# tpy001/VFMSeg

Hardware: AMD Instinct MI355X
Metric: train images/sec @512x512 DINOv2-L+LoRA (dg_lora_dinov2_ms_masked, 1024^2 sample = LR+HR 512^2 passes) (higher is better)
Workload: dtype bf16; 1 GPU; configs[1]: dg_lora_dinov2_ms_masked.py, synthetic 1024^2 19-class samples -> 2x512^2 passes, bs=2/GPU, full train step (fwd+bwd+allreduce+AdamW), LoRA dropout on; global_batch=2, parallelism=dp1

## Files before the change

vfmseg_amd/csrc/attention_bf16.hip:

```cpp
#include "attn_bf16_dev.h"

template <bool DQ, int NW = 4>
__global__ void __launch_bounds__(NW * 64, 2) k_attn_bf16_q(AttnP p) {
  extern __shared__ __attribute__((aligned(16))) char smem[];
  const int tid = threadIdx.x, lane = tid & 63;
  const int wave = __builtin_amdgcn_readfirstlane(tid >> 6);
  const int nq = p.nq_main + p.nq_extra, nk = p.nk_main + p.nk_extra;
  int bx, bh;
  {
    const bool light = !DQ && NW == 4 && p.nq_extra == 1 && (p.nq_main & 127) == 0 && nk <= ATTN_EXTRA_MAX;
    const int gx = gridDim.x, nbx = gx - (light ? 1 : 0), nfull = nbx * gridDim.y, lin = blockIdx.y * gx + blockIdx.x;
    if (lin >= nfull) {
      const int e = lin - nfull;
      if constexpr (!DQ) attn_extra_fwd(p, e / p.H, e % p.H, p.nq_main, smem);
      return;
    }
    xcd_map(lin, nbx, gridDim.y, p.xcd, bx, bh);
  }
  const bool cls_key = DQ && NW == 4 && p.nk_extra == 1 && p.cls_scratch != nullptr;
  const int b = bh / p.H, hh = bh % p.H;
  const int col0 = hh * 64;
  const int h = lane >> 5;
  const FragOff fo = frag_offsets(lane);
  const int q0 = bx * (NW * 32) + wave * 32;
  const int qi = q0 + (lane & 31);
  const bool qvalid = qi < nq;
  const long qrow = tok_row(b, qvalid ? qi : nq - 1, p.nq_main, p.B);
  const bf16_t* Kb = (const bf16_t*)p.k;
  const bf16_t* Vb = (const bf16_t*)p.v;
  bf16x8 qf[4], dof[4];
  load_stationary((const bf16_t*)p.q, p.ldq, qrow, col0, h, qf);
  float lse_l = 0.f, delta_l = 0.f;
  if (DQ) {
    load_stationary((const bf16_t*)p.dout, p.ld_do, qrow, col0, h, dof);
    lse_l = p.lse[((long)b * p.H + hh) * nq + (qvalid ? qi : nq - 1)] * LOG2E;
    bf16x8 of[4];
    load_stationary((const bf16_t*)p.o, p.ldo, qrow, col0, h, of);
    float dsum = 0.f;
#pragma unroll
    for (int kk = 0; kk < 4; ++kk)
#pragma unroll
      for (int e2 = 0; e2 < 8; ++e2) dsum = fmaf((float)dof[kk][e2], (float)of[kk][e2], dsum);
    delta_l = half_sum(dsum);
    if (qvalid && h == 0) p.delta[((long)b * p.H + hh) * nq + qi] = -delta_l;
    if (cls_key && p.nq_extra == 1 && bx == 0 && wave == 0) {
      const long crow = tok_row(b, p.nq_main, p.nq_main, p.B);
      bf16x8 cg[4], co[4];
      load_stationary((const bf16_t*)p.dout, p.ld_do, crow, col0, h, cg);
      load_stationary((const bf16_t*)p.o, p.ldo, crow, col0, h, co);
      float cs = 0.f;
#pragma unroll
      for (int kk = 0; kk < 4; ++kk)
#pragma unroll
        for (int e2 = 0; e2 < 8; ++e2) cs = fmaf((float)cg[kk][e2], (float)co[kk][e2], cs);
      cs = half_sum(cs);
      if (lane == 0) p.delta[((long)b * p.H + hh) * nq + p.nq_main] = -cs;
    }
  }
  float p_cls = 0.f, ds_cls = 0.f;
  const float c = p.scale * LOG2E;
  f32x16 oacc[2] = {zero16(), zero16()};
  float m = -INFINITY, l = 0.f;
  const bool r1 = NW == 4 && p.nk_extra == 1 && (!DQ || cls_key);
  const int nk_loop = r1 ? p.nk_main : nk;
  const int nt = (nk_loop + TROWS - 1) / TROWS;
  unsigned koff[8 / NW], voff[8 / NW];
  tile_offsets<NW>(p.ldk, wave, lane, koff);
  tile_offsets<NW>(p.ldv, wave, lane, voff);
  const int n_int = min(nk_loop, p.nk_main) / TROWS;
  const bool span_ok = 64l * p.ldk * 2 < (1l << 31) && 64l * p.ldv * 2 < (1l << 31);
  auto stage = [&](int buf, int t) {
    char* kt = smem + buf * 2 * TILE_BYTES;
    if (t < n_int && span_ok) {
      const long row0 = (long)b * p.nk_main + (long)t * TROWS;
      stage_tile_fast<NW>(Kb + row0 * p.ldk + col0, koff, kt, wave);
      stage_tile_fast<NW>(Vb + row0 * p.ldv + col0, voff, kt + TILE_BYTES, wave);
    } else {
      stage_tile<NW, true>(Kb, p.ldk, col0, b, t * TROWS, nk_loop, p.nk_main, p.B, kt, wave, lane);
      stage_tile<NW, true>(Vb, p.ldv, col0, b, t * TROWS, nk_loop, p.nk_main, p.B, kt + TILE_BYTES, wave, lane);
    }
  };
  stage(0, 0);
  if (r1) {
    const long crow = tok_row(b, p.nk_main, p.nk_main, p.B);
    bf16x8 kcf[4];
    load_stationary(Kb, p.ldk, crow, col0, h, kcf);
    const float s_e = dot_frag(qf, kcf);
    float oc[2][16];
    if (!DQ) {
      load_outcols(Vb, p.ldv, crow, col0, h, oc);
      m = s_e;
      l = h == 0 ? 1.f : 0.f;
#pragma unroll
      for (int j = 0; j < 2; ++j)
#pragma unroll
        for (int r = 0; r < 16; ++r) oacc[j][r] = oc[j][r];
    } else {
      bf16x8 vcf[4];
      load_stationary(Vb, p.ldv, crow, col0, h, vcf);
      const float dp_e = dot_frag(dof, vcf);
      p_cls = __builtin_amdgcn_exp2f(fmaf(s_e, c, -lse_l));
      ds_cls = p_cls * (dp_e - delta_l);
      load_outcols(Kb, p.ldk, crow, col0, h, oc);
#pragma unroll
      for (int j = 0; j < 2; ++j)
#pragma unroll
        for (int r = 0; r < 16; ++r) oacc[j][r] = ds_cls * oc[j][r];
    }
  }
#pragma unroll
  for (int kk = 0; kk < 4; ++kk) {
    asm volatile("" ::"v"(qf[kk]));
    if constexpr (DQ) asm volatile("" ::"v"(dof[kk]));
  }
  asm volatile("" ::"v"(lse_l), "v"(delta_l), "v"(m), "v"(l), "v"(p_cls), "v"(ds_cls));
#pragma unroll
  for (int j = 0; j < 2; ++j) asm volatile("" ::"v"(oacc[j]));
  constexpr int PT = 8 / NW;
  int buf = 0;
  for (int t = 0; t < nt; ++t) {
    const int nbuf = buf == 2 ? 0 : buf + 1;
    const bool il = (p.il & (DQ ? 2 : 1)) && (t + 1 < nt) && (t + 1 < n_int) && span_ok;
    if (t + 1 < nt && !il) {
      stage(nbuf, t + 1);
      if constexpr (NW == 4) asm volatile("s_waitcnt vmcnt(4)" ::: "memory");
      else asm volatile("s_waitcnt vmcnt(8)" ::: "memory");
    } else {
      asm volatile("s_waitcnt vmcnt(0)" ::: "memory");
    }
    __builtin_amdgcn_s_barrier();
    const char* kt = smem + buf * 2 * TILE_BYTES;
    const char* vt = kt + TILE_BYTES;
    f32x16 sacc[2] = {zero16(), zero16()};
    {
      bf16x8 kfr[8];
#pragma unroll
      for (int i = 0; i < 8; ++i) kfr[i] = row_frag(kt, fo, i >> 2, i & 3);
      char* nkt = smem + nbuf * 2 * TILE_BYTES;
      const long row1 = (long)b * p.nk_main + (long)(t + 1) * TROWS;
#pragma unroll
      for (int i = 0; i < 8; ++i) {
        sacc[i >> 2] = MFMA(kfr[i], qf[i & 3], sacc[i >> 2]);
        if (il) {
          if constexpr (NW == 4) {
            if (i & 1) {
              const int j = i >> 1;
              if (j < PT) stage_piece_fast<NW>(Kb + row1 * p.ldk + col0, koff[j], nkt, wave, j);
              else stage_piece_fast<NW>(Vb + row1 * p.ldv + col0, voff[j - PT], nkt + TILE_BYTES, wave, j - PT);
            }
          } else {
            if (i < PT) stage_piece_fast<NW>(Kb + row1 * p.ldk + col0, koff[i], nkt, wave, i);
            else stage_piece_fast<NW>(Vb + row1 * p.ldv + col0, voff[i - PT], nkt + TILE_BYTES, wave, i - PT);
          }
        }
      }
    }
    const bool tail = (t == nt - 1) && (nk_loop % TROWS != 0);
    if (!DQ) {
      float mx = -INFINITY;
      if (tail) {  asm volatile("" ::: "memory");
#pragma unroll
        for (int kb = 0; kb < 2; ++kb)
#pragma unroll
          for (int r = 0; r < 16; ++r)
            if (t * TROWS + kb * 32 + acc_row(r, h) >= nk_loop) sacc[kb][r] = -INFINITY;
      }
      {
        float m4[4] = {-INFINITY, -INFINITY, -INFINITY, -INFINITY};
#pragma unroll
        for (int kb = 0; kb < 2; ++kb)
#pragma unroll
          for (int r = 0; r < 16; ++r) m4[r & 3] = fmaxf(m4[r & 3], sacc[kb][r]);
        mx = fmaxf(fmaxf(m4[0], m4[1]), fmaxf(m4[2], m4[3]));
      }
      mx = half_max(mx);
      const bool need = (mx - m) * c > 8.0f;
      const float mn = need ? mx : m;
      const float alpha = need ? __builtin_amdgcn_exp2f((m - mn) * c) : 1.0f;
      const float mnc = mn * c;
      f32x2 rs2[2] = {f32x2{0.f, 0.f}, f32x2{0.f, 0.f}};
      const f32x2 c2 = f32x2{c, c}, mnc2 = f32x2{-mnc, -mnc};
#pragma unroll
      for (int kb = 0; kb < 2; ++kb)
#pragma unroll
        for (int r = 0; r < 16; r += 2) {
          const f32x2 x = __builtin_elementwise_fma(f32x2{sacc[kb][r], sacc[kb][r + 1]}, c2, mnc2);
          const f32x2 pv = f32x2{__builtin_amdgcn_exp2f(x.x), __builtin_amdgcn_exp2f(x.y)};
          sacc[kb][r] = pv.x, sacc[kb][r + 1] = pv.y;
          rs2[(r >> 1) & 1] += pv;
        }
      l = l * alpha + ((rs2[0].x + rs2[0].y) + (rs2[1].x + rs2[1].y));
      m = mn;
      if (__ballot(alpha != 1.0f) != 0ull) {
#pragma unroll
        for (int j = 0; j < 2; ++j)
#pragma unroll
          for (int r = 0; r < 16; ++r) oacc[j][r] *= alpha;
      }
    } else {
      f32x16 dpacc[2] = {zero16(), zero16()};
#pragma unroll
      for (int kb = 0; kb < 2; ++kb)
#pragma unroll
        for (int kk = 0; kk < 4; ++kk) dpacc[kb] = MFMA(row_frag(vt, fo, kb, kk), dof[kk], dpacc[kb]);
      {
        const f32x2 c2 = f32x2{c, c}, nl2 = f32x2{-lse_l, -lse_l}, nd2 = f32x2{-delta_l, -delta_l};
#pragma unroll
        for (int kb = 0; kb < 2; ++kb)
#pragma unroll
          for (int r = 0; r < 16; r += 2) {
            const f32x2 x = __builtin_elementwise_fma(f32x2{sacc[kb][r], sacc[kb][r + 1]}, c2, nl2);
            const f32x2 pv = f32x2{__builtin_amdgcn_exp2f(x.x), __builtin_amdgcn_exp2f(x.y)};
            const f32x2 ds = pv * (f32x2{dpacc[kb][r], dpacc[kb][r + 1]} + nd2);
            sacc[kb][r] = ds.x, sacc[kb][r + 1] = ds.y;
          }
      }
      if (tail) {  asm volatile("" ::: "memory");
#pragma unroll
        for (int kb = 0; kb < 2; ++kb)
#pragma unroll
          for (int r = 0; r < 16; ++r)
            if (t * TROWS + kb * 32 + acc_row(r, h) >= nk_loop) sacc[kb][r] = 0.f;
      }
    }
    const char* t2 = DQ ? kt : vt;
#pragma unroll
    for (int kb = 0; kb < 2; ++kb)
#pragma unroll
      for (int s = 0; s < 2; ++s) {
        const bf16x8 pb = acc_frag(sacc[kb], s);
#pragma unroll
        for (int j = 0; j < 2; ++j) oacc[j] = MFMA(tr_frag(t2, fo, kb, s, j), pb, oacc[j]);
      }
    buf = nbuf;
  }
  if constexpr (DQ) {
    if (cls_key) {
      __syncthreads();
      float* red = reinterpret_cast<float*>(smem) + wave * (32 * 65);
      float* scr = p.cls_scratch + ((long)b * p.H + hh) * 192;
      float wp = p_cls, wd = ds_cls;
      if (!qvalid) wp = 0.f, wd = 0.f;
      cls_partial(wd, qf, red, lane, scr + 64);
      cls_partial(wp, dof, red, lane, scr + 128);
    }
  }
  float mult;
  if (!DQ) {
    l = half_sum(l);
    mult = 1.f / l;
    if (qvalid && h == 0 && p.lse) p.lse[((long)b * p.H + hh) * nq + qi] = m * p.scale + __logf(l);
  } else {
    mult = p.scale;
  }
  if (qvalid) {
    bf16_t* out = DQ ? (bf16_t*)p.dq : (bf16_t*)p.o;
    const long ldo = DQ ? p.ld_dq : p.ldo;
#pragma unroll
    for (int j = 0; j < 2; ++j) store_block_rows(oacc[j], mult, out + qrow * ldo + col0 + 32 * j, h);
  }
}

template <int NW = 4>
__global__ void __launch_bounds__(NW * 64, 2) k_attn_bf16_dkv(AttnP p) {
  extern __shared__ __attribute__((aligned(16))) char smem[];
  constexpr int STAGE = 2 * TILE_BYTES + 1024;
  const int tid = threadIdx.x, lane = tid & 63;
  const int wave = __builtin_amdgcn_readfirstlane(tid >> 6);
  const int nq = p.nq_main + p.nq_extra, nk = p.nk_main + p.nk_extra;
  int bx, bh;
  xcd_map(blockIdx.y * gridDim.x + blockIdx.x, gridDim.x, gridDim.y, p.xcd, bx, bh);
  const bool cls_query = NW == 4 && p.nq_extra == 1 && p.cls_scratch != nullptr;
  float ds_cls = 0.f;
  const int b = bh / p.H, hh = bh % p.H;
  const int col0 = hh * 64;
  const int h = lane >> 5;
  const FragOff fo = frag_offsets(lane);
  const int k0 = bx * (NW * 32) + wave * 32;
  const int ki = k0 + (lane & 31);
  const bool kvalid = ki < nk;
  const long krow = tok_row(b, kvalid ? ki : nk - 1, p.nk_main, p.B);
  bf16x8 kf[4], vf[4];
  load_stationary((const bf16_t*)p.k, p.ldk, krow, col0, h, kf);
  load_stationary((const bf16_t*)p.v, p.ldv, krow, col0, h, vf);
  const bf16_t* Qb = (const bf16_t*)p.q;
  const bf16_t* Ob = (const bf16_t*)p.dout;
  const float* lse_g = p.lse + ((long)b * p.H + hh) * nq;
  const float* del_g = p.delta + ((long)b * p.H + hh) * nq;
  const float c = p.scale * LOG2E;
  f32x16 dk[2] = {zero16(), zero16()}, dv[2] = {zero16(), zero16()};
  const int nq_loop = cls_query ? p.nq_main : nq;
  const int nt = (nq_loop + TROWS - 1) / TROWS;
  unsigned qoff[8 / NW], ooff[8 / NW];
  tile_offsets<NW>(p.ldq, wave, lane, qoff);
  tile_offsets<NW>(p.ld_do, wave, lane, ooff);
  const int n_int = min(nq_loop, p.nq_main) / TROWS;
  const bool span_ok = 64l * p.ldq * 2 < (1l << 31) && 64l * p.ld_do * 2 < (1l << 31);
  auto stage = [&](int buf, int t) {
    char* qt = smem + buf * STAGE;
    if (t < n_int && span_ok) {
      const long row0 = (long)b * p.nq_main + (long)t * TROWS;
      stage_tile_fast<NW>(Qb + row0 * p.ldq + col0, qoff, qt, wave);
      stage_tile_fast<NW>(Ob + row0 * p.ld_do + col0, ooff, qt + TILE_BYTES, wave);
    } else {
      stage_tile<NW, true>(Qb, p.ldq, col0, b, t * TROWS, nq_loop, p.nq_main, p.B, qt, wave, lane);
      stage_tile<NW, true>(Ob, p.ld_do, col0, b, t * TROWS, nq_loop, p.nq_main, p.B, qt + TILE_BYTES, wave, lane);
    }
    int qq = t * TROWS + lane;
    if (qq > nq_loop - 1) qq = nq_loop - 1;
    const float* src = (wave & 1) ? del_g : lse_g;
    glds4_raw(src + qq, qt + 2 * TILE_BYTES + wave * 256);
  };
  stage(0, 0);
  if (cls_query) {
    const long crow = tok_row(b, p.nq_main, p.nq_main, p.B);
    bf16x8 qcf[4], gcf[4];
    load_stationary(Qb, p.ldq, crow, col0, h, qcf);
    load_stationary(Ob, p.ld_do, crow, col0, h, gcf);
    const float s_e = dot_frag(kf, qcf), dp_e = dot_frag(vf, gcf);
    const float p_e = __builtin_amdgcn_exp2f(fmaf(s_e, c, -lse_g[p.nq_main] * LOG2E));
    ds_cls = p_e * (dp_e + del_g[p.nq_main]);
    float oc[2][16];
    load_outcols(Ob, p.ld_do, crow, col0, h, oc);
#pragma unroll
    for (int j = 0; j < 2; ++j)
#pragma unroll
      for (int r = 0; r < 16; ++r) dv[j][r] = p_e * oc[j][r];
    load_outcols(Qb, p.ldq, crow, col0, h, oc);
#pragma unroll
    for (int j = 0; j < 2; ++j)
#pragma unroll
      for (int r = 0; r < 16; ++r) dk[j][r] = ds_cls * oc[j][r];
  }
#pragma unroll
  for (int kk = 0; kk < 4; ++kk) asm volatile("" ::"v"(kf[kk]), "v"(vf[kk]));
  asm volatile("" ::"v"(ds_cls));
#pragma unroll
  for (int j = 0; j < 2; ++j) asm volatile("" ::"v"(dk[j]), "v"(dv[j]));
  int buf = 0;
  for (int t = 0; t < nt; ++t) {
    const int nbuf = buf == 2 ? 0 : buf + 1;
    if (t + 1 < nt) {
      stage(nbuf, t + 1);
      if constexpr (NW == 4) asm volatile("s_waitcnt vmcnt(5)" ::: "memory");
      else asm volatile("s_waitcnt vmcnt(9)" ::: "memory");
    } else {
      asm volatile("s_waitcnt vmcnt(0)" ::: "memory");
    }
    __builtin_amdgcn_s_barrier();
    const char* qt = smem + buf * STAGE;
    const char* ot = qt + TILE_BYTES;
    const float* lse_s = reinterpret_cast<const float*>(qt + 2 * TILE_BYTES);
    const float* del_s = lse_s + 64;
    const bool tail = (t == nt - 1) && (nq_loop % TROWS != 0);
#pragma unroll
    for (int qb = 0; qb < 2; ++qb) {
      f32x16 sacc = zero16(), dpacc;
#pragma unroll
      for (int g = 0; g < 4; ++g) {
        const float4 nd = *reinterpret_cast<const float4*>(del_s + qb * 32 + 8 * g + 4 * h);
        dpacc[4 * g] = nd.x, dpacc[4 * g + 1] = nd.y, dpacc[4 * g + 2] = nd.z, dpacc[4 * g + 3] = nd.w;
      }
#pragma unroll
      for (int kk = 0; kk < 4; ++kk) {
        sacc = MFMA(row_frag(qt, fo, qb, kk), kf[kk], sacc);
        dpacc = MFMA(row_frag(ot, fo, qb, kk), vf[kk], dpacc);
      }
      f32x16 pacc;
#pragma unroll
      for (int g = 0; g < 4; ++g) {
        const float4 ls = *reinterpret_cast<const float4*>(lse_s + qb * 32 + 8 * g + 4 * h);
        const f32x2 c2 = f32x2{c, c}, nl2e = f32x2{-LOG2E, -LOG2E};
        const f32x2 lsv[2] = {f32x2{ls.x, ls.y} * nl2e, f32x2{ls.z, ls.w} * nl2e};
#pragma unroll
        for (int e = 0; e < 2; ++e) {
          const int r = 4 * g + 2 * e;
          const f32x2 x = __builtin_elementwise_fma(f32x2{sacc[r], sacc[r + 1]}, c2, lsv[e]);
          const f32x2 pv = f32x2{__builtin_amdgcn_exp2f(x.x), __builtin_amdgcn_exp2f(x.y)};
          const f32x2 ds = pv * f32x2{dpacc[r], dpacc[r + 1]};
          pacc[r] = pv.x, pacc[r + 1] = pv.y;
          sacc[r] = ds.x, sacc[r + 1] = ds.y;
        }
      }
      if (tail) {  asm volatile("" ::: "memory");
#pragma unroll
        for (int r = 0; r < 16; ++r)
          if (t * TROWS + qb * 32 + acc_row(r, h) >= nq_loop) pacc[r] = 0.f, sacc[r] = 0.f;
      }
#pragma unroll
      for (int s = 0; s < 2; ++s) {
        const bf16x8 pb = acc_frag(pacc, s), dsb = acc_frag(sacc, s);
#pragma unroll
        for (int j = 0; j < 2; ++j) {
          dv[j] = MFMA(tr_frag(ot, fo, qb, s, j), pb, dv[j]);
          dk[j] = MFMA(tr_frag(qt, fo, qb, s, j), dsb, dk[j]);
        }
      }
    }
    buf = nbuf;
  }
  if (cls_query) {
    __syncthreads();
    float* red = reinterpret_cast<float*>(smem) + wave * (32 * 65);
    float wd = ds_cls;
    if (!kvalid) wd = 0.f;
    cls_partial(wd, kf, red, lane, p.cls_scratch + ((long)b * p.H + hh) * 192);
  }
  if (kvalid) {
    bf16_t* odk = (bf16_t*)p.dk;
    bf16_t* odv = (bf16_t*)p.dv;
#pragma unroll
    for (int j = 0; j < 2; ++j) {
      store_block_rows(dk[j], p.scale, odk + krow * p.ld_dk + col0 + 32 * j, h);
      store_block_rows(dv[j], 1.0f, odv + krow * p.ld_dv + col0 + 32 * j, h);
    }
  }
}

static bool aligned_ok(const vfm_attn_desc* d, bool bwd) {
  auto ok = [](const void* ptr, long ld) { return ((uintptr_t)ptr % 16 == 0) && (ld % 8 == 0); };
  bool r = ok(d->q, d->ldq) && ok(d->k, d->ldk) && ok(d->v, d->ldv) && ok(d->o, d->ldo);
  if (bwd) r = r && ok(d->dout, d->ld_do) && ok(d->dq, d->ld_dq) && ok(d->dk, d->ld_dk) && ok(d->dv, d->ld_dv);
  return r;
}

int g_attn_short_grid = 256;
static bool short_grid(const vfm_attn_desc* d, int n) { return (long)cdiv(n, 128) * d->B * d->H < g_attn_short_grid; }

int g_attn_il = 3;
int g_attn_xcd = 1;
int g_attn_fwd64 = 0;
#ifdef VFM_EXPERIMENTAL_FWD64
bool vfm_attn_fwd64_launch(const vfm_attn_desc* d, const AttnP& p, hipStream_t s);
#else
static bool vfm_attn_fwd64_launch(const vfm_attn_desc*, const AttnP&, hipStream_t) { return false; }
#endif
int g_attn_lds_pad = 0;
int vfm_attn_bf16_fwd_impl(const vfm_attn_desc* d, hipStream_t s) {
  VFM_CHECK(aligned_ok(d, false), VFM_E_ALIGN, "vfm_attn_fwd(bf16): operands must be 16-byte aligned, ld %% 8 == 0");
  const AttnP p = to_p(d);
  const int nq = d->nq_main + d->nq_extra;
  if (g_attn_fwd64 && vfm_attn_fwd64_launch(d, p, s)) {
    VFM_LAUNCH_CHECK();
    return VFM_OK;
  }
  const size_t shm = 6 * TILE_BYTES + g_attn_lds_pad;
  static int attr_pad = -1;
  if (attr_pad != g_attn_lds_pad) {
    (void)hipFuncSetAttribute((const void*)k_attn_bf16_q<false, 4>, hipFuncAttributeMaxDynamicSharedMemorySize, (int)shm);
    attr_pad = g_attn_lds_pad;
  }
  if (short_grid(d, nq)) hipLaunchKernelGGL((k_attn_bf16_q<false, 2>), dim3(cdiv(nq, 64), d->B * d->H), dim3(128), shm, s, p);
  else hipLaunchKernelGGL((k_attn_bf16_q<false, 4>), dim3(cdiv(nq, 128), d->B * d->H), dim3(256), shm, s, p);
  VFM_LAUNCH_CHECK();
  return VFM_OK;
}

__global__ void __launch_bounds__(64) k_attn_cls_finish(AttnP p) {
  const int bh = blockIdx.x, b = bh / p.H, hh = bh % p.H, lane = threadIdx.x;
  const int nq = p.nq_main + p.nq_extra;
  const long row = tok_row(b, p.nq_main, p.nq_main, p.B);
  const int col = hh * 64 + lane;
  const float qc = bf16_to_f32(((const bf16_t*)p.q)[row * p.ldq + col]), kc = bf16_to_f32(((const bf16_t*)p.k)[row * p.ldk + col]);
  const float vc = bf16_to_f32(((const bf16_t*)p.v)[row * p.ldv + col]), gc = bf16_to_f32(((const bf16_t*)p.dout)[row * p.ld_do + col]);
  const float s = wave_sum(qc * kc) * p.scale, dp = wave_sum(gc * vc);
  const float lse = p.lse[(long)bh * nq + p.nq_main], ndelta = p.delta[(long)bh * nq + p.nq_main];
  const float pv = __expf(s - lse), ds = pv * (dp + ndelta);
  float* scr = p.cls_scratch + (long)bh * 192;
  ((bf16_t*)p.dq)[row * p.ld_dq + col] = f32_to_bf16((scr[lane] + ds * kc) * p.scale);
  ((bf16_t*)p.dk)[row * p.ld_dk + col] = f32_to_bf16((scr[64 + lane] + ds * qc) * p.scale);
  ((bf16_t*)p.dv)[row * p.ld_dv + col] = f32_to_bf16(scr[128 + lane] + pv * gc);
  scr[lane] = 0.f, scr[64 + lane] = 0.f, scr[128 + lane] = 0.f;
}

int vfm_attn_bf16_bwd_impl(const vfm_attn_desc* d, hipStream_t s) {
  VFM_CHECK(aligned_ok(d, true), VFM_E_ALIGN, "vfm_attn_bwd(bf16): operands must be 16-byte aligned, ld %% 8 == 0");
  AttnP p = to_p(d);
  const int nq = d->nq_main + d->nq_extra, nk = d->nk_main + d->nk_extra;
  const bool cls = d->nq_extra == 1 && d->nk_extra == 1 && d->nq_main == d->nk_main && (d->nq_main % 128) == 0 && !short_grid(d, nq);
  p.cls_scratch = cls ? d->delta + (long)d->B * d->H * nq : nullptr;
  if (short_grid(d, nq)) hipLaunchKernelGGL((k_attn_bf16_q<true, 2>), dim3(cdiv(nq, 64), d->B * d->H), dim3(128), 6 * TILE_BYTES, s, p);
  else hipLaunchKernelGGL((k_attn_bf16_q<true, 4>), dim3(cdiv(cls ? d->nq_main : nq, 128), d->B * d->H), dim3(256), 6 * TILE_BYTES, s, p);
  if (short_grid(d, nk)) hipLaunchKernelGGL((k_attn_bf16_dkv<2>), dim3(cdiv(nk, 64), d->B * d->H), dim3(128), 3 * (2 * TILE_BYTES + 1024), s, p);
  else hipLaunchKernelGGL((k_attn_bf16_dkv<4>), dim3(cdiv(cls ? d->nk_main : nk, 128), d->B * d->H), dim3(256), 3 * (2 * TILE_BYTES + 1024), s, p);
  if (cls) hipLaunchKernelGGL(k_attn_cls_finish, dim3(d->B * d->H), dim3(64), 0, s, p);
  VFM_LAUNCH_CHECK();
  return VFM_OK;
}
```

vfmseg_amd/csrc/attn_common.h:

```cpp
#pragma once
#include "common.h"

struct AttnP {
  const void* q; const void* k; const void* v; void* o;
  int dt; long ldq, ldk, ldv, ldo;
  int B, H;
  int nq_main, nq_extra, nk_main, nk_extra;
  float scale;
  float* lse;
  const void* dout; long ld_do;
  void* dq; void* dk; void* dv; long ld_dq, ld_dk, ld_dv;
  float* delta;
  float* cls_scratch;
  int xcd;
  int il;
};

__device__ __forceinline__ long tok_row(int b, int i, int n_main, int B) {
  return i < n_main ? (long)b * n_main + i : (long)B * n_main + b;
}


static inline AttnP to_p(const vfm_attn_desc* d) {
  AttnP p;
  p.q = d->q; p.k = d->k; p.v = d->v; p.o = d->o;
  p.dt = d->dt; p.ldq = d->ldq; p.ldk = d->ldk; p.ldv = d->ldv; p.ldo = d->ldo;
  p.B = d->B; p.H = d->H;
  p.nq_main = d->nq_main; p.nq_extra = d->nq_extra; p.nk_main = d->nk_main; p.nk_extra = d->nk_extra;
  p.scale = d->scale; p.lse = d->lse;
  p.dout = d->dout; p.ld_do = d->ld_do;
  p.dq = d->dq; p.dk = d->dk; p.dv = d->dv; p.ld_dq = d->ld_dq; p.ld_dk = d->ld_dk; p.ld_dv = d->ld_dv;
  p.delta = d->delta;
  p.cls_scratch = nullptr;
  extern int g_attn_xcd;
  p.xcd = g_attn_xcd;
  extern int g_attn_il;
  p.il = g_attn_il;
  return p;
}
```

vfmseg_amd/csrc/elementwise.hip:

```cpp
#include "common.h"

thread_local char g_vfm_err[512] = {0};

extern "C" const char* vfm_last_error(void) { return g_vfm_err; }
extern "C" int vfm_abi_version(void) { return 5; }
extern "C" int vfm_half_kind(void) { return VFM_HALF_KIND; }

template <typename TI, typename TO>
__global__ void k_cast(const TI* __restrict__ src, long ld_src, TO* __restrict__ dst, long ld_dst, long rows, long cols,
                       const float* __restrict__ colscale) {
  const long cols4 = cols >> 2;
  const long total = rows * cols4;
  for (long i = blockIdx.x * (long)blockDim.x + threadIdx.x; i < total; i += (long)gridDim.x * blockDim.x) {
    const long r = i / cols4, c = (i - r * cols4) << 2;
    float v[4];
#pragma unroll
    for (int j = 0; j < 4; ++j) v[j] = ld_f32(src + r * ld_src + c + j);
    if (colscale) {
#pragma unroll
      for (int j = 0; j < 4; ++j) v[j] *= colscale[c + j];
    }
#pragma unroll
    for (int j = 0; j < 4; ++j) st_f32(dst + r * ld_dst + c + j, v[j]);
  }
  const long tail0 = cols4 << 2;
  const long ntail = cols - tail0;
  if (ntail) {
    for (long i = blockIdx.x * (long)blockDim.x + threadIdx.x; i < rows * ntail; i += (long)gridDim.x * blockDim.x) {
      const long r = i / ntail, c = tail0 + (i - r * ntail);
      float v = ld_f32(src + r * ld_src + c);
      if (colscale) v *= colscale[c];
      st_f32(dst + r * ld_dst + c, v);
    }
  }
}

extern "C" int vfm_cast(const void* src, int src_dt, long ld_src, void* dst, int dst_dt, long ld_dst, long rows, long cols,
                        const float* colscale, void* stream) {
  VFM_CHECK(rows >= 0 && cols >= 0 && ld_src >= cols && ld_dst >= cols, VFM_E_SHAPE, "vfm_cast: bad shape");
  if (rows == 0 || cols == 0) return VFM_OK;
  hipStream_t s = (hipStream_t)stream;
  const long total = rows * ((cols + 3) / 4);
  const int grid = (int)((total + 255) / 256 > 4096 ? 4096 : (total + 255) / 256);
#define L(TI, TO) hipLaunchKernelGGL((k_cast<TI, TO>), dim3(grid), dim3(256), 0, s, (const TI*)src, ld_src, (TO*)dst, ld_dst, rows, cols, colscale)
  if (src_dt == VFM_F32 && dst_dt == VFM_F32) L(float, float);
  else if (src_dt == VFM_F32 && dst_dt == VFM_BF16) L(float, bf16_t);
  else if (src_dt == VFM_BF16 && dst_dt == VFM_F32) L(bf16_t, float);
  else if (src_dt == VFM_BF16 && dst_dt == VFM_BF16) L(bf16_t, bf16_t);
  else VFM_FAIL(VFM_E_INVAL, "vfm_cast: dtype");
#undef L
  VFM_LAUNCH_CHECK();
  return VFM_OK;
}

__global__ void k_split3(const float* __restrict__ src, long sr, long sc, bf16_t* __restrict__ dst, long ld_dst, long rows, long K, long Kp,
                         int pattern) {
  const long per_row = Kp / 4;
  const long total = rows * per_row;
  for (long i = (long)blockIdx.x * blockDim.x + threadIdx.x; i < total; i += (long)gridDim.x * blockDim.x) {
    const long r = i / per_row, c = (i % per_row) * 4;
    float v[4];
    if (sc == 1 && c + 3 < K && ((reinterpret_cast<uintptr_t>(src + r * sr + c) & 15) == 0)) {
      const float4 f = *reinterpret_cast<const float4*>(src + r * sr + c);
      v[0] = f.x, v[1] = f.y, v[2] = f.z, v[3] = f.w;
    } else {
#pragma unroll
      for (int e = 0; e < 4; ++e) v[e] = (c + e < K) ? src[r * sr + (c + e) * sc] : 0.f;
    }
    ushort4 hi, lo;
    bf16_t* ph = &hi.x;
    bf16_t* pl = &lo.x;
#pragma unroll
    for (int e = 0; e < 4; ++e) {
      ph[e] = f32_to_bf16(v[e]);
      pl[e] = f32_to_bf16(v[e] - bf16_to_f32(ph[e]));
    }
    bf16_t* d = dst + r * ld_dst + c;
    *reinterpret_cast<ushort4*>(d) = hi;
    *reinterpret_cast<ushort4*>(d + Kp) = pattern == 0 ? hi : lo;
    *reinterpret_cast<ushort4*>(d + 2 * Kp) = pattern == 0 ? lo : hi;
  }
}

extern "C" int vfm_split3(const float* src, long stride_r, long stride_c, void* dst, long ld_dst, long rows, long K, int pattern, void* stream) {
  const long Kp = (K + 63) / 64 * 64;
  VFM_CHECK(rows >= 0 && K > 0 && ld_dst >= 3 * Kp && ld_dst % 4 == 0 && ((uintptr_t)dst % 8) == 0 && (pattern == 0 || pattern == 1), VFM_E_SHAPE,
            "vfm_split3: dst must hold rows x 3 ceil64(K) bf16 (ld %% 4 == 0, 8-byte aligned)");
  if (rows == 0) return VFM_OK;
  const long total = rows * (Kp / 4);
  const int grid = (int)((total + 255) / 256 > 8192 ? 8192 : (total + 255) / 256);
  hipLaunchKernelGGL(k_split3, dim3(grid), dim3(256), 0, (hipStream_t)stream, src, stride_r, stride_c, (bf16_t*)dst, ld_dst, rows, K, Kp, pattern);
  VFM_LAUNCH_CHECK();
  return VFM_OK;
}

template <typename TI, typename TO>
__global__ void k_transpose(const TI* __restrict__ src, long ld_src, TO* __restrict__ dst, long ld_dst, long rows, long cols,
                            long pad_rows) {
  __shared__ float tile[64][65];
  const long r0 = (long)blockIdx.y * 64, c0 = (long)blockIdx.x * 64;
  const int tx = threadIdx.x & 63, ty = threadIdx.x >> 6;
  for (int i = ty; i < 64; i += 4) {
    const long r = r0 + i, c = c0 + tx;
    tile[i][tx] = (r < rows && c < cols) ? ld_f32(src + r * ld_src + c) : 0.f;
  }
  __syncthreads();
  for (int i = ty; i < 64; i += 4) {
    const long c = c0 + i, r = r0 + tx;
    if (c < cols && r < pad_rows) st_f32(dst + c * ld_dst + r, tile[tx][i]);
  }
}

extern "C" int vfm_transpose(const void* src, int src_dt, long ld_src, void* dst, int dst_dt, long ld_dst, long rows, long cols,
                             long pad_rows, void* stream) {
  VFM_CHECK(pad_rows >= rows && ld_dst >= pad_rows && ld_src >= cols, VFM_E_SHAPE, "vfm_transpose: bad shape");
  if (cols == 0 || pad_rows == 0) return VFM_OK;
  hipStream_t s = (hipStream_t)stream;
  dim3 grid(cdiv(cols, 64), cdiv(pad_rows, 64));
#define L(TI, TO) hipLaunchKernelGGL((k_transpose<TI, TO>), grid, dim3(256), 0, s, (const TI*)src, ld_src, (TO*)dst, ld_dst, rows, cols, pad_rows)
  if (src_dt == VFM_F32 && dst_dt == VFM_F32) L(float, float);
  else if (src_dt == VFM_F32 && dst_dt == VFM_BF16) L(float, bf16_t);
  else if (src_dt == VFM_BF16 && dst_dt == VFM_F32) L(bf16_t, float);
  else if (src_dt == VFM_BF16 && dst_dt == VFM_BF16) L(bf16_t, bf16_t);
  else VFM_FAIL(VFM_E_INVAL, "vfm_transpose: dtype");
#undef L
  VFM_LAUNCH_CHECK();
  return VFM_OK;
}

template <typename TI, typename TO>
__global__ void k_strided_copy(const TI* __restrict__ src, TO* __restrict__ dst, long n0, long n1, long n2, long n3, long s0,
                               long s1, long s2, long s3, long d0, long d1, long d2, long d3, int accumulate) {
  const long total = n0 * n1 * n2 * n3;
  for (long i = blockIdx.x * (long)blockDim.x + threadIdx.x; i < total; i += (long)gridDim.x * blockDim.x) {
    long t = i;
    const long i3 = t % n3; t /= n3;
    const long i2 = t % n2; t /= n2;
    const long i1 = t % n1; t /= n1;
    const float v = ld_f32(src + t * s0 + i1 * s1 + i2 * s2 + i3 * s3);
    TO* q = dst + t * d0 + i1 * d1 + i2 * d2 + i3 * d3;
    st_f32(q, accumulate ? ld_f32(q) + v : v);
  }
}

extern "C" int vfm_strided_copy(const void* src, int src_dt, void* dst, int dst_dt, long n0, long n1, long n2, long n3,
                                long s0, long s1, long s2, long s3, long d0, long d1, long d2, long d3, int accumulate,
                                void* stream) {
  const long total = n0 * n1 * n2 * n3;
  if (total == 0) return VFM_OK;
  hipStream_t s = (hipStream_t)stream;
  const int grid = (int)((total + 255) / 256 > 4096 ? 4096 : (total + 255) / 256);
#define L(TI, TO) hipLaunchKernelGGL((k_strided_copy<TI, TO>), dim3(grid), dim3(256), 0, s, (const TI*)src, (TO*)dst, n0, n1, n2, n3, s0, s1, s2, s3, d0, d1, d2, d3, accumulate)
  if (src_dt == VFM_F32 && dst_dt == VFM_F32) L(float, float);
  else if (src_dt == VFM_F32 && dst_dt == VFM_BF16) L(float, bf16_t);
  else if (src_dt == VFM_BF16 && dst_dt == VFM_F32) L(bf16_t, float);
  else if (src_dt == VFM_BF16 && dst_dt == VFM_BF16) L(bf16_t, bf16_t);
  else VFM_FAIL(VFM_E_INVAL, "vfm_strided_copy: dtype");
#undef L
  VFM_LAUNCH_CHECK();
  return VFM_OK;
}

__global__ void k_axpby(const float* __restrict__ x, float a, float* __restrict__ y, float b, long n) {
  for (long i = blockIdx.x * (long)blockDim.x + threadIdx.x; i < n; i += (long)gridDim.x * blockDim.x)
    y[i] = (b == 0.f) ? a * x[i] : a * x[i] + b * y[i];
}
extern "C" int vfm_axpby(const float* x, float a, float* y, float b, long n, void* stream) {
  if (n == 0) return VFM_OK;
  const int grid = (int)((n + 255) / 256 > 4096 ? 4096 : (n + 255) / 256);
  hipLaunchKernelGGL(k_axpby, dim3(grid), dim3(256), 0, (hipStream_t)stream, x, a, y, b, n);
  VFM_LAUNCH_CHECK();
  return VFM_OK;
}
__global__ void k_scale_dev(float* __restrict__ y, const float* __restrict__ sc, long n) {
  const float s = *sc;
  for (long i = blockIdx.x * (long)blockDim.x + threadIdx.x; i < n; i += (long)gridDim.x * blockDim.x) y[i] *= s;
}
extern "C" int vfm_scale_by_device_scalar(float* y, const float* scalar, long n, void* stream) {
  if (n == 0) return VFM_OK;
  const int grid = (int)((n + 255) / 256 > 4096 ? 4096 : (n + 255) / 256);
  hipLaunchKernelGGL(k_scale_dev, dim3(grid), dim3(256), 0, (hipStream_t)stream, y, scalar, n);
  VFM_LAUNCH_CHECK();
  return VFM_OK;
}

template <typename T>
__global__ void k_colsum1(const T* __restrict__ x, long ld, long rows, long cols, float* __restrict__ ws, int CT) {
  __shared__ float sh[256];
  const int rl = 256 / CT;
  const int tx = threadIdx.x % CT, ty = threadIdx.x / CT;
  const long c = (long)blockIdx.x * CT + tx;
  float acc = 0.f;
  if (c < cols)
    for (long r = (long)blockIdx.y * rl + ty; r < rows; r += (long)gridDim.y * rl) acc += ld_f32(x + r * ld + c);
  sh[threadIdx.x] = acc;
  __syncthreads();
  if (ty == 0 && c < cols) {
    float a = 0.f;
    for (int k = 0; k < rl; ++k) a += sh[k * CT + tx];
    ws[(long)blockIdx.y * cols + c] = a;
  }
}
__global__ void __launch_bounds__(256) k_colsum2(const float* __restrict__ ws, long cols, int parts, float* __restrict__ out, int accumulate) {
  __shared__ float sh[4][64];
  const int tx = threadIdx.x & 63, g = threadIdx.x >> 6;
  const long c = blockIdx.x * 64L + tx;
  float a = 0.f;
  if (c < cols) {
    int p = g;
    for (; p + 12 < parts; p += 16) {
      const float v0 = ws[(long)p * cols + c], v1 = ws[(long)(p + 4) * cols + c], v2 = ws[(long)(p + 8) * cols + c], v3 = ws[(long)(p + 12) * cols + c];
      a += (v0 + v1) + (v2 + v3);
    }
    for (; p < parts; p += 4) a += ws[(long)p * cols + c];
  }
  sh[g][tx] = a;
  __syncthreads();
  if (g == 0 && c < cols) {
    const float t = (sh[0][tx] + sh[1][tx]) + (sh[2][tx] + sh[3][tx]);
    out[c] = accumulate ? out[c] + t : t;
  }
}
extern "C" int vfm_colsum(const void* x, int dt, long ld, long rows, long cols, float* out, int accumulate, float* ws,
                          void* stream) {
  VFM_CHECK(ld >= cols && ws, VFM_E_SHAPE, "vfm_colsum: bad args");
  if (cols == 0) return VFM_OK;
  hipStream_t s = (hipStream_t)stream;
  int CT = 64;
  while (CT > 8 && CT / 2 >= cols) CT /= 2;
  const int rl = 256 / CT;
  long parts = (rows + rl * 8 - 1) / (rl * 8);
  if (parts > 64) parts = 64;
  if (parts < 1) parts = 1;
  dim3 grid(cdiv(cols, CT), (unsigned)parts);
  if (dt == VFM_F32) hipLaunchKernelGGL(k_colsum1<float>, grid, dim3(256), 0, s, (const float*)x, ld, rows, cols, ws, CT);
  else if (dt == VFM_BF16) hipLaunchKernelGGL(k_colsum1<bf16_t>, grid, dim3(256), 0, s, (const bf16_t*)x, ld, rows, cols, ws, CT);
  else VFM_FAIL(VFM_E_INVAL, "vfm_colsum: dtype");
  hipLaunchKernelGGL(k_colsum2, dim3(cdiv(cols, 64)), dim3(256), 0, s, ws, cols, (int)parts, out, accumulate);
  VFM_LAUNCH_CHECK();
  return VFM_OK;
}

__global__ void k_slab_reduce(const float* __restrict__ slabs, int kch, long P, long Q, long rows_used, float alpha,
                              float* __restrict__ dst, long sp, long sq, int accumulate) {
  const long total = rows_used * Q;
  for (long i = blockIdx.x * (long)blockDim.x + threadIdx.x; i < total; i += (long)gridDim.x * blockDim.x) {
    const long p = i / Q, q = i - p * Q;
    float a = 0.f;
    for (int k = 0; k < kch; ++k) a += slabs[((long)k * P + p) * Q + q];
    a *= alpha;
    float* d = dst + p * sp + q * sq;
    *d = accumulate ? *d + a : a;
  }
}
extern "C" int vfm_slab_reduce(const float* slabs, int kch, long P, long Q, long rows_used, float alpha, float* dst, long sp,
                               long sq, int accumulate, void* stream) {
  VFM_CHECK(kch >= 1 && rows_used >= 0 && rows_used <= P, VFM_E_SHAPE, "vfm_slab_reduce: bad shape");
  const long total = rows_used * Q;
  if (total == 0) return VFM_OK;
  const int grid = (int)((total + 255) / 256 > 4096 ? 4096 : (total + 255) / 256);
  hipLaunchKernelGGL(k_slab_reduce, dim3(grid), dim3(256), 0, (hipStream_t)stream, slabs, kch, P, Q, rows_used, alpha, dst, sp, sq,
                     accumulate);
  VFM_LAUNCH_CHECK();
  return VFM_OK;
}

__global__ void __launch_bounds__(256) k_strided_copy_batch(const vfm_copy_job* __restrict__ tab) {
  const vfm_copy_job t = tab[blockIdx.y];
  const unsigned n1 = (unsigned)t.n[1], n2 = (unsigned)t.n[2], n3 = (unsigned)t.n[3];
  const unsigned total = (unsigned)t.n[0] * n1 * n2 * n3;
  for (unsigned i = blockIdx.x * 256u + threadIdx.x; i < total; i += gridDim.x * 256u) {
    unsigned r = i;
    const unsigned i3 = r % n3; r /= n3;
    const unsigned i2 = r % n2; r /= n2;
    const unsigned i1 = r % n1; r /= n1;
    const float* sp = t.src + ((long)r * t.s[0] + (long)i1 * t.s[1] + (long)i2 * t.s[2] + (long)i3 * t.s[3]);
    float v = sp[0];
    for (long c = 1; c < t.nsum; ++c) v += sp[c * t.sum_stride];
    const long o = (long)r * t.d[0] + (long)i1 * t.d[1] + (long)i2 * t.d[2] + (long)i3 * t.d[3];
    if (t.accumulate) ((float*)t.dst)[o] += v;
    else st_any(t.dst, o, (int)t.dst_dt, v);
  }
}
extern "C" int vfm_strided_copy_batch(const vfm_copy_job* table_dev, int njobs, long max_elems, void* stream) {
  VFM_CHECK(table_dev && njobs >= 0, VFM_E_INVAL, "vfm_strided_copy_batch: bad args");
  if (njobs == 0 || max_elems <= 0) return VFM_OK;
  VFM_CHECK(max_elems < (1l << 31), VFM_E_SHAPE, "vfm_strided_copy_batch: jobs are limited to 2^31 elements");
  int gx = (int)((max_elems + 2047) / 2048);
  if (gx > 2048) gx = 2048;
  if (gx < 1) gx = 1;
  hipLaunchKernelGGL(k_strided_copy_batch, dim3(gx, njobs), dim3(256), 0, (hipStream_t)stream, table_dev);
  VFM_LAUNCH_CHECK();
  return VFM_OK;
}

__global__ void k_lora_pack(const vfm_lora_site* __restrict__ tab, int dt) {
  const vfm_lora_site t = tab[blockIdx.y];
  const long na = t.r * t.K, nb = t.N * t.r;
  for (long i = blockIdx.x * (long)blockDim.x + threadIdx.x; i < na + nb; i += (long)gridDim.x * blockDim.x) {
    if (i < na) {
      const long rr = i / t.K, k = i - rr * t.K;
      const float v = t.A[i];
      st_any(t.a, rr * t.ld_a + k, dt, v);
      st_any(t.at, k * t.ld_at + rr, dt, v);
    } else {
      const long j = i - na;
      const long n = j / t.r, rr = j - n * t.r;
      const float v = t.B[j];
      st_any(t.w, n * t.ld_w + t.Kw + rr, dt, v);
      if (t.wt) st_any(t.wt, (t.Kw + rr) * t.ld_wt + n, dt, v);
    }
  }
}
extern "C" int vfm_lora_pack(const vfm_lora_site* table_dev, int nsites, long max_elems, int dt, void* stream) {
  VFM_CHECK(table_dev && nsites >= 0 && (dt == VFM_F32 || dt == VFM_BF16), VFM_E_INVAL, "vfm_lora_pack: bad args");
  if (nsites == 0) return VFM_OK;
  int gx = (int)((max_elems + 255) / 256);
  if (gx > 256) gx = 256;
  if (gx < 1) gx = 1;
  hipLaunchKernelGGL(k_lora_pack, dim3(gx, nsites), dim3(256), 0, (hipStream_t)stream, table_dev, dt);
  VFM_LAUNCH_CHECK();
  return VFM_OK;
}

struct F8 { float v[8]; };
__device__ __forceinline__ F8 ld8_bf16(const bf16_t* p) {
  const uint4 u = *reinterpret_cast<const uint4*>(p);
  F8 r;
  r.v[0] = h16_lo(u.x), r.v[1] = h16_hi(u.x);
  r.v[2] = h16_lo(u.y), r.v[3] = h16_hi(u.y);
  r.v[4] = h16_lo(u.z), r.v[5] = h16_hi(u.z);
  r.v[6] = h16_lo(u.w), r.v[7] = h16_hi(u.w);
  return r;
}
__device__ __forceinline__ void st8_bf16(bf16_t* p, const F8& r) {
  uint4 u;
  u.x = (uint32_t)f32_to_bf16(r.v[0]) | ((uint32_t)f32_to_bf16(r.v[1]) << 16);
  u.y = (uint32_t)f32_to_bf16(r.v[2]) | ((uint32_t)f32_to_bf16(r.v[3]) << 16);
  u.z = (uint32_t)f32_to_bf16(r.v[4]) | ((uint32_t)f32_to_bf16(r.v[5]) << 16);
  u.w = (uint32_t)f32_to_bf16(r.v[6]) | ((uint32_t)f32_to_bf16(r.v[7]) << 16);
  *reinterpret_cast<uint4*>(p) = u;
}
__device__ __forceinline__ F8 ld8_f32(const float* p) {
  const float4 a = *reinterpret_cast<const float4*>(p), b = *reinterpret_cast<const float4*>(p + 4);
  F8 r;
  r.v[0] = a.x, r.v[1] = a.y, r.v[2] = a.z, r.v[3] = a.w, r.v[4] = b.x, r.v[5] = b.y, r.v[6] = b.z, r.v[7] = b.w;
  return r;
}
__device__ __forceinline__ void st8_f32(float* p, const F8& r) {
  *reinterpret_cast<float4*>(p) = make_float4(r.v[0], r.v[1], r.v[2], r.v[3]);
  *reinterpret_cast<float4*>(p + 4) = make_float4(r.v[4], r.v[5], r.v[6], r.v[7]);
}
static inline bool al16(const void* p) { return ((uintptr_t)p & 15) == 0; }
static inline int grid8(long total8) { return (int)((total8 + 255) / 256 > 16384 ? 16384 : (total8 + 255) / 256); }

__global__ void k_dropout_mask_bf16x8(bf16_t* __restrict__ out, long n8, float p, float keep_scale, uint64_t seed, uint64_t offset) {
  for (long i = blockIdx.x * (long)blockDim.x + threadIdx.x; i < n8; i += (long)gridDim.x * blockDim.x) {
    F8 r;
#pragma unroll
    for (int e = 0; e < 8; ++e) {
      const float u = (hash_u32(seed, offset + (uint64_t)(i * 8 + e)) >> 8) * (1.0f / 16777216.0f);
      r.v[e] = u >= p ? keep_scale : 0.f;
    }
    st8_bf16(out + i * 8, r);
  }
}
__global__ void k_mul_mask_bf16x8(const bf16_t* __restrict__ src, long ld_src, const bf16_t* __restrict__ mask, long mask_ld, long rpg,
                                  bf16_t* __restrict__ dst, long ld_dst, long rows, int cols8) {
  const long total = rows * cols8;
  for (long i = blockIdx.x * (long)blockDim.x + threadIdx.x; i < total; i += (long)gridDim.x * blockDim.x) {
    const long r = i / cols8;
    const int c = (int)(i - r * cols8) * 8;
    F8 a = ld8_bf16(src + r * ld_src + c);
    const F8 m = ld8_bf16(mask + (r / rpg) * mask_ld + c);
#pragma unroll
    for (int e = 0; e < 8; ++e) a.v[e] *= m.v[e];
    st8_bf16(dst + r * ld_dst + c, a);
  }
}
__global__ void k_act_grad_mul_bf16x8(const bf16_t* __restrict__ dy, long ld_dy, const bf16_t* __restrict__ pre, long ld_pre,
                                      bf16_t* __restrict__ out, long ld_out, long rows, int cols8, int act) {
  const long total = rows * cols8;
  for (long i = blockIdx.x * (long)blockDim.x + threadIdx.x; i < total; i += (long)gridDim.x * blockDim.x) {
    const long r = i / cols8;
    const int c = (int)(i - r * cols8) * 8;
    F8 d = ld8_bf16(dy + r * ld_dy + c);
    const F8 p = ld8_bf16(pre + r * ld_pre + c);
#pragma unroll
    for (int e = 0; e < 8; ++e) {
      const float x = p.v[e];
      const float g = act == VFM_ACT_GELU ? gelu_grad_f(x) : (act == VFM_ACT_RELU ? (x > 0.f ? 1.f : 0.f) : (act == VFM_ACT_QGELU ? qgelu_grad_f(x) : 1.f));
      d.v[e] *= g;
    }
    st8_bf16(out + r * ld_out + c, d);
  }
}
template <bool OUT_BF16>
__global__ void k_swiglu_fwd_x8(const bf16_t* __restrict__ h, long ld_h, void* __restrict__ out, long ld_out, long rows, long C, int c8) {
  const long total = rows * c8;
  for (long i = blockIdx.x * (long)blockDim.x + threadIdx.x; i < total; i += (long)gridDim.x * blockDim.x) {
    const long r = i / c8;
    const int c = (int)(i - r * c8) * 8;
    const F8 a = ld8_bf16(h + r * ld_h + c), g = ld8_bf16(h + r * ld_h + C + c);
    F8 o;
#pragma unroll
    for (int e = 0; e < 8; ++e) o.v[e] = a.v[e] / (1.f + __expf(-a.v[e])) * g.v[e];
    if constexpr (OUT_BF16) st8_bf16((bf16_t*)out + r * ld_out + c, o);
    else st8_f32((float*)out + r * ld_out + c, o);
  }
}
template <bool DO_BF16>
__global__ void k_swiglu_bwd_x8(const bf16_t* __restrict__ h, long ld_h, const void* __restrict__ dout, long ld_do, bf16_t* __restrict__ dh,
                                long ld_dh, long rows, long C, int c8) {
  const long total = rows * c8;
  for (long i = blockIdx.x * (long)blockDim.x + threadIdx.x; i < total; i += (long)gridDim.x * blockDim.x) {
    const long r = i / c8;
    const int c = (int)(i - r * c8) * 8;
    const F8 a = ld8_bf16(h + r * ld_h + c), g = ld8_bf16(h + r * ld_h + C + c);
    F8 d;
    if constexpr (DO_BF16) d = ld8_bf16((const bf16_t*)dout + r * ld_do + c);
    else d = ld8_f32((const float*)dout + r * ld_do + c);
    F8 da, dg;
#pragma unroll
    for (int e = 0; e < 8; ++e) {
      const float sg = 1.f / (1.f + __expf(-a.v[e]));
      da.v[e] = d.v[e] * g.v[e] * sg * (1.f + a.v[e] * (1.f - sg));
      dg.v[e] = d.v[e] * a.v[e] * sg;
    }
    st8_bf16(dh + r * ld_dh + c, da);
    st8_bf16(dh + r * ld_dh + C + c, dg);
  }
}

template <typename T>
__global__ void k_dropout_mask(T* __restrict__ out, long n, float p, float keep_scale, uint64_t seed, uint64_t offset) {
  for (long i = blockIdx.x * (long)blockDim.x + threadIdx.x; i < n; i += (long)gridDim.x * blockDim.x) {
    const float u = (hash_u32(seed, offset + (uint64_t)i) >> 8) * (1.0f / 16777216.0f);
    st_f32(out + i, u >= p ? keep_scale : 0.f);
  }
}
extern "C" int vfm_dropout_mask(void* out, int dt, long n, float p, uint64_t seed, uint64_t offset, void* stream) {
  VFM_CHECK(p >= 0.f && p < 1.f, VFM_E_INVAL, "vfm_dropout_mask: p");
  if (n == 0) return VFM_OK;
  const int grid = (int)((n + 255) / 256 > 4096 ? 4096 : (n + 255) / 256);
  const float ks = 1.0f / (1.0f - p);
  if (dt == VFM_F32) hipLaunchKernelGGL(k_dropout_mask<float>, dim3(grid), dim3(256), 0, (hipStream_t)stream, (float*)out, n, p, ks, seed, offset);
  else if (dt == VFM_BF16 && n % 8 == 0 && al16(out))
    hipLaunchKernelGGL(k_dropout_mask_bf16x8, dim3(grid8(n / 8)), dim3(256), 0, (hipStream_t)stream, (bf16_t*)out, n / 8, p, ks, seed, offset);
  else if (dt == VFM_BF16) hipLaunchKernelGGL(k_dropout_mask<bf16_t>, dim3(grid), dim3(256), 0, (hipStream_t)stream, (bf16_t*)out, n, p, ks, seed, offset);
  else VFM_FAIL(VFM_E_INVAL, "vfm_dropout_mask: dtype");
  VFM_LAUNCH_CHECK();
  return VFM_OK;
}

__global__ void k_mul_mask(const void* __restrict__ src, int src_dt, long ld_src, const void* __restrict__ mask, int mask_dt,
                           long mask_ld, long rpg, void* __restrict__ dst, int dst_dt, long ld_dst, long rows, long cols) {
  const long total = rows * cols;
  for (long i = blockIdx.x * (long)blockDim.x + threadIdx.x; i < total; i += (long)gridDim.x * blockDim.x) {
    const long r = i / cols, c = i - r * cols;
    const float m = ld_any(mask, (r / rpg) * mask_ld + c, mask_dt);
    st_any(dst, r * ld_dst + c, dst_dt, ld_any(src, r * ld_src + c, src_dt) * m);
  }
}
template <typename TS, typename TM, typename TD>
__global__ void k_mul_mask_x8(const TS* __restrict__ src, long ld_src, const TM* __restrict__ mask, long mask_ld, long rpg, TD* __restrict__ dst,
                              long ld_dst, long rows, int cols8) {
  const long total = rows * cols8;
  for (long i = blockIdx.x * (long)blockDim.x + threadIdx.x; i < total; i += (long)gridDim.x * blockDim.x) {
    const long r = i / cols8;
    const int c = (int)(i - r * cols8) * 8;
    F8 a, m;
    if constexpr (sizeof(TS) == 2) a = ld8_bf16(src + r * ld_src + c); else a = ld8_f32(src + r * ld_src + c);
    if constexpr (sizeof(TM) == 2) m = ld8_bf16(mask + (r / rpg) * mask_ld + c); else m = ld8_f32(mask + (r / rpg) * mask_ld + c);
#pragma unroll
    for (int e = 0; e < 8; ++e) a.v[e] *= m.v[e];
    if constexpr (sizeof(TD) == 2) st8_bf16(dst + r * ld_dst + c, a); else st8_f32(dst + r * ld_dst + c, a);
  }
}
template <typename TS, typename TM, typename TD>
static void launch_mul_mask_x8(const void* src, long ld_src, const void* mask, long mask_ld, long rpg, void* dst, long ld_dst, long rows, long cols,
                               hipStream_t s) {
  hipLaunchKernelGGL((k_mul_mask_x8<TS, TM, TD>), dim3(grid8(rows * cols / 8)), dim3(256), 0, s, (const TS*)src, ld_src, (const TM*)mask, mask_ld, rpg,
                     (TD*)dst, ld_dst, rows, (int)(cols / 8));
}
extern "C" int vfm_mul_mask(const void* src, int src_dt, long ld_src, const void* mask, int mask_dt, long mask_ld,
                            long rows_per_group, void* dst, int dst_dt, long ld_dst, long rows, long cols, void* stream) {
  VFM_CHECK(rows_per_group >= 1, VFM_E_INVAL, "vfm_mul_mask: rows_per_group");
  const long total = rows * cols;
  if (total == 0) return VFM_OK;
  auto h16 = [](int dt) { return dt == VFM_BF16; };
  auto okdt = [](int dt) { return dt == VFM_BF16 || dt == VFM_F32; };
  if (okdt(src_dt) && okdt(mask_dt) && okdt(dst_dt) && !(h16(src_dt) && h16(mask_dt) && h16(dst_dt)) && cols % 8 == 0 && ld_src % 8 == 0 &&
      mask_ld % 8 == 0 && ld_dst % 8 == 0 && al16(src) && al16(mask) && al16(dst)) {
    hipStream_t s = (hipStream_t)stream;
    const int key = (h16(src_dt) ? 4 : 0) | (h16(mask_dt) ? 2 : 0) | (h16(dst_dt) ? 1 : 0);
#define MM(TS, TM, TD) launch_mul_mask_x8<TS, TM, TD>(src, ld_src, mask, mask_ld, rows_per_group, dst, ld_dst, rows, cols, s)
    switch (key) {
      case 0: MM(float, float, float); break;
      case 1: MM(float, float, bf16_t); break;
      case 2: MM(float, bf16_t, float); break;
      case 3: MM(float, bf16_t, bf16_t); break;
      case 4: MM(bf16_t, float, float); break;
      case 5: MM(bf16_t, float, bf16_t); break;
      default: MM(bf16_t, bf16_t, float); break;
    }
#undef MM
    VFM_LAUNCH_CHECK();
    return VFM_OK;
  }
  if (src_dt == VFM_BF16 && mask_dt == VFM_BF16 && dst_dt == VFM_BF16 && cols % 8 == 0 && ld_src % 8 == 0 && mask_ld % 8 == 0 && ld_dst % 8 == 0 &&
      al16(src) && al16(mask) && al16(dst)) {
    hipLaunchKernelGGL(k_mul_mask_bf16x8, dim3(grid8(total / 8)), dim3(256), 0, (hipStream_t)stream, (const bf16_t*)src, ld_src, (const bf16_t*)mask,
                       mask_ld, rows_per_group, (bf16_t*)dst, ld_dst, rows, (int)(cols / 8));
    VFM_LAUNCH_CHECK();
    return VFM_OK;
  }
  const int grid = (int)((total + 255) / 256 > 8192 ? 8192 : (total + 255) / 256);
  hipLaunchKernelGGL(k_mul_mask, dim3(grid), dim3(256), 0, (hipStream_t)stream, src, src_dt, ld_src, mask, mask_dt, mask_ld,
                     rows_per_group, dst, dst_dt, ld_dst, rows, cols);
  VFM_LAUNCH_CHECK();
  return VFM_OK;
}

__global__ void k_geglu_fwd(const void* __restrict__ h, int h_dt, long ld_h, void* __restrict__ out, int out_dt, long ld_out,
                            long rows, long C) {
  const long total = rows * C;
  for (long i = blockIdx.x * (long)blockDim.x + threadIdx.x; i < total; i += (long)gridDim.x * blockDim.x) {
    const long r = i / C, c = i - r * C;
    const float a = ld_any(h, r * ld_h + c, h_dt), g = ld_any(h, r * ld_h + C + c, h_dt);
    st_any(out, r * ld_out + c, out_dt, a * gelu_f(g));
  }
}
__global__ void k_geglu_bwd(const void* __restrict__ h, int h_dt, long ld_h, const void* __restrict__ dout, int do_dt,
                            long ld_do, void* __restrict__ dh, int dh_dt, long ld_dh, long rows, long C) {
  const long total = rows * C;
  for (long i = blockIdx.x * (long)blockDim.x + threadIdx.x; i < total; i += (long)gridDim.x * blockDim.x) {
    const long r = i / C, c = i - r * C;
    const float a = ld_any(h, r * ld_h + c, h_dt), g = ld_any(h, r * ld_h + C + c, h_dt);
    const float d = ld_any(dout, r * ld_do + c, do_dt);
    st_any(dh, r * ld_dh + c, dh_dt, d * gelu_f(g));
    st_any(dh, r * ld_dh + C + c, dh_dt, d * a * gelu_grad_f(g));
// ... 297 lines not shown
```

vfmseg_amd/csrc/gemm_bf16.hip:

```cpp
#include "gemm_dev.h"

template <int BM, int BN, int WM_W, int WN_W, int NS>
struct Cfg {
  static constexpr int WAVES = WM_W * WN_W;
  static constexpr int THREADS = WAVES * 64;
  static constexpr int A_BYTES = BM * BK * 2, B_BYTES = BN * BK * 2;
  static constexpr int STAGE_BYTES = A_BYTES + B_BYTES;
  static constexpr int A_PIECES = BM / 8 / WAVES, B_PIECES = BN / 8 / WAVES;
  static constexpr int PIECES = A_PIECES + B_PIECES;
  static constexpr int WM = BM / WM_W, WN = BN / WN_W;
  static constexpr int MI = WM / 32, NI = WN / 32;
  static constexpr int EPI_LD = WN + 4;
  static constexpr int EPI_BYTES = WAVES * 32 * EPI_LD * 4;
  static constexpr int SMEM = (NS * STAGE_BYTES > EPI_BYTES) ? NS * STAGE_BYTES : EPI_BYTES;
  static_assert(BM % (8 * WAVES) == 0 && BN % (8 * WAVES) == 0, "tile rows must split into whole DMA pieces per wave");
  static_assert(WM % 32 == 0 && WN % 32 == 0, "wave tile must be a multiple of the 32x32 MFMA");
};

typedef short s16x4 __attribute__((ext_vector_type(4)));

__device__ __attribute__((aligned(16))) unsigned char g_zero_row[512];
template <int BM, int BN, int WM_W, int WN_W, int NS, bool VEC, bool BT, bool AT = false>
__global__ void __launch_bounds__(WM_W* WN_W * 64)
    k_gemm_bf16(const bf16_t* __restrict__ A, long lda, const bf16_t* __restrict__ B, long ldb, long M, long N, long K,
                long stride_a, long stride_b, long stride_c, int tiles_m, int tiles_n, long kb_rows, EpiParams e, SkinnyTail sk) {
  using C = Cfg<BM, BN, WM_W, WN_W, NS>;
  extern __shared__ __attribute__((aligned(16))) char smem[];
  if constexpr (!BT && C::THREADS == 512 && C::SMEM >= 65536) {
    if (sk.nblk > 0 && (int)blockIdx.x >= tiles_m * tiles_n) {
      skinny_tile(sk.A, sk.lda, B, ldb, sk.M, N, K, (long)((int)blockIdx.x - tiles_m * tiles_n) * 32, sk.e, 0, smem);
      return;
    }
  }
  const int tid = threadIdx.x, lane = tid & 63;
  const int wave = __builtin_amdgcn_readfirstlane(tid >> 6);
  const int wm = wave / WN_W, wn = wave % WN_W;

  const int ntiles = tiles_m * tiles_n;
  int bid = blockIdx.x;
  {
    const int q = ntiles >> 3, r = ntiles & 7, xcd = bid & 7, idx = bid >> 3;
    bid = (xcd < r ? xcd * (q + 1) : r * (q + 1) + (xcd - r) * q) + idx;
  }
  constexpr int GM = 8;
  const int group = bid / (GM * tiles_n);
  const int first_m = group * GM;
  const int gsz = min(tiles_m - first_m, GM);
  const int tm = first_m + (bid % (GM * tiles_n)) % gsz;
  const int tn = (bid % (GM * tiles_n)) / gsz;
  const long m0 = (long)tm * BM, n0 = (long)tn * BN;
  const long z = blockIdx.y;
  const bf16_t* Ab = A + z * stride_a;
  const bf16_t* Bb = B + z * stride_b;
  long kb_valid = K;
  if constexpr (BT) {
    if (kb_rows > 0) {
      kb_valid = kb_rows - (ldb > 0 ? z * (stride_b / ldb) : 0);
      if (kb_valid > K) kb_valid = K;
      if (kb_valid < 1) kb_valid = 1;
    } else if (kb_rows < 0) {
      kb_valid = -kb_rows;
      if (kb_valid > K) kb_valid = K;
    }
  }

  const int lr = lane >> 3, pc = lane & 7;
  const bf16_t* a_src[C::A_PIECES];
  const bf16_t* b_src[C::B_PIECES];
  int at_row[C::A_PIECES];
#pragma unroll
  for (int j = 0; j < C::A_PIECES; ++j) {
    if constexpr (!AT) {
      const int r = (wave * C::A_PIECES + j) * 8 + lr;
      long gm = m0 + r;
      if (gm > M - 1) gm = M - 1;
      a_src[j] = Ab + gm * lda + ((pc ^ ((r >> 1) & 7)) << 3);
    } else {
      static_assert(!AT || (BT && BM == 128), "transposed-A path: BM = 128 (256-byte LDS rows), together with transposed B");
      const int piece = wave * C::A_PIECES + j;
      const int r = piece * 4 + (lane >> 4);
      const int c = (lane & 15) ^ ((r & 3) << 2);
      long gm = m0 + c * 8;
      if (gm > M - 8) gm = M - 8;
      at_row[j] = r;
      a_src[j] = Ab + gm;
    }
  }
  int bt_row[C::B_PIECES];
#pragma unroll
  for (int j = 0; j < C::B_PIECES; ++j) {
    if constexpr (!BT) {
      const int r = (wave * C::B_PIECES + j) * 8 + lr;
      long gn = n0 + r;
      if (gn > N - 1) gn = N - 1;
      b_src[j] = Bb + gn * ldb + ((pc ^ ((r >> 1) & 7)) << 3);
    } else {
      static_assert(!BT || BN == 128, "transposed-B path is built for BN = 128 (256-byte LDS rows)");
      const int piece = wave * C::B_PIECES + j;
      const int r = piece * 4 + (lane >> 4);
      const int c = (lane & 15) ^ ((r & 3) << 2);
      long gn = n0 + c * 8;
      if (gn > N - 8) gn = N - 8;
      bt_row[j] = r;
      b_src[j] = Bb + gn;
    }
  }
  auto stage = [&](int slot, long k0) {
    char* sa = smem + slot * C::STAGE_BYTES;
    char* sb = sa + C::A_BYTES;
#pragma unroll
    for (int j = 0; j < C::A_PIECES; ++j) {
      if constexpr (!AT) {
        glds16(a_src[j] + k0, sa + (wave * C::A_PIECES + j) * 1024);
      } else {
        const long kr = k0 + at_row[j];
        const bf16_t* src = kr < kb_valid ? a_src[j] + kr * lda : reinterpret_cast<const bf16_t*>(g_zero_row) + (lane & 15) * 8;
        glds16(src, sa + (wave * C::A_PIECES + j) * 1024);
      }
    }
#pragma unroll
    for (int j = 0; j < C::B_PIECES; ++j) {
      if constexpr (!BT) {
        glds16(b_src[j] + k0, sb + (wave * C::B_PIECES + j) * 1024);
      } else {
        long kr = k0 + bt_row[j];
        if (kr > kb_valid - 1) kr = kb_valid - 1;
        glds16(b_src[j] + kr * ldb, sb + (wave * C::B_PIECES + j) * 1024);
      }
    }
  };

  f32x16 acc[C::MI][C::NI];
#pragma unroll
  for (int i = 0; i < C::MI; ++i)
#pragma unroll
    for (int j = 0; j < C::NI; ++j)
#pragma unroll
      for (int r = 0; r < 16; ++r) acc[i][j][r] = 0.f;

  const int fr = lane & 31, fh = lane >> 5;
  int a_off[C::MI], a_sw[C::MI], b_off[C::NI], b_sw[C::NI];
#pragma unroll
  for (int i = 0; i < C::MI; ++i) {
    const int r = wm * C::WM + i * 32 + fr;
    a_off[i] = r * 128;
    a_sw[i] = (r >> 1) & 7;
  }
#pragma unroll
  for (int j = 0; j < C::NI; ++j) {
    const int r = wn * C::WN + j * 32 + fr;
    b_off[j] = r * 128;
    b_sw[j] = (r >> 1) & 7;
  }

  const int nk = (int)(K / BK);
#pragma unroll
  for (int s = 0; s < NS - 1; ++s)
    if (s < nk) stage(s, (long)s * BK);

  for (int t = 0; t < nk; ++t) {
    const int inflight = min(NS - 2, nk - 1 - t);
    if (inflight >= NS - 2 && NS >= 2) wait_vmcnt<(NS - 2) * C::PIECES>();
    else if (NS >= 4 && inflight == NS - 3) wait_vmcnt<(NS >= 3 ? (NS - 3) : 0) * C::PIECES>();
    else if (NS >= 5 && inflight == NS - 4) wait_vmcnt<(NS >= 4 ? (NS - 4) : 0) * C::PIECES>();
    else wait_vmcnt<0>();
    __builtin_amdgcn_s_barrier();
    if (t + NS - 1 < nk) stage((t + NS - 1) % NS, (long)(t + NS - 1) * BK);
    const char* sa = smem + (t % NS) * C::STAGE_BYTES;
    const char* sb = sa + C::A_BYTES;
    auto read_b = [&](int s2, int j) -> bf16x8 {
      if constexpr (!BT) {
        return *reinterpret_cast<const bf16x8*>(sb + b_off[j] + (((2 * s2 + fh) ^ b_sw[j]) << 4));
      } else {
        const int g = lane >> 4, i2 = lane & 15, q = i2 >> 2, p = i2 & 3, h2 = g >> 1;
        const int chunk = (wn * C::WN + j * 32) / 8 + 2 * (g & 1) + (p >> 1);
        const int r0 = 16 * s2 + 8 * h2 + q, r1 = r0 + 4;
        const s16x4 lo = __builtin_amdgcn_ds_read_tr16_b64_v4i16(
            (__attribute__((address_space(3))) s16x4*)(sb + r0 * 256 + ((chunk ^ ((r0 & 3) << 2)) << 4) + ((p & 1) << 3)));
        const s16x4 hi = __builtin_amdgcn_ds_read_tr16_b64_v4i16(
            (__attribute__((address_space(3))) s16x4*)(sb + r1 * 256 + ((chunk ^ ((r1 & 3) << 2)) << 4) + ((p & 1) << 3)));
        union { struct { s16x4 a, b; } st; bf16x8 v; } u;
        u.st.a = lo;
        u.st.b = hi;
        return u.v;
      }
    };
    auto read_a = [&](int s2, int i) -> bf16x8 {
      if constexpr (!AT) {
        return *reinterpret_cast<const bf16x8*>(sa + a_off[i] + (((2 * s2 + fh) ^ a_sw[i]) << 4));
      } else {
        const int g = lane >> 4, i2 = lane & 15, q = i2 >> 2, p = i2 & 3, h2 = g >> 1;
        const int chunk = (wm * C::WM + i * 32) / 8 + 2 * (g & 1) + (p >> 1);
        const int r0 = 16 * s2 + 8 * h2 + q, r1 = r0 + 4;
        const s16x4 lo = __builtin_amdgcn_ds_read_tr16_b64_v4i16(
            (__attribute__((address_space(3))) s16x4*)(sa + r0 * 256 + ((chunk ^ ((r0 & 3) << 2)) << 4) + ((p & 1) << 3)));
        const s16x4 hi = __builtin_amdgcn_ds_read_tr16_b64_v4i16(
            (__attribute__((address_space(3))) s16x4*)(sa + r1 * 256 + ((chunk ^ ((r1 & 3) << 2)) << 4) + ((p & 1) << 3)));
        union { struct { s16x4 a, b; } st; bf16x8 v; } u;
        u.st.a = lo;
        u.st.b = hi;
        return u.v;
      }
    };
    bf16x8 af[2][C::MI], bfr[2][C::NI];
#pragma unroll
    for (int i = 0; i < C::MI; ++i) af[0][i] = read_a(0, i);
#pragma unroll
    for (int j = 0; j < C::NI; ++j) bfr[0][j] = read_b(0, j);
#pragma unroll
    for (int s = 0; s < BK / 16; ++s) {
      const int cur = s & 1, nxt = cur ^ 1;
      if (s + 1 < BK / 16) {
#pragma unroll
        for (int i = 0; i < C::MI; ++i)
          af[nxt][i] = read_a(s + 1, i);
#pragma unroll
        for (int j = 0; j < C::NI; ++j) bfr[nxt][j] = read_b(s + 1, j);
      }
#pragma unroll
      for (int i = 0; i < C::MI; ++i)
#pragma unroll
        for (int j = 0; j < C::NI; ++j)
          acc[i][j] = VFM_MFMA16(af[cur][i], bfr[cur][j], acc[i][j]);
    }
  }

  const long zoff = z * stride_c;
  __syncthreads();
  float* img = reinterpret_cast<float*>(smem) + wave * 32 * C::EPI_LD;
  if constexpr (VEC) epi_wave_tile<C::MI, C::NI, 1>(e, zoff, acc, img, lane, m0 + wm * C::WM, n0 + wn * C::WN, M, N);
  else epi_scalar<C::MI, C::NI, 1>(e, zoff, acc, img, lane, m0 + wm * C::WM, n0 + wn * C::WN, M, N);
}

template <int BM, int BN, int WM_W, int WN_W, int NS, bool VEC, bool BT, bool AT = false>
static bool launch_one(const vfm_gemm_desc* d, hipStream_t s, const vfm_gemm_desc* tail = nullptr) {
  using C = Cfg<BM, BN, WM_W, WN_W, NS>;
  const int tiles_m = cdiv(d->M, BM), tiles_n = cdiv(d->N, BN);
  const long batch = d->batch > 0 ? d->batch : 1;
  static bool attr = false;
  if (!attr) {
    (void)hipFuncSetAttribute((const void*)k_gemm_bf16<BM, BN, WM_W, WN_W, NS, VEC, BT, AT>, hipFuncAttributeMaxDynamicSharedMemorySize, C::SMEM);
    attr = true;
  }
  SkinnyTail sk;
  sk.nblk = 0;
  const bool fold = tail && !BT && C::THREADS == 512 && C::SMEM >= 65536 && batch == 1;
  if (fold) {
    sk.A = (const bf16_t*)tail->A, sk.lda = tail->sa_m, sk.M = tail->M, sk.nblk = cdiv(tail->N, 32), sk.e = make_epi(tail);
  }
  dim3 grid(tiles_m * tiles_n + sk.nblk, (unsigned)batch), blk(C::THREADS);
  const long ldb = BT ? d->sb_k : d->sb_n;
  const long kb_rows = d->kb_rows;
  hipLaunchKernelGGL((k_gemm_bf16<BM, BN, WM_W, WN_W, NS, VEC, BT, AT>), grid, blk, C::SMEM, s, (const bf16_t*)d->A, AT ? d->sa_k : d->sa_m,
                     (const bf16_t*)d->B, ldb, d->M, d->N, d->K, d->stride_a, d->stride_b, d->stride_c, tiles_m, tiles_n, kb_rows,
                     make_epi(d), sk);
  return fold || !tail;
}

template <int BM, int BN, int WM_W, int WN_W, int NS>
static bool launch_cfg(const vfm_gemm_desc* d, hipStream_t s, bool vec, const vfm_gemm_desc* tail = nullptr) {
  if (vec) return launch_one<BM, BN, WM_W, WN_W, NS, true, false>(d, s, tail);
  return launch_one<BM, BN, WM_W, WN_W, NS, false, false>(d, s, tail);
}

template <int BM, int WM_W, int WN_W, int NS = 2>
static void launch_bt(const vfm_gemm_desc* d, hipStream_t s, bool vec) {
  if (vec) launch_one<BM, 128, WM_W, WN_W, NS, true, true>(d, s);
  else launch_one<BM, 128, WM_W, WN_W, NS, false, true>(d, s);
}

__global__ void __launch_bounds__(512) k_gemm_bf16_skinny(const bf16_t* __restrict__ A, long lda, const bf16_t* __restrict__ B, long ldb,
                                                          long M, long N, long K, long stride_a, long stride_b, long stride_c,
                                                          EpiParams e) {
  __shared__ __attribute__((aligned(16))) char stg[65536];
  const long z = blockIdx.y;
  skinny_tile(A + z * stride_a, lda, B + z * stride_b, ldb, M, N, K, (long)blockIdx.x * 32, e, z * stride_c, stg);
}

static void launch_skinny(const vfm_gemm_desc* d, hipStream_t s) {
  const long batch = d->batch > 0 ? d->batch : 1;
  hipLaunchKernelGGL(k_gemm_bf16_skinny, dim3(cdiv(d->N, 32), (unsigned)batch), dim3(512), 0, s, (const bf16_t*)d->A, d->sa_m,
                     (const bf16_t*)d->B, d->sb_n, d->M, d->N, d->K, d->stride_a, d->stride_b, d->stride_c, make_epi(d));
}

static int g_force_cfg = -1;
static int g_split_tail = 3;
static int g_batch_tiles = 1;
static int g_bt64 = 1;
static int g_fold_tail = 1;
static int g_use_pp = 184;
long g_nt_bytes = 0;
static int g_use_ps = 0;
static int g_use_192 = 3;
static int g_w44_k = 1024;
static int g_deep_sep_k = 0;
static int g_deep_tail_k = 0;
extern "C" int vfm_tune(const char* key, int value) {
  if (key && strcmp(key, "gemm_cfg") == 0) {
    g_force_cfg = value;
    return VFM_OK;
  }
  if (key && strcmp(key, "pp_dbg") == 0) {
    extern int g_pp_dbg;
    g_pp_dbg = value;
    return VFM_OK;
  }
  if (key && strcmp(key, "attn_short_grid") == 0) {
    extern int g_attn_short_grid;
    g_attn_short_grid = value;
    return VFM_OK;
  }
  if (key && strcmp(key, "attn_il") == 0) {
    if (value < 0 || value > 3) VFM_FAIL(VFM_E_INVAL, "vfm_tune(attn_il): 0 .. 3");
    extern int g_attn_il;
    g_attn_il = value;
    return VFM_OK;
  }
  if (key && strcmp(key, "attn_xcd") == 0) {
    extern int g_attn_xcd;
    g_attn_xcd = value;
    return VFM_OK;
  }
  if (key && strcmp(key, "attn_fwd64") == 0) {
    extern int g_attn_fwd64;
    g_attn_fwd64 = value;
    return VFM_OK;
  }
  if (key && strcmp(key, "attn_lds_pad") == 0) {
    extern int g_attn_lds_pad;
    g_attn_lds_pad = value;
    return VFM_OK;
  }
  if (key && strcmp(key, "gemm_w44_k") == 0) {
    if (value < 0) VFM_FAIL(VFM_E_INVAL, "vfm_tune(gemm_w44_k): negative value");
    g_w44_k = value;
    return VFM_OK;
  }
  if (key && strcmp(key, "gemm_deep_sep_k") == 0) {
    if (value < 0) return VFM_E_INVAL;
    g_deep_sep_k = value;
    return VFM_OK;
  }
  if (key && strcmp(key, "gemm_deep_tail_k") == 0) {
    g_deep_tail_k = value;
    return VFM_OK;
  }
  if (key && strcmp(key, "gemm_nt_mb") == 0) {
    g_nt_bytes = (long)value << 20;
    return VFM_OK;
  }
  if (key && strcmp(key, "ps_burst") == 0) {
#ifdef VFM_EXPERIMENTAL_GEMM
    extern int g_ps_burst;
    g_ps_burst = value;
#endif
    return VFM_OK;
  }
  if (key && strcmp(key, "gemm_use_ps") == 0) {
    g_use_ps = value;
    return VFM_OK;
  }
  if (key && strcmp(key, "gemm_use_pp") == 0) {
    g_use_pp = value;
    return VFM_OK;
  }
  if (key && strcmp(key, "gemm_use_192") == 0) {
    g_use_192 = value;
    return VFM_OK;
  }
  if (key && strcmp(key, "gemm_batch_tiles") == 0) {
    g_batch_tiles = value;
    return VFM_OK;
  }
  if (key && strcmp(key, "gemm_bt64") == 0) {
    g_bt64 = value;
    return VFM_OK;
  }
  if (key && strcmp(key, "gemm_fold_tail") == 0) {
    g_fold_tail = value;
    return VFM_OK;
  }
  if (key && strcmp(key, "gemm_split_tail") == 0) {
    g_split_tail = value;
    return VFM_OK;
  }
  VFM_FAIL(VFM_E_INVAL, "vfm_tune: unknown key");
}

static bool vec_ok(const vfm_gemm_desc* d) {
  auto a16 = [](const void* p) { return ((uintptr_t)p % 16) == 0; };
  const long bm = d->bias_mod > 0 ? d->bias_mod : d->N;
  bool ok = (d->N % 4 == 0) && (d->ldc % 4 == 0) && a16(d->C) && (d->stride_c % 4 == 0);
  if (d->bias) ok = ok && a16(d->bias) && (bm % 4 == 0);
  if (d->colscale) ok = ok && a16(d->colscale);
  if (d->residual) ok = ok && a16(d->residual) && (d->ldr % 4 == 0);
  if (d->aux) ok = ok && a16(d->aux) && (d->ld_aux % 4 == 0);
  if (d->C2) ok = ok && a16(d->C2) && (d->ldc2 % 4 == 0);
  return ok;
}

static int gemm_main(const vfm_gemm_desc* d, hipStream_t s, const vfm_gemm_desc* tail = nullptr, bool* folded = nullptr);
bool vfm_gemm_launch_pp256(const vfm_gemm_desc* d, hipStream_t s, bool vec, const vfm_gemm_desc* tail);
bool vfm_gemm_launch_pp128(const vfm_gemm_desc* d, hipStream_t s, bool vec, const vfm_gemm_desc* tail);
bool vfm_gemm_launch_w4(const vfm_gemm_desc* d, hipStream_t s, bool vec, const vfm_gemm_desc* tail, int waves);
bool vfm_gemm_splitk_ok(const vfm_gemm_desc* d, bool vec);
bool vfm_gemm_launch_w4_splitk(const vfm_gemm_desc* d, hipStream_t s, const vfm_gemm_desc* tail);
#ifdef VFM_EXPERIMENTAL_GEMM
bool vfm_gemm_launch_v5(const vfm_gemm_desc* d, hipStream_t s, bool vec, const vfm_gemm_desc* tail, int form);
bool vfm_gemm_ps_ok(const vfm_gemm_desc* d, int per);
bool vfm_gemm_launch_ps(const vfm_gemm_desc* d, hipStream_t s, const vfm_gemm_desc* tail, int per);
#else
static bool vfm_gemm_launch_v5(const vfm_gemm_desc*, hipStream_t, bool, const vfm_gemm_desc*, int) { return false; }
static bool vfm_gemm_ps_ok(const vfm_gemm_desc*, int) { return false; }
static bool vfm_gemm_launch_ps(const vfm_gemm_desc*, hipStream_t, const vfm_gemm_desc*, int) { return false; }
#endif

int vfm_gemm_bf16_impl(const vfm_gemm_desc* d0, hipStream_t s) {
  const long tail = d0->M % 128;
  const bool bt = (d0->sb_n == 1 && d0->sb_k != 1);
  if (bt) return gemm_main(d0, s);
  const long t128m = (long)((d0->M - tail) / 128) * cdiv(d0->N, 128);
  const bool pp_coarse = !(g_use_pp & 64) && tail > 0 && t128m >= 96 && t128m <= 160 && d0->N >= 512 && d0->K >= 1024 && d0->batch <= 1;
  const bool rows64 = !pp_coarse && d0->N > 32 && d0->K >= 512 && (long)cdiv(d0->M, 128) * cdiv(d0->N, 128) <= 160 &&
                      (long)cdiv(d0->M, 64) * cdiv(d0->N, 64) <= 544;
  if (g_split_tail && !(rows64 && (g_split_tail & 2)) && d0->M > 512 && tail > 0 && tail <= 32 && (d0->batch <= 1)) {
    vfm_gemm_desc dm = *d0, dt = *d0;
    const long mm = d0->M - tail;
    dm.M = mm;
    dt.M = tail;
    auto adv = [&](const void* p, int dt_, long ld) -> const void* {
      return p ? (const void*)((const char*)p + mm * ld * (dt_ == VFM_BF16 || dt_ == VFM_SPLIT3 ? 2 : 4)) : nullptr;
    };
    dt.A = adv(d0->A, VFM_BF16, d0->sa_m);
    dt.C = (void*)adv(d0->C, d0->c_dt, d0->ldc);
    dt.residual = adv(d0->residual, d0->r_dt, d0->ldr);
    dt.aux = adv(d0->aux, d0->aux_dt, d0->ld_aux);
    dt.C2 = (void*)adv(d0->C2, d0->c2_dt, d0->ldc2);
    bool folded = false;
    int rc = gemm_main(&dm, s, g_fold_tail ? &dt : nullptr, &folded);
    if (rc) return rc;
    if (!folded) launch_skinny(&dt, s);
    return VFM_OK;
  }
  if (d0->M <= 32 && d0->N >= 32) {
    launch_skinny(d0, s);
    return VFM_OK;
  }
  return gemm_main(d0, s);
}

static int gemm_main(const vfm_gemm_desc* d, hipStream_t s, const vfm_gemm_desc* tail, bool* folded) {
  const bool vec = vec_ok(d);
  bool fd = false;
  if (d->sb_n == 1 && d->sb_k != 1) {
    if (d->sa_m == 1 && d->sa_k != 1) {
      if (vec) launch_one<128, 128, 2, 4, 2, true, true, true>(d, s);
      else launch_one<128, 128, 2, 4, 2, false, true, true>(d, s);
      return VFM_OK;
    }
    const bool few = (long)cdiv(d->M, 128) * cdiv(d->N, 128) * (d->batch > 0 ? d->batch : 1) < 128;
    if (d->M <= 64 || (g_bt64 && few)) launch_bt<64, 1, 4>(d, s, vec);
    else launch_bt<128, 2, 4>(d, s, vec);
    return VFM_OK;
  }
  int cfg = g_force_cfg;
  if (cfg < 0) {
    const long nbatch = d->batch > 0 ? d->batch : 1;
    const long t128 = (long)cdiv(d->M, 128) * cdiv(d->N, 128) * (g_batch_tiles ? nbatch : 1);
    const long t256 = (long)cdiv(d->M, 256) * cdiv(d->N, 256);
    const bool span31 = (d->M + 128) * d->sa_m < (1l << 31) && (d->N + 128) * d->sb_n < (1l << 31);
    const bool span33 = (d->M + 256) * d->sa_m < (1l << 31) && (d->N + 256) * d->sb_n < (1l << 31);
    const long t192 = (long)cdiv(d->M, 192) * cdiv(d->N, 256);
    const double eff192 = (double)t192 / (256.0 * cdiv(t192, 256)), eff256 = (double)t256 / (256.0 * cdiv(t256, 256));
    const bool big_m = d->M >= 8192 && d->N >= 1024 && d->K >= 1024 && nbatch == 1 && span33 && !(g_use_pp & 64);
    if (d->N <= 32) cfg = 10;
    else if ((g_use_192 & 1) && big_m && eff192 >= eff256 + 0.08)
      cfg = 40;
    else if ((g_use_192 & 2) && big_m && d->N >= 2048 && t256 > 256 && eff256 >= 0.8 && eff256 < 0.9)
      cfg = 33;
    else if ((g_use_ps & 1) && d->N >= 2048 && t256 >= 224 && t256 % 256 == 0 && d->K >= 1024 && vfm_gemm_ps_ok(d, 2))
      cfg = 37;
    else if (!(g_use_pp & 64) && tail && t128 >= 96 && t128 <= 160 && d->N >= 512 && d->K >= 1024 && span31 && nbatch == 1)
      cfg = 31;
    else if (!(g_use_pp & 64) && d->N >= 1024 && d->N < 2048 && t256 >= 128 && t256 <= 200 && span33 && nbatch == 1 &&
             (d->K >= 2048 || (t256 >= 170 && d->K >= 1024)))
      cfg = 33;
    else if (!(g_use_pp & 64) && d->N >= 4096 && t256 >= 700 && t256 < 768 && d->K >= 1024 && span33 && nbatch == 1)
      cfg = 33;
    else if (!(g_use_pp & 64) && d->N >= 2048 && t256 >= 224 && t256 <= 256 && d->K >= 1024 && span33 && nbatch == 1 && !tail)
      cfg = 33;
    else if (t128 <= 160 && d->K >= 512 && (long)cdiv(d->M, 64) * cdiv(d->N, 64) <= 544)
      cfg = 10;
    else if (t128 <= 160) cfg = 18;
    else if ((g_use_pp & 2) && t128 > 160 && t128 <= 272 && d->K >= 256 && (d->M + 128) * d->sa_m < (1l << 31) && (d->N + 128) * d->sb_n < (1l << 31))
      cfg = 31;
    else if ((g_use_pp & 128) && d->N >= 2048 && t256 >= 176 && t256 < 256 && d->K >= 512 && span33 && nbatch == 1)
      cfg = 33;
    else if ((g_use_pp & 16) && d->N >= 2048 && (t256 % 256 == 0 || t256 >= 768) && d->K >= 128 && (d->M + 256) * d->sa_m < (1l << 31) &&
             (d->N + 256) * d->sb_n < (1l << 31))
      cfg = 33;
    else if (d->N >= 2048 && (t256 % 256 == 0 || t256 >= 768) && !(g_use_pp & 8))
      cfg = ((g_use_pp & 1) && d->K >= 128 && (d->M + 256) * d->sa_m < (1l << 31) && (d->N + 256) * d->sb_n < (1l << 31)) ? 30 : 16;
    else cfg = 17;
    if (cfg == 17 && (g_use_pp & 32) && d->K >= 128 && (d->M + 128) * d->sa_m < (1l << 31) && (d->N + 128) * d->sb_n < (1l << 31))
      cfg = 34;
    if (cfg == 34 && g_w44_k > 0 && d->K >= g_w44_k) cfg = 52;
    if (cfg == 34 && !tail && t128 <= 256 && d->K >= 256 && d->M % 128 == 0) cfg = 35;
    if (cfg == 34 && tail && t128 <= 256 && d->M % 128 == 0 && d->K >= g_deep_tail_k && g_deep_tail_k > 0) cfg = 35;
    if (cfg == 34 && tail && t128 <= 256 && d->M % 128 == 0 && d->K >= 256 && g_deep_sep_k > 0 && d->K >= g_deep_sep_k) {
      if (folded) *folded = false;
      vfm_gemm_launch_w4(d, s, vec, nullptr, 3);
      return VFM_OK;
    }
  }
  switch (cfg) {
    case 0: fd = launch_cfg<128, 128, 2, 2, 2>(d, s, vec, tail); break;
    case 1: fd = launch_cfg<128, 128, 2, 2, 3>(d, s, vec, tail); break;
    case 2: fd = launch_cfg<128, 128, 2, 2, 4>(d, s, vec, tail); break;
    case 3: fd = launch_cfg<128, 64, 2, 2, 3>(d, s, vec, tail); break;
    case 4: fd = launch_cfg<128, 64, 2, 2, 4>(d, s, vec, tail); break;
    case 5: fd = launch_cfg<256, 128, 2, 2, 2>(d, s, vec, tail); break;
    case 6: fd = launch_cfg<256, 128, 2, 2, 3>(d, s, vec, tail); break;
    case 7: fd = launch_cfg<256, 128, 4, 2, 3>(d, s, vec, tail); break;
    case 8: fd = launch_cfg<256, 256, 2, 4, 2>(d, s, vec, tail); break;
    case 9: fd = launch_cfg<128, 256, 2, 2, 3>(d, s, vec, tail); break;
    case 10: fd = launch_cfg<64, 64, 2, 2, 4>(d, s, vec, tail); break;
    case 11: fd = launch_cfg<256, 64, 4, 2, 3>(d, s, vec, tail); break;
    case 12: fd = launch_cfg<128, 128, 4, 2, 2>(d, s, vec, tail); break;
    case 13: fd = launch_cfg<128, 128, 4, 2, 3>(d, s, vec, tail); break;
    case 14: fd = launch_cfg<256, 128, 4, 2, 2>(d, s, vec, tail); break;
    case 15: fd = launch_cfg<256, 256, 4, 2, 2>(d, s, vec, tail); break;
    case 16: fd = launch_cfg<256, 256, 4, 4, 2>(d, s, vec, tail); break;
    case 17: fd = launch_cfg<128, 128, 2, 4, 2>(d, s, vec, tail); break;
    case 18: fd = launch_cfg<64, 128, 2, 2, 2>(d, s, vec, tail); break;
    case 19: fd = launch_cfg<128, 64, 2, 2, 2>(d, s, vec, tail); break;
    case 20: fd = launch_cfg<256, 128, 4, 4, 3>(d, s, vec, tail); break;
    case 21: fd = launch_cfg<128, 256, 4, 4, 3>(d, s, vec, tail); break;
    case 22: fd = launch_cfg<256, 128, 4, 4, 2>(d, s, vec, tail); break;
    case 23: fd = launch_cfg<128, 128, 4, 4, 3>(d, s, vec, tail); break;
    case 24: fd = launch_cfg<128, 128, 4, 4, 2>(d, s, vec, tail); break;
    case 25: fd = launch_cfg<64, 128, 2, 2, 4>(d, s, vec, tail); break;
    case 26: fd = launch_cfg<32, 64, 1, 2, 4>(d, s, vec, tail); break;
    case 27: fd = launch_cfg<32, 128, 1, 4, 4>(d, s, vec, tail); break;
    case 28: fd = launch_cfg<64, 64, 2, 2, 6>(d, s, vec, tail); break;
    case 29: fd = launch_cfg<32, 64, 1, 2, 8>(d, s, vec, tail); break;
    case 31:
      VFM_CHECK(d->K >= 256, VFM_E_UNSUPPORTED, "vfm_gemm(bf16): the 128x128 ping-pong kernel needs K >= 256");
      fd = vfm_gemm_launch_pp128(d, s, vec, tail);
      break;
    case 32:
    case 33:
    case 34:
    case 35:
    case 36:
      VFM_CHECK(d->K >= 128 && d->K % 64 == 0 && (d->M + 256) * d->sa_m < (1l << 31) && (d->N + 256) * d->sb_n < (1l << 31), VFM_E_UNSUPPORTED,
                "vfm_gemm(bf16): the 4-wave 256x256 kernel needs K >= 128 and operands spanning < 4 GiB");
      VFM_CHECK(cfg < 35 || d->K >= 256, VFM_E_UNSUPPORTED, "vfm_gemm(bf16): the deep-ring 128x128 kernels need K >= 256");
      fd = vfm_gemm_launch_w4(d, s, vec, tail, cfg == 32 ? 4 : (cfg == 33 ? 8 : (cfg == 34 ? 2 : (cfg == 35 ? 3 : 5))));
      break;
    case 51:
      VFM_CHECK(d->K % 64 == 0 && (d->M + 256) * d->sa_m < (1l << 31) && (d->N + 256) * d->sb_n < (1l << 31) && vfm_gemm_splitk_ok(d, vec), VFM_E_UNSUPPORTED,
                "vfm_gemm(bf16): the split-K ring kernel needs K %% 128 == 0, K >= 512, one batch, <= 512 tiles of 128 x 128, a 16-byte aligned epilogue");
      fd = vfm_gemm_launch_w4_splitk(d, s, tail);
      break;
    case 52:
      VFM_CHECK(d->K >= 128 && d->K % 64 == 0 && (d->M + 256) * d->sa_m < (1l << 31) && (d->N + 256) * d->sb_n < (1l << 31), VFM_E_UNSUPPORTED,
                "vfm_gemm(bf16): the 4-wave 128x128 kernel needs K >= 128 and operands spanning < 4 GiB");
      fd = vfm_gemm_launch_w4(d, s, vec, tail, 9);
      break;
    case 39:
    case 40:
      VFM_CHECK(d->K >= 128 && d->K % 64 == 0 && (d->M + 256) * d->sa_m < (1l << 31) && (d->N + 256) * d->sb_n < (1l << 31), VFM_E_UNSUPPORTED,
                "vfm_gemm(bf16): the 192x256 kernel needs K >= 128 and operands spanning < 4 GiB");
      fd = vfm_gemm_launch_w4(d, s, vec, tail, cfg == 39 ? 6 : 7);
      break;
    case 50:
#ifndef VFM_EXPERIMENTAL_GEMM
      VFM_FAIL(VFM_E_UNSUPPORTED, "vfm_gemm(bf16): config 50 (gemm_v5.hip) is an experiment: build with VFMSEG_EXPERIMENTAL=1");
#endif
      VFM_CHECK(d->K >= 128 && d->K % 64 == 0 && (d->M + 256) * d->sa_m < (1l << 31) && (d->N + 256) * d->sb_n < (1l << 31), VFM_E_UNSUPPORTED,
                "vfm_gemm(bf16): the 16x16x32 256x256 kernel needs K >= 128 and operands spanning < 4 GiB");
      fd = vfm_gemm_launch_v5(d, s, vec, tail, 0);
      break;
    case 37:
    case 38:
      VFM_CHECK(vfm_gemm_ps_ok(d, cfg == 37 ? 2 : 1), VFM_E_UNSUPPORTED,
                "vfm_gemm(bf16): the persistent kernel needs M %% 256 == 0, N %% %d == 0, K %% 64 == 0, K >= 576 and a bf16 bias / GELU / multiply epilogue",
                cfg == 37 ? 256 : 128);
      fd = vfm_gemm_launch_ps(d, s, tail, cfg == 37 ? 2 : 1);
      break;
    case 30:
      VFM_CHECK(d->K >= 128, VFM_E_UNSUPPORTED, "vfm_gemm(bf16): the ping-pong kernel needs K >= 128");
      fd = vfm_gemm_launch_pp256(d, s, vec, tail);
      break;
    default: VFM_FAIL(VFM_E_INVAL, "vfm_gemm(bf16): unknown config %d", cfg);
  }
  if (folded) *folded = fd && tail;
  return VFM_OK;
}
```

vfmseg_amd/csrc/norm.hip:

```cpp
#include "common.h"

__device__ __forceinline__ float act_f(float v, int act) {
  return act == VFM_ACT_GELU ? gelu_f(v) : (act == VFM_ACT_RELU ? fmaxf(v, 0.f) : v);
}
__device__ __forceinline__ float act_grad_f(float v, int act) {
  return act == VFM_ACT_GELU ? gelu_grad_f(v) : (act == VFM_ACT_RELU ? (v > 0.f ? 1.f : 0.f) : 1.f);
}

template <typename TO, int MAXPL>
__global__ void k_ln_fwd(const float* __restrict__ x, long ld_x, const float* __restrict__ w, const float* __restrict__ b,
                         float eps, TO* __restrict__ y, long ld_y, float* __restrict__ stats, long rows, int C) {
  const int lane = threadIdx.x & 63;
  const long row = (long)blockIdx.x * (blockDim.x >> 6) + (threadIdx.x >> 6);
  if (row >= rows) return;
  const float* xr = x + row * ld_x;
  float v[MAXPL];
  float s = 0.f;
#pragma unroll
  for (int i = 0; i < MAXPL; ++i) {
    const int c = i * 64 + lane;
    v[i] = c < C ? xr[c] : 0.f;
    s += v[i];
  }
  const float mean = wave_sum(s) / C;
  float q = 0.f;
#pragma unroll
  for (int i = 0; i < MAXPL; ++i) {
    const int c = i * 64 + lane;
    const float d = c < C ? v[i] - mean : 0.f;
    q += d * d;
  }
  const float rstd = rsqrtf(wave_sum(q) / C + eps);
  if (stats && lane == 0) {
    stats[row * 2] = mean;
    stats[row * 2 + 1] = rstd;
  }
#pragma unroll
  for (int i = 0; i < MAXPL; ++i) {
    const int c = i * 64 + lane;
    if (c < C) st_f32(y + row * ld_y + c, (v[i] - mean) * rstd * w[c] + b[c]);
  }
}


struct LnDrop {
  void* yd; long ld_yd; void* mask; long ld_mask; float p, keep_scale; uint64_t seed, offset;
};
struct Split3Out {
  bf16_t* y3; long ld3; long plane;
};
__device__ __forceinline__ void store_split4(const Split3Out& so, long row, int c0, float4 o) {
  const bf16_t h0 = f32_to_bf16(o.x), h1 = f32_to_bf16(o.y), h2 = f32_to_bf16(o.z), h3 = f32_to_bf16(o.w);
  const ushort4 hi = {h0, h1, h2, h3};
  const ushort4 lo = {f32_to_bf16(o.x - bf16_to_f32(h0)), f32_to_bf16(o.y - bf16_to_f32(h1)), f32_to_bf16(o.z - bf16_to_f32(h2)),
                      f32_to_bf16(o.w - bf16_to_f32(h3))};
  bf16_t* p = so.y3 + row * so.ld3 + c0;
  *reinterpret_cast<ushort4*>(p) = hi;
  *reinterpret_cast<ushort4*>(p + so.plane) = hi;
  *reinterpret_cast<ushort4*>(p + 2 * so.plane) = lo;
}
template <typename TO, int NV, bool DROP = false, bool SPLIT = false>
__global__ void k_ln_fwd_v4(const float* __restrict__ x, long ld_x, const float* __restrict__ w, const float* __restrict__ b,
                            float eps, TO* __restrict__ y, long ld_y, float* __restrict__ stats, long rows, int C, LnDrop dr = LnDrop(),
                            Split3Out so = Split3Out()) {
  const int lane = threadIdx.x & 63;
  const long row = (long)blockIdx.x * (blockDim.x >> 6) + (threadIdx.x >> 6);
  if (row >= rows) return;
  const float* xr = x + row * ld_x;
  float4 v[NV];
  float s = 0.f;
#pragma unroll
  for (int i = 0; i < NV; ++i) {
    v[i] = *reinterpret_cast<const float4*>(xr + (i * 64 + lane) * 4);
    s += (v[i].x + v[i].y) + (v[i].z + v[i].w);
  }
  const float mean = wave_sum(s) / C;
  float q = 0.f;
#pragma unroll
  for (int i = 0; i < NV; ++i) {
    const float a = v[i].x - mean, bb = v[i].y - mean, c = v[i].z - mean, d = v[i].w - mean;
    q += (a * a + bb * bb) + (c * c + d * d);
  }
  const float rstd = rsqrtf(wave_sum(q) / C + eps);
  if (stats && lane == 0) {
    stats[row * 2] = mean;
    stats[row * 2 + 1] = rstd;
  }
#pragma unroll
  for (int i = 0; i < NV; ++i) {
    const int c0 = (i * 64 + lane) * 4;
    const float4 ww = *reinterpret_cast<const float4*>(w + c0);
    const float4 bv = *reinterpret_cast<const float4*>(b + c0);
    float4 o;
    o.x = (v[i].x - mean) * rstd * ww.x + bv.x;
    o.y = (v[i].y - mean) * rstd * ww.y + bv.y;
    o.z = (v[i].z - mean) * rstd * ww.z + bv.z;
    o.w = (v[i].w - mean) * rstd * ww.w + bv.w;
    if constexpr (sizeof(TO) == 2) {
      ushort4 p = {f32_to_bf16(o.x), f32_to_bf16(o.y), f32_to_bf16(o.z), f32_to_bf16(o.w)};
      *reinterpret_cast<ushort4*>(y + row * ld_y + c0) = p;
      if constexpr (DROP) {
        const uint64_t e0 = dr.offset + (uint64_t)row * C + c0;
        const bf16_t ks = f32_to_bf16(dr.keep_scale);
        const float ksf = bf16_to_f32(ks);
        ushort4 mk, yd;
        const bool k0 = (hash_u32(dr.seed, e0) >> 8) * (1.0f / 16777216.0f) >= dr.p;
        const bool k1 = (hash_u32(dr.seed, e0 + 1) >> 8) * (1.0f / 16777216.0f) >= dr.p;
        const bool k2 = (hash_u32(dr.seed, e0 + 2) >> 8) * (1.0f / 16777216.0f) >= dr.p;
        const bool k3 = (hash_u32(dr.seed, e0 + 3) >> 8) * (1.0f / 16777216.0f) >= dr.p;
        mk.x = k0 ? ks : 0, mk.y = k1 ? ks : 0, mk.z = k2 ? ks : 0, mk.w = k3 ? ks : 0;
        yd.x = k0 ? f32_to_bf16(bf16_to_f32(p.x) * ksf) : f32_to_bf16(bf16_to_f32(p.x) * 0.f);
        yd.y = k1 ? f32_to_bf16(bf16_to_f32(p.y) * ksf) : f32_to_bf16(bf16_to_f32(p.y) * 0.f);
        yd.z = k2 ? f32_to_bf16(bf16_to_f32(p.z) * ksf) : f32_to_bf16(bf16_to_f32(p.z) * 0.f);
        yd.w = k3 ? f32_to_bf16(bf16_to_f32(p.w) * ksf) : f32_to_bf16(bf16_to_f32(p.w) * 0.f);
        *reinterpret_cast<ushort4*>((bf16_t*)dr.mask + row * dr.ld_mask + c0) = mk;
        *reinterpret_cast<ushort4*>((bf16_t*)dr.yd + row * dr.ld_yd + c0) = yd;
      }
    } else {
      if (!SPLIT || y != nullptr) *reinterpret_cast<float4*>(y + row * ld_y + c0) = o;
      if constexpr (SPLIT) store_split4(so, row, c0, o);
    }
  }
}

template <typename TD, int NV>
__global__ void k_ln_bwd_v4(const TD* __restrict__ dy, long ld_dy, const float* __restrict__ x, long ld_x,
                            const float* __restrict__ w, const float* __restrict__ stats, float* __restrict__ dx, long ld_dx,
                            int accumulate_dx, long rows, int C, bf16_t* __restrict__ t_out = nullptr, long ld_t = 0,
                            const float* __restrict__ t_scale = nullptr) {
  const int lane = threadIdx.x & 63;
  const long row = (long)blockIdx.x * (blockDim.x >> 6) + (threadIdx.x >> 6);
  if (row >= rows) return;
  const float mean = stats[row * 2], rstd = stats[row * 2 + 1];
  float4 g[NV], xh[NV];
  float s1 = 0.f, s2 = 0.f;
#pragma unroll
  for (int i = 0; i < NV; ++i) {
    const int c0 = (i * 64 + lane) * 4;
    float4 d;
    if constexpr (sizeof(TD) == 2) {
      const ushort4 p = *reinterpret_cast<const ushort4*>(dy + row * ld_dy + c0);
      d = make_float4(bf16_to_f32(p.x), bf16_to_f32(p.y), bf16_to_f32(p.z), bf16_to_f32(p.w));
    } else {
      d = *reinterpret_cast<const float4*>(dy + row * ld_dy + c0);
    }
    const float4 xv = *reinterpret_cast<const float4*>(x + row * ld_x + c0);
    const float4 ww = *reinterpret_cast<const float4*>(w + c0);
    xh[i] = make_float4((xv.x - mean) * rstd, (xv.y - mean) * rstd, (xv.z - mean) * rstd, (xv.w - mean) * rstd);
    g[i] = make_float4(d.x * ww.x, d.y * ww.y, d.z * ww.z, d.w * ww.w);
    s1 += (g[i].x + g[i].y) + (g[i].z + g[i].w);
    s2 += (g[i].x * xh[i].x + g[i].y * xh[i].y) + (g[i].z * xh[i].z + g[i].w * xh[i].w);
  }
  s1 = wave_sum(s1) / C;
  s2 = wave_sum(s2) / C;
#pragma unroll
  for (int i = 0; i < NV; ++i) {
    const int c0 = (i * 64 + lane) * 4;
    float4 o = make_float4(rstd * (g[i].x - s1 - xh[i].x * s2), rstd * (g[i].y - s1 - xh[i].y * s2),
                           rstd * (g[i].z - s1 - xh[i].z * s2), rstd * (g[i].w - s1 - xh[i].w * s2));
    float4* p = reinterpret_cast<float4*>(dx + row * ld_dx + c0);
    if (accumulate_dx) {
      const float4 old = *p;
      o.x += old.x, o.y += old.y, o.z += old.z, o.w += old.w;
    }
    *p = o;
    if (t_out) {
      const float4 ts = *reinterpret_cast<const float4*>(t_scale + c0);
      const ushort4 tv = {f32_to_bf16(o.x * ts.x), f32_to_bf16(o.y * ts.y), f32_to_bf16(o.z * ts.z), f32_to_bf16(o.w * ts.w)};
      *reinterpret_cast<ushort4*>(t_out + row * ld_t + c0) = tv;
    }
  }
}

template <typename TO, int MAXP2>
__global__ void k_ln_fwd_v2(const float* __restrict__ x, long ld_x, const float* __restrict__ w, const float* __restrict__ b, float eps,
                            TO* __restrict__ y, long ld_y, float* __restrict__ stats, long rows, int C) {
  const int lane = threadIdx.x & 63;
  const long row = (long)blockIdx.x * (blockDim.x >> 6) + (threadIdx.x >> 6);
  if (row >= rows) return;
  const float* xr = x + row * ld_x;
  float2 v[MAXP2];
  float s = 0.f;
#pragma unroll
  for (int i = 0; i < MAXP2; ++i) {
    const int c = (i * 64 + lane) * 2;
    v[i] = c < C ? *reinterpret_cast<const float2*>(xr + c) : make_float2(0.f, 0.f);
    s += v[i].x + v[i].y;
  }
  const float mean = wave_sum(s) / C;
  float q = 0.f;
#pragma unroll
  for (int i = 0; i < MAXP2; ++i) {
    const int c = (i * 64 + lane) * 2;
    if (c < C) {
      const float a = v[i].x - mean, bb = v[i].y - mean;
      q += a * a + bb * bb;
    }
  }
  const float rstd = rsqrtf(wave_sum(q) / C + eps);
  if (stats && lane == 0) {
    stats[row * 2] = mean;
    stats[row * 2 + 1] = rstd;
  }
#pragma unroll
  for (int i = 0; i < MAXP2; ++i) {
    const int c = (i * 64 + lane) * 2;
    if (c < C) {
      const float2 ww = *reinterpret_cast<const float2*>(w + c), bv = *reinterpret_cast<const float2*>(b + c);
      const float o0 = (v[i].x - mean) * rstd * ww.x + bv.x, o1 = (v[i].y - mean) * rstd * ww.y + bv.y;
      if constexpr (sizeof(TO) == 2) {
        const ushort2 pk = {f32_to_bf16(o0), f32_to_bf16(o1)};
        *reinterpret_cast<ushort2*>(y + row * ld_y + c) = pk;
      } else {
        *reinterpret_cast<float2*>(y + row * ld_y + c) = make_float2(o0, o1);
      }
    }
  }
}

template <typename TO, int MAXP4>
__global__ void k_ln_fwd_v4t(const float* __restrict__ x, long ld_x, const float* __restrict__ w, const float* __restrict__ b, float eps,
                             TO* __restrict__ y, long ld_y, float* __restrict__ stats, long rows, int C) {
  const int lane = threadIdx.x & 63;
  const long row = (long)blockIdx.x * (blockDim.x >> 6) + (threadIdx.x >> 6);
  if (row >= rows) return;
  const float* xr = x + row * ld_x;
  float v[MAXP4][4];
  float s = 0.f;
#pragma unroll
  for (int i = 0; i < MAXP4; ++i) {
    const int c = (i * 64 + lane) * 4;
    const float4 t = c < C ? *reinterpret_cast<const float4*>(xr + c) : make_float4(0.f, 0.f, 0.f, 0.f);
    v[i][0] = t.x, v[i][1] = t.y, v[i][2] = t.z, v[i][3] = t.w;
#pragma unroll
    for (int e = 0; e < 4; ++e)
      if (c + e < C) s += v[i][e];
  }
  const float mean = wave_sum(s) / C;
  float q = 0.f;
#pragma unroll
  for (int i = 0; i < MAXP4; ++i) {
    const int c = (i * 64 + lane) * 4;
#pragma unroll
    for (int e = 0; e < 4; ++e)
      if (c + e < C) q += (v[i][e] - mean) * (v[i][e] - mean);
  }
  const float rstd = rsqrtf(wave_sum(q) / C + eps);
  if (stats && lane == 0) {
    stats[row * 2] = mean;
    stats[row * 2 + 1] = rstd;
  }
#pragma unroll
  for (int i = 0; i < MAXP4; ++i) {
    const int c = (i * 64 + lane) * 4;
    if (c < C) {
      if (c + 4 <= C) {
        const float4 ww = *reinterpret_cast<const float4*>(w + c), bv = *reinterpret_cast<const float4*>(b + c);
        const float o0 = (v[i][0] - mean) * rstd * ww.x + bv.x, o1 = (v[i][1] - mean) * rstd * ww.y + bv.y;
        const float o2 = (v[i][2] - mean) * rstd * ww.z + bv.z, o3 = (v[i][3] - mean) * rstd * ww.w + bv.w;
        if constexpr (sizeof(TO) == 2) {
          const ushort4 pk = {f32_to_bf16(o0), f32_to_bf16(o1), f32_to_bf16(o2), f32_to_bf16(o3)};
          *reinterpret_cast<ushort4*>(y + row * ld_y + c) = pk;
        } else {
          *reinterpret_cast<float4*>(y + row * ld_y + c) = make_float4(o0, o1, o2, o3);
        }
      } else {
#pragma unroll
        for (int e = 0; e < 4; ++e)
          if (c + e < C) {
            const float o = (v[i][e] - mean) * rstd * w[c + e] + b[c + e];
            if constexpr (sizeof(TO) == 2) y[row * ld_y + c + e] = f32_to_bf16(o);
            else y[row * ld_y + c + e] = o;
          }
      }
    }
  }
}

extern "C" int vfm_layernorm_fwd_split3(const float* x, long ld_x, const float* w, const float* b, float eps, float* y, long ld_y, void* y3,
                                        long ld3, long plane, float* stats, long rows, long C, void* stream) {
  const int nv = (int)(C / 256);
  VFM_CHECK(C > 0 && C % 256 == 0 && (nv == 1 || nv == 2 || nv == 4 || nv == 5 || nv == 8) && ld_x >= C && ld_x % 4 == 0 && (uintptr_t)x % 16 == 0 &&
                (uintptr_t)w % 16 == 0 && (uintptr_t)b % 16 == 0,
            VFM_E_SHAPE, "vfm_layernorm_fwd_split3: C=%ld must be 256, 512, 1024, 1280 or 2048 with 16-byte aligned rows", C);
  VFM_CHECK(y3 && (uintptr_t)y3 % 8 == 0 && plane >= C && plane % 4 == 0 && ld3 >= 3 * plane && ld3 % 4 == 0 && (!y || (ld_y >= C && ld_y % 4 == 0 && (uintptr_t)y % 16 == 0)),
            VFM_E_ALIGN, "vfm_layernorm_fwd_split3: y3 [rows, >= 3 plane] bf16 with plane >= C, 8-byte aligned; y (optional fp32 copy) 16-byte aligned");
  if (rows == 0) return VFM_OK;
  hipStream_t s = (hipStream_t)stream;
  dim3 grid(cdiv(rows, 4)), blk(256);
  Split3Out so;
  so.y3 = (bf16_t*)y3, so.ld3 = ld3, so.plane = plane;
#define LVS(NV) hipLaunchKernelGGL((k_ln_fwd_v4<float, NV, false, true>), grid, blk, 0, s, x, ld_x, w, b, eps, y, ld_y, stats, rows, (int)C, LnDrop(), so)
  if (nv == 1) LVS(1); else if (nv == 2) LVS(2); else if (nv == 4) LVS(4); else if (nv == 5) LVS(5); else LVS(8);
#undef LVS
  VFM_LAUNCH_CHECK();
  return VFM_OK;
}

extern "C" int vfm_layernorm_fwd(const float* x, long ld_x, const float* w, const float* b, float eps, void* y, int y_dt,
                                 long ld_y, float* stats, long rows, long C, void* stream) {
  VFM_CHECK(C > 0 && C <= 3072 && ld_x >= C && ld_y >= C, VFM_E_SHAPE, "vfm_layernorm_fwd: C=%ld unsupported", C);
  if (rows == 0) return VFM_OK;
  hipStream_t s = (hipStream_t)stream;
  dim3 grid(cdiv(rows, 4)), blk(256);
  const int nvq = (int)(C / 256);
  const bool v4 = (C % 256 == 0) && (nvq == 1 || nvq == 2 || nvq == 4 || nvq == 5 || nvq == 8) && (ld_x % 4 == 0) && (ld_y % 4 == 0) && ((uintptr_t)x % 16 == 0) &&
                  ((uintptr_t)y % 8 == 0) && ((uintptr_t)w % 16 == 0) && ((uintptr_t)b % 16 == 0);
  if (v4) {
#define LV(TO, NV) hipLaunchKernelGGL((k_ln_fwd_v4<TO, NV>), grid, blk, 0, s, x, ld_x, w, b, eps, (TO*)y, ld_y, stats, rows, (int)C)
    const int nv = (int)(C / 256);
    if (y_dt == VFM_BF16) { if (nv == 1) LV(bf16_t, 1); else if (nv == 4) LV(bf16_t, 4); else if (nv == 5) LV(bf16_t, 5); else if (nv == 2) LV(bf16_t, 2); else LV(bf16_t, 8); }
    else if (y_dt == VFM_F32) { if (nv == 1) LV(float, 1); else if (nv == 4) LV(float, 4); else if (nv == 5) LV(float, 5); else if (nv == 2) LV(float, 2); else LV(float, 8); }
    else VFM_FAIL(VFM_E_INVAL, "vfm_layernorm_fwd: dtype");
#undef LV
    if (!(nv == 1 || nv == 2 || nv == 4 || nv == 5 || nv == 8)) VFM_FAIL(VFM_E_SHAPE, "vfm_layernorm_fwd: C=%ld", C);
    VFM_LAUNCH_CHECK();
    return VFM_OK;
  }
  if (C > 1024 && C <= 2816 && ld_x % 4 == 0 && ld_y % 4 == 0 && ld_x >= (C + 3) / 4 * 4 && ld_y >= (C + 3) / 4 * 4 && (uintptr_t)x % 16 == 0 &&
      (uintptr_t)y % 16 == 0 && (uintptr_t)w % 16 == 0 && (uintptr_t)b % 16 == 0) {
    if (y_dt == VFM_BF16) hipLaunchKernelGGL((k_ln_fwd_v4t<bf16_t, 11>), grid, blk, 0, s, x, ld_x, w, b, eps, (bf16_t*)y, ld_y, stats, rows, (int)C);
    else if (y_dt == VFM_F32) hipLaunchKernelGGL((k_ln_fwd_v4t<float, 11>), grid, blk, 0, s, x, ld_x, w, b, eps, (float*)y, ld_y, stats, rows, (int)C);
    else VFM_FAIL(VFM_E_INVAL, "vfm_layernorm_fwd: dtype");
    VFM_LAUNCH_CHECK();
    return VFM_OK;
  }
  if (C > 1024 && C % 2 == 0 && ld_x % 2 == 0 && ld_y % 2 == 0 && (uintptr_t)x % 8 == 0 && (uintptr_t)y % 8 == 0 && (uintptr_t)w % 8 == 0 &&
      (uintptr_t)b % 8 == 0) {
    if (y_dt == VFM_BF16) hipLaunchKernelGGL((k_ln_fwd_v2<bf16_t, 24>), grid, blk, 0, s, x, ld_x, w, b, eps, (bf16_t*)y, ld_y, stats, rows, (int)C);
    else if (y_dt == VFM_F32) hipLaunchKernelGGL((k_ln_fwd_v2<float, 24>), grid, blk, 0, s, x, ld_x, w, b, eps, (float*)y, ld_y, stats, rows, (int)C);
    else VFM_FAIL(VFM_E_INVAL, "vfm_layernorm_fwd: dtype");
    VFM_LAUNCH_CHECK();
    return VFM_OK;
  }
#define L(TO, PL) hipLaunchKernelGGL((k_ln_fwd<TO, PL>), grid, blk, 0, s, x, ld_x, w, b, eps, (TO*)y, ld_y, stats, rows, (int)C)
  const int pl = (int)((C + 63) / 64);
  if (y_dt == VFM_BF16) { if (pl <= 4) L(bf16_t, 4); else if (pl <= 16) L(bf16_t, 16); else if (pl <= 32) L(bf16_t, 32); else L(bf16_t, 48); }
  else if (y_dt == VFM_F32) { if (pl <= 4) L(float, 4); else if (pl <= 16) L(float, 16); else if (pl <= 32) L(float, 32); else L(float, 48); }
  else VFM_FAIL(VFM_E_INVAL, "vfm_layernorm_fwd: dtype");
#undef L
  VFM_LAUNCH_CHECK();
  return VFM_OK;
}

extern "C" int vfm_layernorm_dropout_fwd(const float* x, long ld_x, const float* w, const float* b, float eps, void* y, long ld_y,
                                         float* stats, void* y_drop, long ld_yd, void* mask, long ld_mask, float p, uint64_t seed,
                                         uint64_t offset, long rows, long C, void* stream) {
  VFM_CHECK(p >= 0.f && p < 1.f, VFM_E_INVAL, "vfm_layernorm_dropout_fwd: p");
  const long nv = C / 256;
  VFM_CHECK(C % 256 == 0 && (nv == 1 || nv == 2 || nv == 4 || nv == 5 || nv == 8), VFM_E_SHAPE, "vfm_layernorm_dropout_fwd: C=%ld", C);
  VFM_CHECK(ld_x % 4 == 0 && ld_y % 4 == 0 && ld_yd % 4 == 0 && ld_mask % 4 == 0 && (uintptr_t)x % 16 == 0 && (uintptr_t)y % 8 == 0 &&
                (uintptr_t)y_drop % 8 == 0 && (uintptr_t)mask % 8 == 0 && (uintptr_t)w % 16 == 0 && (uintptr_t)b % 16 == 0,
            VFM_E_ALIGN, "vfm_layernorm_dropout_fwd: alignment");
  if (rows == 0) return VFM_OK;
  hipStream_t s = (hipStream_t)stream;
  dim3 blk(256), grid(cdiv(rows, 4));
  LnDrop dr{y_drop, ld_yd, mask, ld_mask, p, 1.0f / (1.0f - p), seed, offset};
#define LVD(NV) hipLaunchKernelGGL((k_ln_fwd_v4<bf16_t, NV, true>), grid, blk, 0, s, x, ld_x, w, b, eps, (bf16_t*)y, ld_y, stats, rows, (int)C, dr)
  if (nv == 1) LVD(1); else if (nv == 2) LVD(2); else if (nv == 4) LVD(4); else if (nv == 5) LVD(5); else LVD(8);
#undef LVD
  VFM_LAUNCH_CHECK();
  return VFM_OK;
}

template <typename TD, int MAXPL, bool NEED_W>
__global__ void k_ln_bwd(const TD* __restrict__ dy, long ld_dy, const float* __restrict__ x, long ld_x,
                         const float* __restrict__ w, const float* __restrict__ stats, float* __restrict__ dx, long ld_dx,
                         int accumulate_dx, float* __restrict__ ws, long rows, int C) {
  const int lane = threadIdx.x & 63, wv = threadIdx.x >> 6, nw = blockDim.x >> 6;
  float pdw[NEED_W ? MAXPL : 1], pdb[NEED_W ? MAXPL : 1];
#pragma unroll
  for (int i = 0; i < (NEED_W ? MAXPL : 1); ++i) pdw[i] = pdb[i] = 0.f;
  for (long row = (long)blockIdx.x * nw + wv; row < rows; row += (long)gridDim.x * nw) {
    const float mean = stats[row * 2], rstd = stats[row * 2 + 1];
    float g[MAXPL], xh[MAXPL];
    float s1 = 0.f, s2 = 0.f;
#pragma unroll
    for (int i = 0; i < MAXPL; ++i) {
      const int c = i * 64 + lane;
      if (c < C) {
        const float d = ld_f32(dy + row * ld_dy + c);
        xh[i] = (x[row * ld_x + c] - mean) * rstd;
        g[i] = d * w[c];
        s1 += g[i];
        s2 += g[i] * xh[i];
        if constexpr (NEED_W) {
          pdw[i] += d * xh[i];
          pdb[i] += d;
        }
      } else {
        g[i] = xh[i] = 0.f;
      }
    }
    s1 = wave_sum(s1) / C;
    s2 = wave_sum(s2) / C;
#pragma unroll
    for (int i = 0; i < MAXPL; ++i) {
      const int c = i * 64 + lane;
      if (c < C) {
        const float v = rstd * (g[i] - s1 - xh[i] * s2);
        float* p = dx + row * ld_dx + c;
        *p = accumulate_dx ? *p + v : v;
      }
    }
  }
  if constexpr (NEED_W) {
    extern __shared__ float sh[];
#pragma unroll
    for (int i = 0; i < MAXPL; ++i) {
      const int c = i * 64 + lane;
      if (c < C) {
        sh[(wv * 2 + 0) * C + c] = pdw[i];
        sh[(wv * 2 + 1) * C + c] = pdb[i];
      }
    }
    __syncthreads();
    for (int c = threadIdx.x; c < 2 * C; c += blockDim.x) {
      const int which = c / C, cc = c - which * C;
      float a = 0.f;
      for (int k = 0; k < nw; ++k) a += sh[(k * 2 + which) * C + cc];
      ws[((long)blockIdx.x * 2 + which) * C + cc] = a;
    }
  }
}
__global__ void k_ln_bwd_fin(const float* __restrict__ ws, int parts, int C, float* __restrict__ dw, float* __restrict__ db) {
  __shared__ float sh[2][4][64];
  const int tx = threadIdx.x & 63, ty = threadIdx.x >> 6;
  const int c = blockIdx.x * 64 + tx;
  float a = 0.f, b = 0.f;
  if (c < C) {
#pragma unroll 8
    for (int p = ty; p < parts; p += 4) {
      a += ws[((long)p * 2 + 0) * C + c];
      b += ws[((long)p * 2 + 1) * C + c];
    }
  }
  sh[0][ty][tx] = a, sh[1][ty][tx] = b;
  __syncthreads();
  if (ty == 0 && c < C) {
    if (dw) dw[c] += (sh[0][0][tx] + sh[0][1][tx]) + (sh[0][2][tx] + sh[0][3][tx]);
    if (db) db[c] += (sh[1][0][tx] + sh[1][1][tx]) + (sh[1][2][tx] + sh[1][3][tx]);
  }
}

template <typename TD, int MAXP4>
__global__ void k_ln_bwd_v4t(const TD* __restrict__ dy, long ld_dy, const float* __restrict__ x, long ld_x, const float* __restrict__ w,
                             const float* __restrict__ stats, float* __restrict__ dx, long ld_dx, int accumulate_dx, long rows, int C) {
  const int lane = threadIdx.x & 63;
  const long row = (long)blockIdx.x * (blockDim.x >> 6) + (threadIdx.x >> 6);
  if (row >= rows) return;
  const float mean = stats[row * 2], rstd = stats[row * 2 + 1];
  float g[MAXP4][4], xh[MAXP4][4];
  float s1 = 0.f, s2 = 0.f;
#pragma unroll
  for (int i = 0; i < MAXP4; ++i) {
    const int c = (i * 64 + lane) * 4;
#pragma unroll
    for (int e = 0; e < 4; ++e) g[i][e] = xh[i][e] = 0.f;
    if (c < C) {
      float d[4];
      if constexpr (sizeof(TD) == 2) {
        const ushort4 pp = *reinterpret_cast<const ushort4*>(dy + row * ld_dy + c);
        d[0] = bf16_to_f32(pp.x), d[1] = bf16_to_f32(pp.y), d[2] = bf16_to_f32(pp.z), d[3] = bf16_to_f32(pp.w);
      } else {
        const float4 t = *reinterpret_cast<const float4*>(dy + row * ld_dy + c);
        d[0] = t.x, d[1] = t.y, d[2] = t.z, d[3] = t.w;
      }
      const float4 xv4 = *reinterpret_cast<const float4*>(x + row * ld_x + c);
      const float xv[4] = {xv4.x, xv4.y, xv4.z, xv4.w};
      float wv[4] = {0.f, 0.f, 0.f, 0.f};
      if (c + 4 <= C) {
        const float4 ww = *reinterpret_cast<const float4*>(w + c);
        wv[0] = ww.x, wv[1] = ww.y, wv[2] = ww.z, wv[3] = ww.w;
      } else {
#pragma unroll
        for (int e = 0; e < 4; ++e)
          if (c + e < C) wv[e] = w[c + e];
      }
#pragma unroll
      for (int e = 0; e < 4; ++e)
        if (c + e < C) {
          xh[i][e] = (xv[e] - mean) * rstd;
          g[i][e] = d[e] * wv[e];
          s1 += g[i][e];
          s2 += g[i][e] * xh[i][e];
        }
    }
  }
  s1 = wave_sum(s1) / C;
  s2 = wave_sum(s2) / C;
#pragma unroll
  for (int i = 0; i < MAXP4; ++i) {
    const int c = (i * 64 + lane) * 4;
    if (c < C) {
      float o[4];
#pragma unroll
      for (int e = 0; e < 4; ++e) o[e] = rstd * (g[i][e] - s1 - xh[i][e] * s2);
      if (c + 4 <= C) {
        float4* pp = reinterpret_cast<float4*>(dx + row * ld_dx + c);
        if (accumulate_dx) {
          const float4 old = *pp;
          o[0] += old.x, o[1] += old.y, o[2] += old.z, o[3] += old.w;
        }
        *pp = make_float4(o[0], o[1], o[2], o[3]);
      } else {
#pragma unroll
        for (int e = 0; e < 4; ++e)
          if (c + e < C) dx[row * ld_dx + c + e] = accumulate_dx ? dx[row * ld_dx + c + e] + o[e] : o[e];
      }
    }
  }
}

static int ln_bwd_impl(const void* dy, int dy_dt, long ld_dy, const float* x, long ld_x, const float* w, const float* stats,
                       float* dx, long ld_dx, int accumulate_dx, float* dw, float* db, float* ws, long rows, long C, void* t_out,
                       long ld_t, const float* t_scale, void* stream);
extern "C" int vfm_layernorm_bwd(const void* dy, int dy_dt, long ld_dy, const float* x, long ld_x, const float* w,
                                 const float* stats, float* dx, long ld_dx, int accumulate_dx, float* dw, float* db,
                                 float* ws, long rows, long C, void* stream) {
  return ln_bwd_impl(dy, dy_dt, ld_dy, x, ld_x, w, stats, dx, ld_dx, accumulate_dx, dw, db, ws, rows, C, nullptr, 0, nullptr, stream);
}
extern "C" int vfm_layernorm_bwd_scaled(const void* dy, int dy_dt, long ld_dy, const float* x, long ld_x, const float* w,
                                        const float* stats, float* dx, long ld_dx, int accumulate_dx, void* t_out, long ld_t,
                                        const float* t_scale, long rows, long C, void* stream) {
  VFM_CHECK(t_out && t_scale && ld_t % 4 == 0 && (uintptr_t)t_out % 8 == 0 && (uintptr_t)t_scale % 16 == 0, VFM_E_INVAL,
            "vfm_layernorm_bwd_scaled: t_out / t_scale");
  return ln_bwd_impl(dy, dy_dt, ld_dy, x, ld_x, w, stats, dx, ld_dx, accumulate_dx, nullptr, nullptr, nullptr, rows, C, t_out, ld_t,
                     t_scale, stream);
}
template <typename TD, int MAXP2>
__global__ void k_ln_bwd_v2(const TD* __restrict__ dy, long ld_dy, const float* __restrict__ x, long ld_x, const float* __restrict__ w,
                            const float* __restrict__ stats, float* __restrict__ dx, long ld_dx, int accumulate_dx, long rows, int C) {
  const int lane = threadIdx.x & 63;
  const long row = (long)blockIdx.x * (blockDim.x >> 6) + (threadIdx.x >> 6);
  if (row >= rows) return;
  const float mean = stats[row * 2], rstd = stats[row * 2 + 1];
  float2 g[MAXP2], xh[MAXP2];
  float s1 = 0.f, s2 = 0.f;
#pragma unroll
  for (int i = 0; i < MAXP2; ++i) {
    const int c = (i * 64 + lane) * 2;
    g[i] = xh[i] = make_float2(0.f, 0.f);
    if (c < C) {
      float2 d;
      if constexpr (sizeof(TD) == 2) {
        const ushort2 pp = *reinterpret_cast<const ushort2*>(dy + row * ld_dy + c);
        d = make_float2(bf16_to_f32(pp.x), bf16_to_f32(pp.y));
      } else {
        d = *reinterpret_cast<const float2*>(dy + row * ld_dy + c);
      }
      const float2 xv = *reinterpret_cast<const float2*>(x + row * ld_x + c);
      const float2 ww = *reinterpret_cast<const float2*>(w + c);
      xh[i] = make_float2((xv.x - mean) * rstd, (xv.y - mean) * rstd);
      g[i] = make_float2(d.x * ww.x, d.y * ww.y);
      s1 += g[i].x + g[i].y;
      s2 += g[i].x * xh[i].x + g[i].y * xh[i].y;
    }
  }
  s1 = wave_sum(s1) / C;
  s2 = wave_sum(s2) / C;
#pragma unroll
  for (int i = 0; i < MAXP2; ++i) {
    const int c = (i * 64 + lane) * 2;
    if (c < C) {
      float2 o = make_float2(rstd * (g[i].x - s1 - xh[i].x * s2), rstd * (g[i].y - s1 - xh[i].y * s2));
      float2* pp = reinterpret_cast<float2*>(dx + row * ld_dx + c);
      if (accumulate_dx) {
        const float2 old = *pp;
        o.x += old.x, o.y += old.y;
      }
      *pp = o;
    }
  }
}

static int ln_bwd_impl(const void* dy, int dy_dt, long ld_dy, const float* x, long ld_x, const float* w, const float* stats,
                       float* dx, long ld_dx, int accumulate_dx, float* dw, float* db, float* ws, long rows, long C, void* t_out,
                       long ld_t, const float* t_scale, void* stream) {
  VFM_CHECK(C > 0 && (C <= 1024 || (C <= 3072 && !(dw || db))), VFM_E_SHAPE, "vfm_layernorm_bwd: C=%ld unsupported", C);
  VFM_CHECK(!(dw || db) || ws, VFM_E_INVAL, "vfm_layernorm_bwd: ws required for dw/db");
  if (rows == 0) return VFM_OK;
  hipStream_t s = (hipStream_t)stream;
  const bool need_w = (dw || db);
  const int nv = (int)(C / 256);
  const bool v4 = !need_w && (C % 256 == 0) && (nv == 1 || nv == 2 || nv == 4 || nv == 5) && (ld_x % 4 == 0) && (ld_dx % 4 == 0) &&
                  (ld_dy % 4 == 0) && ((uintptr_t)x % 16 == 0) && ((uintptr_t)dx % 16 == 0) && ((uintptr_t)dy % 8 == 0) &&
                  ((uintptr_t)w % 16 == 0);
  if (v4) {
    dim3 grid(cdiv(rows, 4)), blk(256);
#define LV(TD, NV) hipLaunchKernelGGL((k_ln_bwd_v4<TD, NV>), grid, blk, 0, s, (const TD*)dy, ld_dy, x, ld_x, w, stats, dx, ld_dx, accumulate_dx, rows, (int)C, (bf16_t*)t_out, ld_t, t_scale)
    if (dy_dt == VFM_BF16) { if (nv == 1) LV(bf16_t, 1); else if (nv == 2) LV(bf16_t, 2); else if (nv == 4) LV(bf16_t, 4); else LV(bf16_t, 5); }
    else if (dy_dt == VFM_F32) { if (nv == 1) LV(float, 1); else if (nv == 2) LV(float, 2); else if (nv == 4) LV(float, 4); else LV(float, 5); }
    else VFM_FAIL(VFM_E_INVAL, "vfm_layernorm_bwd: dtype");
#undef LV
    VFM_LAUNCH_CHECK();
    return VFM_OK;
  }
  VFM_CHECK(!t_out, VFM_E_UNSUPPORTED, "vfm_layernorm_bwd_scaled: needs the vectorised path (C %% 256 == 0, aligned operands, no dw/db)");
  {
    const long cp = (C + 3) / 4 * 4;
    if (!need_w && C > 1024 && C <= 2816 && ld_x % 4 == 0 && ld_dx % 4 == 0 && ld_dy % 4 == 0 && ld_x >= cp && ld_dx >= cp && ld_dy >= cp &&
        (uintptr_t)x % 16 == 0 && (uintptr_t)dx % 16 == 0 && (uintptr_t)dy % 16 == 0 && (uintptr_t)w % 16 == 0) {
      dim3 grid(cdiv(rows, 4)), blk(256);
      if (dy_dt == VFM_BF16)
        hipLaunchKernelGGL((k_ln_bwd_v4t<bf16_t, 11>), grid, blk, 0, s, (const bf16_t*)dy, ld_dy, x, ld_x, w, stats, dx, ld_dx, accumulate_dx, rows, (int)C);
      else if (dy_dt == VFM_F32)
        hipLaunchKernelGGL((k_ln_bwd_v4t<float, 11>), grid, blk, 0, s, (const float*)dy, ld_dy, x, ld_x, w, stats, dx, ld_dx, accumulate_dx, rows, (int)C);
      else VFM_FAIL(VFM_E_INVAL, "vfm_layernorm_bwd: dtype");
      VFM_LAUNCH_CHECK();
      return VFM_OK;
    }
  }
  if (!need_w && C > 1024 && C % 2 == 0 && ld_x % 2 == 0 && ld_dx % 2 == 0 && ld_dy % 2 == 0 && (uintptr_t)x % 8 == 0 &&
      (uintptr_t)dx % 8 == 0 && (uintptr_t)dy % 8 == 0 && (uintptr_t)w % 8 == 0) {
    dim3 grid(cdiv(rows, 4)), blk(256);
    if (dy_dt == VFM_BF16)
      hipLaunchKernelGGL((k_ln_bwd_v2<bf16_t, 24>), grid, blk, 0, s, (const bf16_t*)dy, ld_dy, x, ld_x, w, stats, dx, ld_dx, accumulate_dx, rows, (int)C);
    else if (dy_dt == VFM_F32)
      hipLaunchKernelGGL((k_ln_bwd_v2<float, 24>), grid, blk, 0, s, (const float*)dy, ld_dy, x, ld_x, w, stats, dx, ld_dx, accumulate_dx, rows, (int)C);
    else VFM_FAIL(VFM_E_INVAL, "vfm_layernorm_bwd: dtype");
    VFM_LAUNCH_CHECK();
    return VFM_OK;
  }
  const int parts = need_w ? 128 : cdiv(rows, 4);
  const size_t shm = need_w ? (size_t)4 * 2 * C * sizeof(float) : 0;
  float* wsp = need_w ? ws : nullptr;
#define L(TD, PL, NW) hipLaunchKernelGGL((k_ln_bwd<TD, PL, NW>), dim3(parts), dim3(256), shm, s, (const TD*)dy, ld_dy, x, ld_x, w, stats, dx, ld_dx, accumulate_dx, wsp, rows, (int)C)
  const int pl = (int)((C + 63) / 64);
  if (need_w) {
    if (dy_dt == VFM_BF16) { if (pl <= 4) L(bf16_t, 4, true); else L(bf16_t, 16, true); }
    else if (dy_dt == VFM_F32) { if (pl <= 4) L(float, 4, true); else L(float, 16, true); }
    else VFM_FAIL(VFM_E_INVAL, "vfm_layernorm_bwd: dtype");
  } else {
    if (dy_dt == VFM_BF16) { if (pl <= 4) L(bf16_t, 4, false); else if (pl <= 16) L(bf16_t, 16, false); else L(bf16_t, 48, false); }
    else if (dy_dt == VFM_F32) { if (pl <= 4) L(float, 4, false); else if (pl <= 16) L(float, 16, false); else L(float, 48, false); }
    else VFM_FAIL(VFM_E_INVAL, "vfm_layernorm_bwd: dtype");
  }
#undef L
  if (need_w) hipLaunchKernelGGL(k_ln_bwd_fin, dim3(cdiv(C, 64)), dim3(256), 0, s, ws, parts, (int)C, dw, db);
  VFM_LAUNCH_CHECK();
  return VFM_OK;
}

template <int MODE, typename TD>
__global__ void k_chan_moments(const float* __restrict__ x, const TD* __restrict__ dy, const float* __restrict__ w,
                               const float* __restrict__ bb, const float* __restrict__ stats, int G, float eps, int act,
                               float* __restrict__ ws, long P, int C, int rows_per_chunk) {
  __shared__ float sh[2][4][64];
  const int tx = threadIdx.x & 63, ty = threadIdx.x >> 6;
  const int c = blockIdx.x * 64 + tx;
  const long b = blockIdx.z;
  const long r0 = (long)blockIdx.y * rows_per_chunk;
  long r1 = r0 + rows_per_chunk;
  if (r1 > P) r1 = P;
  float a1 = 0.f, a2 = 0.f;
  if (c < C) {
    float mean = 0.f, rstd = 1.f, wc = 1.f, bc = 0.f;
    if (MODE == 1) {
      if (G > 0) {
        const int g = c / (C / G);
        mean = stats[(b * G + g) * 2];
        rstd = stats[(b * G + g) * 2 + 1];
      } else {
        mean = stats[c];
        rstd = rsqrtf(stats[C + c] + eps);
      }
      wc = w[c];
      bc = bb[c];
    }
    const float* xp = x + (b * P) * C + c;
    for (long r = r0 + ty; r < r1; r += 4) {
      const float xv = xp[r * C];
      if (MODE == 0) {
        a1 += xv;
        a2 += xv * xv;
      } else {
        const float xh = (xv - mean) * rstd;
        float d = ld_f32(dy + (b * P + r) * C + c);
        if (act != VFM_ACT_NONE) d *= act_grad_f(xh * wc + bc, act);
        a1 += d;
        a2 += d * xh;
      }
    }
  }
  sh[0][ty][tx] = a1;
  sh[1][ty][tx] = a2;
  __syncthreads();
  if (ty == 0 && c < C) {
    const long slot = b * gridDim.y + blockIdx.y;
    ws[(slot * 2 + 0) * C + c] = sh[0][0][tx] + sh[0][1][tx] + sh[0][2][tx] + sh[0][3][tx];
    ws[(slot * 2 + 1) * C + c] = sh[1][0][tx] + sh[1][1][tx] + sh[1][2][tx] + sh[1][3][tx];
  }
}

static inline int pick_chunks(long P) {
  int n = (int)((P + 63) / 64);
  if (n > 64) n = 64;
  if (n < 1) n = 1;
  return n;
}

__device__ __forceinline__ double wave_sum_f64(double v) {
#pragma unroll
  for (int o = 32; o > 0; o >>= 1) v += __shfl_xor(v, o, 64);
  return v;
}
__global__ void k_gn_fin_fwd(const float* __restrict__ ws, int nchunk, int C, int G, long P, float eps,
                             float* __restrict__ stats, int BG) {
  const int i = blockIdx.x * (blockDim.x >> 6) + (threadIdx.x >> 6), lane = threadIdx.x & 63;
  if (i >= BG) return;
  const int b = i / G, g = i - b * G, cg = C / G;
  double s = 0.0, q = 0.0;
  for (int e = lane; e < nchunk * cg; e += 64) {
    const int k = e / cg, j = e - k * cg;
    const long slot = (long)b * nchunk + k;
    s += ws[(slot * 2 + 0) * C + g * cg + j];
    q += ws[(slot * 2 + 1) * C + g * cg + j];
  }
  s = wave_sum_f64(s), q = wave_sum_f64(q);
  if (lane) return;
  const double n = (double)P * cg;
  const double mean = s / n;
  double var = q / n - mean * mean;
  if (var < 0) var = 0;
  stats[i * 2] = (float)mean;
  stats[i * 2 + 1] = (float)(1.0 / sqrt(var + (double)eps));
}
template <typename TO>
__global__ void k_gn_apply(const float* __restrict__ x, const float* __restrict__ w, const float* __restrict__ b,
                           const float* __restrict__ stats, int G, int act, TO* __restrict__ y, long B, long P, int C) {
  const long total = B * P * C;
  const int cg = C / G;
  for (long i = blockIdx.x * (long)blockDim.x + threadIdx.x; i < total; i += (long)gridDim.x * blockDim.x) {
    const int c = (int)(i % C);
    const long bi = i / ((long)P * C);
    const int g = c / cg;
    const float mean = stats[(bi * G + g) * 2], rstd = stats[(bi * G + g) * 2 + 1];
    st_f32(y + i, act_f((x[i] - mean) * rstd * w[c] + b[c], act));
  }
}
extern "C" int vfm_groupnorm_fwd(const float* x, const float* w, const float* b, float eps, int G, int act, void* y, int y_dt,
                                 float* stats, float* ws_in, long B, long P, long C, void* stream) {
  VFM_CHECK(G > 0 && C % G == 0 && ws_in, VFM_E_SHAPE, "vfm_groupnorm_fwd: C %% G / ws");
  if (B * P * C == 0) return VFM_OK;
  hipStream_t s = (hipStream_t)stream;
  const int nchunk = pick_chunks(P);
  const int rpc = (int)((P + nchunk - 1) / nchunk);
  float* ws = ws_in + B * G * 2;
  hipLaunchKernelGGL((k_chan_moments<0, float>), dim3(cdiv(C, 64), nchunk, (unsigned)B), dim3(256), 0, s, x, (const float*)nullptr,
                     (const float*)nullptr, (const float*)nullptr, (const float*)nullptr, 0, 0.f, 0, ws, P, (int)C, rpc);
  hipLaunchKernelGGL(k_gn_fin_fwd, dim3(cdiv(B * G, 4)), dim3(256), 0, s, ws, nchunk, (int)C, G, P, eps, stats, (int)(B * G));
  const long total = B * P * C;
  const int grid = (int)((total + 255) / 256 > 8192 ? 8192 : (total + 255) / 256);
  if (y_dt == VFM_BF16) hipLaunchKernelGGL(k_gn_apply<bf16_t>, dim3(grid), dim3(256), 0, s, x, w, b, stats, G, act, (bf16_t*)y, B, P, (int)C);
  else if (y_dt == VFM_F32) hipLaunchKernelGGL(k_gn_apply<float>, dim3(grid), dim3(256), 0, s, x, w, b, stats, G, act, (float*)y, B, P, (int)C);
  else VFM_FAIL(VFM_E_INVAL, "vfm_groupnorm_fwd: dtype");
  VFM_LAUNCH_CHECK();
  return VFM_OK;
}

__global__ void k_gn_fin_bwd(const float* __restrict__ ws, int nchunk, int C, int G, const float* __restrict__ w,
                             float* __restrict__ gs, int BG) {
  const int i = blockIdx.x * (blockDim.x >> 6) + (threadIdx.x >> 6), lane = threadIdx.x & 63;
  if (i >= BG) return;
  const int b = i / G, g = i - b * G, cg = C / G;
  double s1 = 0.0, s2 = 0.0;
  for (int e = lane; e < nchunk * cg; e += 64) {
    const int k = e / cg, j = e - k * cg;
    const long slot = (long)b * nchunk + k;
    const int c = g * cg + j;
    s1 += (double)w[c] * ws[(slot * 2 + 0) * C + c];
    s2 += (double)w[c] * ws[(slot * 2 + 1) * C + c];
  }
  s1 = wave_sum_f64(s1), s2 = wave_sum_f64(s2);
  if (lane) return;
  gs[i * 2] = (float)s1;
  gs[i * 2 + 1] = (float)s2;
}
__global__ void k_chan_fin_wb(const float* __restrict__ ws, int slots, int C, float* __restrict__ dw, float* __restrict__ db) {
  __shared__ float sh[2][4][64];
  const int tx = threadIdx.x & 63, ty = threadIdx.x >> 6;
  const int c = blockIdx.x * 64 + tx;
  float a = 0.f, b = 0.f;
  if (c < C) {
#pragma unroll 8
    for (int k = ty; k < slots; k += 4) {
      b += ws[((long)k * 2 + 0) * C + c];
      a += ws[((long)k * 2 + 1) * C + c];
    }
  }
  sh[0][ty][tx] = a, sh[1][ty][tx] = b;
  __syncthreads();
  if (ty == 0 && c < C) {
    if (dw) dw[c] += (sh[0][0][tx] + sh[0][1][tx]) + (sh[0][2][tx] + sh[0][3][tx]);
    if (db) db[c] += (sh[1][0][tx] + sh[1][1][tx]) + (sh[1][2][tx] + sh[1][3][tx]);
  }
}
template <typename TD>
__global__ void k_gn_bwd_apply(const TD* __restrict__ dy, const float* __restrict__ x, const float* __restrict__ w,
                               const float* __restrict__ b, const float* __restrict__ stats, const float* __restrict__ gs,
                               int G, int act, float* __restrict__ dx, long B, long P, int C) {
  const long total = B * P * C;
  const int cg = C / G;
  const float inv_n = 1.0f / ((float)P * cg);
  for (long i = blockIdx.x * (long)blockDim.x + threadIdx.x; i < total; i += (long)gridDim.x * blockDim.x) {
    const int c = (int)(i % C);
    const long bi = i / ((long)P * C);
    const int g = c / cg;
    const float mean = stats[(bi * G + g) * 2], rstd = stats[(bi * G + g) * 2 + 1];
    const float xh = (x[i] - mean) * rstd;
    float d = ld_f32(dy + i);
    if (act != VFM_ACT_NONE) d *= act_grad_f(xh * w[c] + b[c], act);
    dx[i] = rstd * (d * w[c] - (gs[(bi * G + g) * 2] + xh * gs[(bi * G + g) * 2 + 1]) * inv_n);
  }
}
extern "C" int vfm_groupnorm_bwd(const void* dy, int dy_dt, const float* x, const float* w, const float* b,
                                 const float* stats, int G, int act, float* dx, float* dw, float* db, float* ws, long B,
                                 long P, long C, void* stream) {
  VFM_CHECK(G > 0 && C % G == 0 && ws, VFM_E_SHAPE, "vfm_groupnorm_bwd: args");
  if (B * P * C == 0) return VFM_OK;
  hipStream_t s = (hipStream_t)stream;
  const int nchunk = pick_chunks(P);
  const int rpc = (int)((P + nchunk - 1) / nchunk);
  float* gs = ws;
  float* part = ws + B * G * 2;
  dim3 grid(cdiv(C, 64), nchunk, (unsigned)B);
  if (dy_dt == VFM_BF16)
    hipLaunchKernelGGL((k_chan_moments<1, bf16_t>), grid, dim3(256), 0, s, x, (const bf16_t*)dy, w, b, stats, G, 0.f, act, part, P, (int)C, rpc);
  else if (dy_dt == VFM_F32)
    hipLaunchKernelGGL((k_chan_moments<1, float>), grid, dim3(256), 0, s, x, (const float*)dy, w, b, stats, G, 0.f, act, part, P, (int)C, rpc);
  else VFM_FAIL(VFM_E_INVAL, "vfm_groupnorm_bwd: dtype");
  hipLaunchKernelGGL(k_gn_fin_bwd, dim3(cdiv(B * G, 4)), dim3(256), 0, s, part, nchunk, (int)C, G, w, gs, (int)(B * G));
  if (dw || db) hipLaunchKernelGGL(k_chan_fin_wb, dim3(cdiv(C, 64)), dim3(256), 0, s, part, (int)(B * nchunk), (int)C, dw, db);
  const long total = B * P * C;
  const int g2 = (int)((total + 255) / 256 > 8192 ? 8192 : (total + 255) / 256);
  if (dy_dt == VFM_BF16) hipLaunchKernelGGL(k_gn_bwd_apply<bf16_t>, dim3(g2), dim3(256), 0, s, (const bf16_t*)dy, x, w, b, stats, gs, G, act, dx, B, P, (int)C);
  else hipLaunchKernelGGL(k_gn_bwd_apply<float>, dim3(g2), dim3(256), 0, s, (const float*)dy, x, w, b, stats, gs, G, act, dx, B, P, (int)C);
  VFM_LAUNCH_CHECK();
  return VFM_OK;
}

#define GNT_THREADS 512
#define GNT_SLAB 32
#define GNT_ROWS 64
#define GNT_STEPS 16
static inline bool gn_tile_covers(long P, long C, int G) {
  if (G <= 0 || C <= 0 || P <= 0 || C % G) return false;
  const long cg = C / G;
  return (cg == 4 || cg == 8 || cg == 16 || cg == 32) && C % GNT_SLAB == 0 && P <= (long)GNT_ROWS * GNT_STEPS;
}
extern "C" int vfm_groupnorm_tile_ok(long P, long C, int G) { return gn_tile_covers(P, C, G) ? 1 : 0; }

__device__ __forceinline__ float gnt_group_sum(float v, int qpg, float (*sh)[8]) {
  v += __shfl_xor(v, 8, 64);
  v += __shfl_xor(v, 16, 64);
  v += __shfl_xor(v, 32, 64);
  for (int o = 1; o < qpg; o <<= 1) v += __shfl_xor(v, o, 64);
  const int lane = threadIdx.x & 63;
  if (lane < 8) sh[threadIdx.x >> 6][lane] = v;
  __syncthreads();
  float r = 0.f;
#pragma unroll
  for (int k = 0; k < GNT_THREADS / 64; ++k) r += sh[k][lane & 7];
  return r;
}
__device__ __forceinline__ void gnt_store4(float* p, float a, float b, float c, float d) { *reinterpret_cast<float4*>(p) = make_float4(a, b, c, d); }
__device__ __forceinline__ void gnt_store4(bf16_t* p, float a, float b, float c, float d) {
  uint2 o;
  o.x = (uint32_t)f32_to_bf16(a) | ((uint32_t)f32_to_bf16(b) << 16);
  o.y = (uint32_t)f32_to_bf16(c) | ((uint32_t)f32_to_bf16(d) << 16);
  *reinterpret_cast<uint2*>(p) = o;
}
__device__ __forceinline__ float4 gnt_load4(const float* p) { return *reinterpret_cast<const float4*>(p); }
__device__ __forceinline__ float4 gnt_load4(const bf16_t* p) {
  const uint2 o = *reinterpret_cast<const uint2*>(p);
  return make_float4(h16_lo(o.x), h16_hi(o.x), h16_lo(o.y), h16_hi(o.y));
}

template <typename TO>
__global__ void __launch_bounds__(GNT_THREADS) k_gn_tile_fwd(const float* __restrict__ x, const float* __restrict__ w, const float* __restrict__ b,
                                                             float eps, int G, int act, TO* __restrict__ y, float* __restrict__ stats, int P, int C) {
  __shared__ float sh[2][GNT_THREADS / 64][8];
  const int lane = threadIdx.x & 63, q = lane & 7, row0 = (threadIdx.x >> 6) * 8 + (lane >> 3);
  const int c0 = blockIdx.x * GNT_SLAB + q * 4, cg = C / G, qpg = cg >> 2;
  const long base = (long)blockIdx.y * P * C + c0;
  float4 v[GNT_STEPS];
#pragma unroll
  for (int k = 0; k < GNT_STEPS; ++k) {
    const int r = k * GNT_ROWS + row0;
    v[k] = r < P ? gnt_load4(x + base + (long)r * C) : make_float4(0.f, 0.f, 0.f, 0.f);
  }
  float s = 0.f;
#pragma unroll
  for (int k = 0; k < GNT_STEPS; ++k) s += (v[k].x + v[k].y) + (v[k].z + v[k].w);
  const float inv_n = 1.0f / ((float)P * (float)cg);
  const float mean = gnt_group_sum(s, qpg, sh[0]) * inv_n;
  float d = 0.f;
#pragma unroll
  for (int k = 0; k < GNT_STEPS; ++k) {
    if (k * GNT_ROWS + row0 < P) {
      const float a0 = v[k].x - mean, a1 = v[k].y - mean, a2 = v[k].z - mean, a3 = v[k].w - mean;
      d += (a0 * a0 + a1 * a1) + (a2 * a2 + a3 * a3);
    }
  }
  const float rstd = 1.0f / sqrtf(gnt_group_sum(d, qpg, sh[1]) * inv_n + eps);
  if (threadIdx.x < 8 && q % qpg == 0) {
    const long i = (long)blockIdx.y * G + c0 / cg;
    stats[i * 2] = mean;
    stats[i * 2 + 1] = rstd;
  }
  const float4 wv = gnt_load4(w + c0), bv = gnt_load4(b + c0);
#pragma unroll
  for (int k = 0; k < GNT_STEPS; ++k) {
    const int r = k * GNT_ROWS + row0;
    if (r < P)
      gnt_store4(y + base + (long)r * C, act_f((v[k].x - mean) * rstd * wv.x + bv.x, act), act_f((v[k].y - mean) * rstd * wv.y + bv.y, act),
                 act_f((v[k].z - mean) * rstd * wv.z + bv.z, act), act_f((v[k].w - mean) * rstd * wv.w + bv.w, act));
  }
}
extern "C" int vfm_groupnorm_tile_fwd(const float* x, const float* w, const float* b, float eps, int G, int act, void* y, int y_dt,
                                      float* stats, long B, long P, long C, void* stream) {
  VFM_CHECK(gn_tile_covers(P, C, G) && B > 0 && B <= 65535, VFM_E_SHAPE, "vfm_groupnorm_tile_fwd: (P %ld, C %ld, G %d) is outside the tile kernel's coverage", P, C, G);
  VFM_CHECK(act == VFM_ACT_NONE || act == VFM_ACT_RELU, VFM_E_UNSUPPORTED, "vfm_groupnorm_tile_fwd: activation");
  hipStream_t s = (hipStream_t)stream;
  const dim3 grid((unsigned)(C / GNT_SLAB), (unsigned)B);
  if (y_dt == VFM_BF16) hipLaunchKernelGGL(k_gn_tile_fwd<bf16_t>, grid, dim3(GNT_THREADS), 0, s, x, w, b, eps, G, act, (bf16_t*)y, stats, (int)P, (int)C);
  else if (y_dt == VFM_F32) hipLaunchKernelGGL(k_gn_tile_fwd<float>, grid, dim3(GNT_THREADS), 0, s, x, w, b, eps, G, act, (float*)y, stats, (int)P, (int)C);
  else VFM_FAIL(VFM_E_INVAL, "vfm_groupnorm_tile_fwd: dtype");
  VFM_LAUNCH_CHECK();
  return VFM_OK;
}

template <typename TD>
__global__ void __launch_bounds__(GNT_THREADS) k_gn_tile_bwd(const TD* __restrict__ dy, const float* __restrict__ x, const float* __restrict__ w,
                                                             const float* __restrict__ b, const float* __restrict__ stats, int G, int act,
                                                             float* __restrict__ dx, float* __restrict__ part, int P, int C) {
  __shared__ float sh[2][GNT_THREADS / 64][8];
  __shared__ float shc[GNT_THREADS / 64][2][GNT_SLAB];
  const int lane = threadIdx.x & 63, q = lane & 7, wave = threadIdx.x >> 6, row0 = wave * 8 + (lane >> 3);
  const int c0 = blockIdx.x * GNT_SLAB + q * 4, cg = C / G, qpg = cg >> 2;
  const long base = (long)blockIdx.y * P * C + c0;
  float4 v[GNT_STEPS], d[GNT_STEPS];
#pragma unroll
  for (int k = 0; k < GNT_STEPS; ++k) {
    const int r = k * GNT_ROWS + row0;
    v[k] = r < P ? gnt_load4(x + base + (long)r * C) : make_float4(0.f, 0.f, 0.f, 0.f);
    d[k] = r < P ? gnt_load4(dy + base + (long)r * C) : make_float4(0.f, 0.f, 0.f, 0.f);
  }
  const long gi = (long)blockIdx.y * G + c0 / cg;
  const float mean = stats[gi * 2], rstd = stats[gi * 2 + 1];
  const float4 wv = gnt_load4(w + c0), bv = gnt_load4(b + c0);
  float4 a1 = make_float4(0.f, 0.f, 0.f, 0.f), a2 = a1;
#pragma unroll
  for (int k = 0; k < GNT_STEPS; ++k) {
    if (k * GNT_ROWS + row0 < P) {
#define GNT_ELEM(m)                                                   \
  {                                                                   \
    const float xh = (v[k].m - mean) * rstd;                          \
    float dz = d[k].m;                                                \
    if (act != VFM_ACT_NONE) dz *= act_grad_f(xh * wv.m + bv.m, act); \
    v[k].m = xh, d[k].m = dz;                                         \
    a1.m += dz, a2.m += dz * xh;                                      \
  }
      GNT_ELEM(x) GNT_ELEM(y) GNT_ELEM(z) GNT_ELEM(w)
#undef GNT_ELEM
    }
  }
  const float s1 = gnt_group_sum((wv.x * a1.x + wv.y * a1.y) + (wv.z * a1.z + wv.w * a1.w), qpg, sh[0]);
  const float s2 = gnt_group_sum((wv.x * a2.x + wv.y * a2.y) + (wv.z * a2.z + wv.w * a2.w), qpg, sh[1]);
#pragma unroll
  for (int o = 8; o < 64; o <<= 1) {
    a1.x += __shfl_xor(a1.x, o, 64), a1.y += __shfl_xor(a1.y, o, 64), a1.z += __shfl_xor(a1.z, o, 64), a1.w += __shfl_xor(a1.w, o, 64);
    a2.x += __shfl_xor(a2.x, o, 64), a2.y += __shfl_xor(a2.y, o, 64), a2.z += __shfl_xor(a2.z, o, 64), a2.w += __shfl_xor(a2.w, o, 64);
  }
  if (lane < 8) {
    *reinterpret_cast<float4*>(&shc[wave][0][q * 4]) = a1;
    *reinterpret_cast<float4*>(&shc[wave][1][q * 4]) = a2;
  }
  __syncthreads();
  if (threadIdx.x < 2 * GNT_SLAB) {
    const int kind = threadIdx.x >> 5, c = threadIdx.x & 31;
    float r = 0.f;
#pragma unroll
    for (int k = 0; k < GNT_THREADS / 64; ++k) r += shc[k][kind][c];
    part[((long)blockIdx.y * 2 + kind) * C + blockIdx.x * GNT_SLAB + c] = r;
  }
  const float inv_n = 1.0f / ((float)P * (float)cg);
#pragma unroll
  for (int k = 0; k < GNT_STEPS; ++k) {
    const int r = k * GNT_ROWS + row0;
    if (r < P)
      gnt_store4(dx + base + (long)r * C, rstd * (d[k].x * wv.x - (s1 + v[k].x * s2) * inv_n), rstd * (d[k].y * wv.y - (s1 + v[k].y * s2) * inv_n),
                 rstd * (d[k].z * wv.z - (s1 + v[k].z * s2) * inv_n), rstd * (d[k].w * wv.w - (s1 + v[k].w * s2) * inv_n));
  }
}
extern "C" int vfm_groupnorm_tile_bwd(const void* dy, int dy_dt, const float* x, const float* w, const float* b, const float* stats,
                                      int G, int act, float* dx, float* dw, float* db, float* ws, long B, long P, long C, void* stream) {
  VFM_CHECK(gn_tile_covers(P, C, G) && B > 0 && B <= 65535, VFM_E_SHAPE, "vfm_groupnorm_tile_bwd: (P %ld, C %ld, G %d) is outside the tile kernel's coverage", P, C, G);
  VFM_CHECK(act == VFM_ACT_NONE || act == VFM_ACT_RELU, VFM_E_UNSUPPORTED, "vfm_groupnorm_tile_bwd: activation");
  VFM_CHECK(ws, VFM_E_INVAL, "vfm_groupnorm_tile_bwd: ws");
  hipStream_t s = (hipStream_t)stream;
  const dim3 grid((unsigned)(C / GNT_SLAB), (unsigned)B);
  if (dy_dt == VFM_BF16) hipLaunchKernelGGL(k_gn_tile_bwd<bf16_t>, grid, dim3(GNT_THREADS), 0, s, (const bf16_t*)dy, x, w, b, stats, G, act, dx, ws, (int)P, (int)C);
  else if (dy_dt == VFM_F32) hipLaunchKernelGGL(k_gn_tile_bwd<float>, grid, dim3(GNT_THREADS), 0, s, (const float*)dy, x, w, b, stats, G, act, dx, ws, (int)P, (int)C);
  else VFM_FAIL(VFM_E_INVAL, "vfm_groupnorm_tile_bwd: dtype");
  if (dw || db) hipLaunchKernelGGL(k_chan_fin_wb, dim3(cdiv(C, 64)), dim3(256), 0, s, ws, (int)B, (int)C, dw, db);
  VFM_LAUNCH_CHECK();
  return VFM_OK;
}

__global__ void __launch_bounds__(256) k_bn_fin_sums(const float* __restrict__ ws, int slots, int C, float* __restrict__ sums) {
  __shared__ double sh[2][4][64];
  const int tx = threadIdx.x & 63, ty = threadIdx.x >> 6;
  const int c = blockIdx.x * 64 + tx;
  double a = 0.0, b = 0.0;
  if (c < C) {
#pragma unroll 8
    for (int k = ty; k < slots; k += 4) {
      a += ws[((long)k * 2 + 0) * C + c];
      b += ws[((long)k * 2 + 1) * C + c];
    }
  }
  sh[0][ty][tx] = a, sh[1][ty][tx] = b;
  __syncthreads();
  if (ty == 0 && c < C) {
    sums[c] = (float)((sh[0][0][tx] + sh[0][1][tx]) + (sh[0][2][tx] + sh[0][3][tx]));
    sums[C + c] = (float)((sh[1][0][tx] + sh[1][1][tx]) + (sh[1][2][tx] + sh[1][3][tx]));
  }
}
extern "C" int vfm_bn_moments(const float* x, long rows, long C, float* sums, float* ws, void* stream) {
  VFM_CHECK(ws && sums, VFM_E_INVAL, "vfm_bn_moments: args");
  hipStream_t s = (hipStream_t)stream;
  const int nchunk = pick_chunks(rows);
  const int rpc = (int)((rows + nchunk - 1) / nchunk);
  hipLaunchKernelGGL((k_chan_moments<0, float>), dim3(cdiv(C, 64), nchunk, 1), dim3(256), 0, s, x, (const float*)nullptr,
                     (const float*)nullptr, (const float*)nullptr, (const float*)nullptr, 0, 0.f, 0, ws, rows, (int)C, rpc);
  hipLaunchKernelGGL(k_bn_fin_sums, dim3(cdiv(C, 64)), dim3(256), 0, s, ws, nchunk, (int)C, sums);
  VFM_LAUNCH_CHECK();
  return VFM_OK;
}
__global__ void k_bn_finalize(const float* __restrict__ sums, float count, float* __restrict__ mean_var,
                              float* __restrict__ rmean, float* __restrict__ rvar, float momentum, int C) {
  const int c = blockIdx.x * blockDim.x + threadIdx.x;
  if (c >= C) return;
  const double mean = (double)sums[c] / count;
  double var = (double)sums[C + c] / count - mean * mean;
  if (var < 0) var = 0;
  mean_var[c] = (float)mean;
  mean_var[C + c] = (float)var;
  if (rmean) rmean[c] = (1.f - momentum) * rmean[c] + momentum * (float)mean;
  if (rvar) rvar[c] = (1.f - momentum) * rvar[c] + momentum * (float)(var * (count / fmaxf(count - 1.f, 1.f)));
}
extern "C" int vfm_bn_finalize(const float* sums, float count, float* mean_var, float* running_mean, float* running_var,
                               float momentum, long C, void* stream) {
  hipLaunchKernelGGL(k_bn_finalize, dim3(cdiv(C, 256)), dim3(256), 0, (hipStream_t)stream, sums, count, mean_var, running_mean,
                     running_var, momentum, (int)C);
  VFM_LAUNCH_CHECK();
  return VFM_OK;
}
template <typename TO>
__global__ void k_bn_apply(const float* __restrict__ x, const float* __restrict__ mv, const float* __restrict__ w,
                           const float* __restrict__ b, float eps, int act, TO* __restrict__ y, long rows, int C) {
  const long total = rows * C;
  for (long i = blockIdx.x * (long)blockDim.x + threadIdx.x; i < total; i += (long)gridDim.x * blockDim.x) {
    const int c = (int)(i % C);
    st_f32(y + i, act_f((x[i] - mv[c]) * rsqrtf(mv[C + c] + eps) * w[c] + b[c], act));
  }
}
extern "C" int vfm_bn_apply(const float* x, const float* mean_var, const float* w, const float* b, float eps, int act, void* y,
                            int y_dt, long rows, long C, void* stream) {
  const long total = rows * C;
  if (total == 0) return VFM_OK;
  const int grid = (int)((total + 255) / 256 > 8192 ? 8192 : (total + 255) / 256);
  hipStream_t s = (hipStream_t)stream;
  if (y_dt == VFM_BF16) hipLaunchKernelGGL(k_bn_apply<bf16_t>, dim3(grid), dim3(256), 0, s, x, mean_var, w, b, eps, act, (bf16_t*)y, rows, (int)C);
  else if (y_dt == VFM_F32) hipLaunchKernelGGL(k_bn_apply<float>, dim3(grid), dim3(256), 0, s, x, mean_var, w, b, eps, act, (float*)y, rows, (int)C);
  else VFM_FAIL(VFM_E_INVAL, "vfm_bn_apply: dtype");
  VFM_LAUNCH_CHECK();
  return VFM_OK;
}
extern "C" int vfm_bn_bwd_reduce(const void* dy, int dy_dt, const float* x, const float* mean_var, const float* w,
                                 const float* b, float eps, int act, float* sums_dy, float* ws, long rows, long C,
                                 void* stream) {
  VFM_CHECK(ws && sums_dy, VFM_E_INVAL, "vfm_bn_bwd_reduce: args");
  hipStream_t s = (hipStream_t)stream;
  const int nchunk = pick_chunks(rows);
  const int rpc = (int)((rows + nchunk - 1) / nchunk);
  dim3 grid(cdiv(C, 64), nchunk, 1);
  if (dy_dt == VFM_BF16)
    hipLaunchKernelGGL((k_chan_moments<1, bf16_t>), grid, dim3(256), 0, s, x, (const bf16_t*)dy, w, b, mean_var, 0, eps, act, ws, rows, (int)C, rpc);
  else if (dy_dt == VFM_F32)
    hipLaunchKernelGGL((k_chan_moments<1, float>), grid, dim3(256), 0, s, x, (const float*)dy, w, b, mean_var, 0, eps, act, ws, rows, (int)C, rpc);
  else VFM_FAIL(VFM_E_INVAL, "vfm_bn_bwd_reduce: dtype");
  hipLaunchKernelGGL(k_bn_fin_sums, dim3(cdiv(C, 64)), dim3(256), 0, s, ws, nchunk, (int)C, sums_dy);
  VFM_LAUNCH_CHECK();
  return VFM_OK;
}
template <typename TD>
__global__ void k_bn_bwd_apply(const TD* __restrict__ dy, const float* __restrict__ x, const float* __restrict__ mv,
                               const float* __restrict__ w, const float* __restrict__ b, float eps, int act,
                               const float* __restrict__ sums, float inv_n, float* __restrict__ dx, long rows, int C) {
  const long total = rows * C;
  for (long i = blockIdx.x * (long)blockDim.x + threadIdx.x; i < total; i += (long)gridDim.x * blockDim.x) {
    const int c = (int)(i % C);
    const float rstd = rsqrtf(mv[C + c] + eps);
    const float xh = (x[i] - mv[c]) * rstd;
    float d = ld_f32(dy + i);
    if (act != VFM_ACT_NONE) d *= act_grad_f(xh * w[c] + b[c], act);
    dx[i] = rstd * w[c] * (d - (sums[c] + xh * sums[C + c]) * inv_n);
  }
}
extern "C" int vfm_bn_bwd_apply(const void* dy, int dy_dt, const float* x, const float* mean_var, const float* w,
                                const float* b, float eps, int act, const float* sums_dy, float total_rows, float* dx,
                                long rows, long C, void* stream) {
  const long total = rows * C;
  if (total == 0) return VFM_OK;
  const int grid = (int)((total + 255) / 256 > 8192 ? 8192 : (total + 255) / 256);
  hipStream_t s = (hipStream_t)stream;
  const float inv_n = 1.0f / total_rows;
  if (dy_dt == VFM_BF16) hipLaunchKernelGGL(k_bn_bwd_apply<bf16_t>, dim3(grid), dim3(256), 0, s, (const bf16_t*)dy, x, mean_var, w, b, eps, act, sums_dy, inv_n, dx, rows, (int)C);
  else if (dy_dt == VFM_F32) hipLaunchKernelGGL(k_bn_bwd_apply<float>, dim3(grid), dim3(256), 0, s, (const float*)dy, x, mean_var, w, b, eps, act, sums_dy, inv_n, dx, rows, (int)C);
  else VFM_FAIL(VFM_E_INVAL, "vfm_bn_bwd_apply: dtype");
  VFM_LAUNCH_CHECK();
  return VFM_OK;
}
```

Before: 128.9 images/s.

## Fold reduction finisher kernels into producer via last-block atomic ticket

Adds a last-block-done pattern: producer blocks write partials with coherent stores, take an atomic ticket on a per-stream counter, and the final block runs the finishing reduction in place of a separate finish kernel. It is applied to the attention CLS finish in the dK/dV backward and, behind flags, to colsum, layernorm backward and channel-moment reductions. The aim is to remove small follow-up kernel launches and their serialization gaps. The cost is extra atomics, a vmcnt wait and barrier in every block, and tail work done by one block. Only the attention CLS fold is enabled by default.

```diff
diff --git a/vfmseg_amd/csrc/attention_bf16.hip b/vfmseg_amd/csrc/attention_bf16.hip
--- a/vfmseg_amd/csrc/attention_bf16.hip
+++ b/vfmseg_amd/csrc/attention_bf16.hip
@@ -1,4 +1,5 @@
 #include "attn_bf16_dev.h"
+#include "fold_fin.h"
 
 template <bool DQ, int NW = 4>
 __global__ void __launch_bounds__(NW * 64, 2) k_attn_bf16_q(AttnP p) {
@@ -259,6 +260,36 @@
 #pragma unroll
     for (int j = 0; j < 2; ++j) store_block_rows(oacc[j], mult, out + qrow * ldo + col0 + 32 * j, h);
   }
+}
+
+struct ClsFin { float kc, qc, gc, pv, ds, sk, sv; };
+__device__ __forceinline__ ClsFin attn_cls_finish_load(const AttnP& p, int bh, int lane) {
+  const int b = bh / p.H, hh = bh % p.H;
+  const int nq = p.nq_main + p.nq_extra;
+  const long row = tok_row(b, p.nq_main, p.nq_main, p.B);
+  const int col = hh * 64 + lane;
+  const float qc = bf16_to_f32(((const bf16_t*)p.q)[row * p.ldq + col]), kc = bf16_to_f32(((const bf16_t*)p.k)[row * p.ldk + col]);
+  const float vc = bf16_to_f32(((const bf16_t*)p.v)[row * p.ldv + col]), gc = bf16_to_f32(((const bf16_t*)p.dout)[row * p.ld_do + col]);
+  const float s = wave_sum(qc * kc) * p.scale, dp = wave_sum(gc * vc);
+  const float lse = p.lse[(long)bh * nq + p.nq_main], ndelta = p.delta[(long)bh * nq + p.nq_main];
+  const float pv = __expf(s - lse), ds = pv * (dp + ndelta);
+  const float* scr = p.cls_scratch + (long)bh * 192;
+  return ClsFin{kc, qc, gc, pv, ds, scr[64 + lane], scr[128 + lane]};
+}
+template <bool COH>
+__device__ __forceinline__ void attn_cls_finish_store(const AttnP& p, int bh, int lane, const ClsFin& f) {
+  const int b = bh / p.H, hh = bh % p.H;
+  const long row = tok_row(b, p.nq_main, p.nq_main, p.B);
+  const int col = hh * 64 + lane;
+  float* scr = p.cls_scratch + (long)bh * 192;
+  ((bf16_t*)p.dq)[row * p.ld_dq + col] = f32_to_bf16((fin_ld<COH>(scr + lane) + f.ds * f.kc) * p.scale);
+  ((bf16_t*)p.dk)[row * p.ld_dk + col] = f32_to_bf16((f.sk + f.ds * f.qc) * p.scale);
+  ((bf16_t*)p.dv)[row * p.ld_dv + col] = f32_to_bf16(f.sv + f.pv * f.gc);
+  scr[lane] = 0.f, scr[64 + lane] = 0.f, scr[128 + lane] = 0.f;
+}
+__global__ void __launch_bounds__(64) k_attn_cls_finish(AttnP p) {
+  const ClsFin f = attn_cls_finish_load(p, blockIdx.x, threadIdx.x);
+  attn_cls_finish_store<false>(p, blockIdx.x, threadIdx.x, f);
 }
 
 template <int NW = 4>
@@ -406,6 +437,15 @@
     if (!kvalid) wd = 0.f;
     cls_partial(wd, kf, red, lane, p.cls_scratch + ((long)b * p.H + hh) * 192);
   }
+  const bool fold = cls_query && p.cls_cnt != nullptr;
+  unsigned ticket = 0;
+  ClsFin cf = {};
+  if (fold) {
+    asm volatile("s_waitcnt vmcnt(0)" ::: "memory");
+    __syncthreads();
+    if (tid == 0) ticket = __hip_atomic_fetch_add(p.cls_cnt + bh, 1u, __ATOMIC_RELAXED, __HIP_MEMORY_SCOPE_AGENT);
+    if (wave == 0) cf = attn_cls_finish_load(p, bh, lane);
+  }
   if (kvalid) {
     bf16_t* odk = (bf16_t*)p.dk;
     bf16_t* odv = (bf16_t*)p.dv;
@@ -413,6 +453,15 @@
     for (int j = 0; j < 2; ++j) {
       store_block_rows(dk[j], p.scale, odk + krow * p.ld_dk + col0 + 32 * j, h);
       store_block_rows(dv[j], 1.0f, odv + krow * p.ld_dv + col0 + 32 * j, h);
+    }
+  }
+  if (fold) {
+    unsigned* slot = reinterpret_cast<unsigned*>(smem);
+    if (tid == 0) *slot = ticket;
+    __syncthreads();
+    if (*reinterpret_cast<volatile unsigned*>(slot) == gridDim.x - 1 && wave == 0) {
+      attn_cls_finish_store<true>(p, bh, lane, cf);
+      if (lane == 0) __hip_atomic_store(p.cls_cnt + bh, 0u, __ATOMIC_RELAXED, __HIP_MEMORY_SCOPE_AGENT);
     }
   }
 }
@@ -456,34 +505,18 @@
   return VFM_OK;
 }
 
-__global__ void __launch_bounds__(64) k_attn_cls_finish(AttnP p) {
-  const int bh = blockIdx.x, b = bh / p.H, hh = bh % p.H, lane = threadIdx.x;
-  const int nq = p.nq_main + p.nq_extra;
-  const long row = tok_row(b, p.nq_main, p.nq_main, p.B);
-  const int col = hh * 64 + lane;
-  const float qc = bf16_to_f32(((const bf16_t*)p.q)[row * p.ldq + col]), kc = bf16_to_f32(((const bf16_t*)p.k)[row * p.ldk + col]);
-  const float vc = bf16_to_f32(((const bf16_t*)p.v)[row * p.ldv + col]), gc = bf16_to_f32(((const bf16_t*)p.dout)[row * p.ld_do + col]);
-  const float s = wave_sum(qc * kc) * p.scale, dp = wave_sum(gc * vc);
-  const float lse = p.lse[(long)bh * nq + p.nq_main], ndelta = p.delta[(long)bh * nq + p.nq_main];
-  const float pv = __expf(s - lse), ds = pv * (dp + ndelta);
-  float* scr = p.cls_scratch + (long)bh * 192;
-  ((bf16_t*)p.dq)[row * p.ld_dq + col] = f32_to_bf16((scr[lane] + ds * kc) * p.scale);
-  ((bf16_t*)p.dk)[row * p.ld_dk + col] = f32_to_bf16((scr[64 + lane] + ds * qc) * p.scale);
-  ((bf16_t*)p.dv)[row * p.ld_dv + col] = f32_to_bf16(scr[128 + lane] + pv * gc);
-  scr[lane] = 0.f, scr[64 + lane] = 0.f, scr[128 + lane] = 0.f;
-}
-
 int vfm_attn_bf16_bwd_impl(const vfm_attn_desc* d, hipStream_t s) {
   VFM_CHECK(aligned_ok(d, true), VFM_E_ALIGN, "vfm_attn_bwd(bf16): operands must be 16-byte aligned, ld %% 8 == 0");
   AttnP p = to_p(d);
   const int nq = d->nq_main + d->nq_extra, nk = d->nk_main + d->nk_extra;
   const bool cls = d->nq_extra == 1 && d->nk_extra == 1 && d->nq_main == d->nk_main && (d->nq_main % 128) == 0 && !short_grid(d, nq);
   p.cls_scratch = cls ? d->delta + (long)d->B * d->H * nq : nullptr;
+  if (cls && (g_fold_fin & FOLD_ATTN_CLS) && d->B * d->H <= FOLD_WORDS) p.cls_cnt = fold_counters(s);
   if (short_grid(d, nq)) hipLaunchKernelGGL((k_attn_bf16_q<true, 2>), dim3(cdiv(nq, 64), d->B * d->H), dim3(128), 6 * TILE_BYTES, s, p);
   else hipLaunchKernelGGL((k_attn_bf16_q<true, 4>), dim3(cdiv(cls ? d->nq_main : nq, 128), d->B * d->H), dim3(256), 6 * TILE_BYTES, s, p);
   if (short_grid(d, nk)) hipLaunchKernelGGL((k_attn_bf16_dkv<2>), dim3(cdiv(nk, 64), d->B * d->H), dim3(128), 3 * (2 * TILE_BYTES + 1024), s, p);
   else hipLaunchKernelGGL((k_attn_bf16_dkv<4>), dim3(cdiv(cls ? d->nk_main : nk, 128), d->B * d->H), dim3(256), 3 * (2 * TILE_BYTES + 1024), s, p);
-  if (cls) hipLaunchKernelGGL(k_attn_cls_finish, dim3(d->B * d->H), dim3(64), 0, s, p);
+  if (cls && !p.cls_cnt) hipLaunchKernelGGL(k_attn_cls_finish, dim3(d->B * d->H), dim3(64), 0, s, p);
   VFM_LAUNCH_CHECK();
   return VFM_OK;
 }
diff --git a/vfmseg_amd/csrc/attn_common.h b/vfmseg_amd/csrc/attn_common.h
--- a/vfmseg_amd/csrc/attn_common.h
+++ b/vfmseg_amd/csrc/attn_common.h
@@ -12,6 +12,7 @@
   void* dq; void* dk; void* dv; long ld_dq, ld_dk, ld_dv;
   float* delta;
   float* cls_scratch;
+  unsigned* cls_cnt;
   int xcd;
   int il;
 };
@@ -32,6 +33,7 @@
   p.dq = d->dq; p.dk = d->dk; p.dv = d->dv; p.ld_dq = d->ld_dq; p.ld_dk = d->ld_dk; p.ld_dv = d->ld_dv;
   p.delta = d->delta;
   p.cls_scratch = nullptr;
+  p.cls_cnt = nullptr;
   extern int g_attn_xcd;
   p.xcd = g_attn_xcd;
   extern int g_attn_il;
diff --git a/vfmseg_amd/csrc/elementwise.hip b/vfmseg_amd/csrc/elementwise.hip
--- a/vfmseg_amd/csrc/elementwise.hip
+++ b/vfmseg_amd/csrc/elementwise.hip
@@ -1,6 +1,23 @@
 #include "common.h"
+#include "fold_fin.h"
 
 thread_local char g_vfm_err[512] = {0};
+
+extern const int g_fold_fin_default = FOLD_ATTN_CLS;
+int g_fold_fin = g_fold_fin_default;
+unsigned* fold_counters(hipStream_t s) {
+  struct Ent { hipStream_t s; unsigned* w; };
+  static thread_local Ent tab[8];
+  static thread_local int n = 0;
+  for (int i = 0; i < n; ++i)
+    if (tab[i].s == s) return tab[i].w;
+  if (n == 8) return nullptr;
+  void* p = nullptr;
+  if (hipMalloc(&p, FOLD_WORDS * sizeof(unsigned)) != hipSuccess) return nullptr;
+  (void)hipMemsetAsync(p, 0, FOLD_WORDS * sizeof(unsigned), s);
+  tab[n].s = s, tab[n].w = (unsigned*)p, ++n;
+  return (unsigned*)p;
+}
 
 extern "C" const char* vfm_last_error(void) { return g_vfm_err; }
 extern "C" int vfm_abi_version(void) { return 5; }
@@ -184,9 +201,33 @@
   return VFM_OK;
 }
 
+template <bool COH>
+__device__ __forceinline__ void colsum2_dev(const float* __restrict__ ws, long cols, int parts, float* __restrict__ out, int accumulate, int vb,
+                                            float (*sh)[64]) {
+  const int tx = threadIdx.x & 63, g = threadIdx.x >> 6;
+  const long c = vb * 64L + tx;
+  float a = 0.f;
+  if (c < cols) {
+    int p = g;
+    for (; p + 12 < parts; p += 16) {
+      const float v0 = fin_ld<COH>(ws + (long)p * cols + c), v1 = fin_ld<COH>(ws + (long)(p + 4) * cols + c),
+                  v2 = fin_ld<COH>(ws + (long)(p + 8) * cols + c), v3 = fin_ld<COH>(ws + (long)(p + 12) * cols + c);
+      a += (v0 + v1) + (v2 + v3);
+    }
+    for (; p < parts; p += 4) a += fin_ld<COH>(ws + (long)p * cols + c);
+  }
+  sh[g][tx] = a;
+  __syncthreads();
+  if (g == 0 && c < cols) {
+    const float t = (sh[0][tx] + sh[1][tx]) + (sh[2][tx] + sh[3][tx]);
+    out[c] = accumulate ? out[c] + t : t;
+  }
+}
 template <typename T>
-__global__ void k_colsum1(const T* __restrict__ x, long ld, long rows, long cols, float* __restrict__ ws, int CT) {
+__global__ void k_colsum1(const T* __restrict__ x, long ld, long rows, long cols, float* __restrict__ ws, int CT, unsigned* __restrict__ cnt,
+                          float* __restrict__ out, int accumulate) {
   __shared__ float sh[256];
+  __shared__ unsigned slot;
   const int rl = 256 / CT;
   const int tx = threadIdx.x % CT, ty = threadIdx.x / CT;
   const long c = (long)blockIdx.x * CT + tx;
@@ -198,28 +239,17 @@
   if (ty == 0 && c < cols) {
     float a = 0.f;
     for (int k = 0; k < rl; ++k) a += sh[k * CT + tx];
-    ws[(long)blockIdx.y * cols + c] = a;
+    fin_st(ws + (long)blockIdx.y * cols + c, a, cnt != nullptr);
+  }
+  if (cnt) {
+    if (!fin_last_block(cnt + blockIdx.x, gridDim.y, &slot)) return;
+    colsum2_dev<true>(ws, cols, (int)gridDim.y, out, accumulate, blockIdx.x, reinterpret_cast<float(*)[64]>(sh));
+    fin_reset(cnt + blockIdx.x);
   }
 }
 __global__ void __launch_bounds__(256) k_colsum2(const float* __restrict__ ws, long cols, int parts, float* __restrict__ out, int accumulate) {
   __shared__ float sh[4][64];
-  const int tx = threadIdx.x & 63, g = threadIdx.x >> 6;
-  const long c = blockIdx.x * 64L + tx;
-  float a = 0.f;
-  if (c < cols) {
-    int p = g;
-    for (; p + 12 < parts; p += 16) {
-      const float v0 = ws[(long)p * cols + c], v1 = ws[(long)(p + 4) * cols + c], v2 = ws[(long)(p + 8) * cols + c], v3 = ws[(long)(p + 12) * cols + c];
-      a += (v0 + v1) + (v2 + v3);
-    }
-    for (; p < parts; p += 4) a += ws[(long)p * cols + c];
-  }
-  sh[g][tx] = a;
-  __syncthreads();
-  if (g == 0 && c < cols) {
-    const float t = (sh[0][tx] + sh[1][tx]) + (sh[2][tx] + sh[3][tx]);
-    out[c] = accumulate ? out[c] + t : t;
-  }
+  colsum2_dev<false>(ws, cols, parts, out, accumulate, blockIdx.x, sh);
 }
 extern "C" int vfm_colsum(const void* x, int dt, long ld, long rows, long cols, float* out, int accumulate, float* ws,
                           void* stream) {
@@ -233,10 +263,11 @@
   if (parts > 64) parts = 64;
   if (parts < 1) parts = 1;
   dim3 grid(cdiv(cols, CT), (unsigned)parts);
-  if (dt == VFM_F32) hipLaunchKernelGGL(k_colsum1<float>, grid, dim3(256), 0, s, (const float*)x, ld, rows, cols, ws, CT);
-  else if (dt == VFM_BF16) hipLaunchKernelGGL(k_colsum1<bf16_t>, grid, dim3(256), 0, s, (const bf16_t*)x, ld, rows, cols, ws, CT);
+  unsigned* cnt = (g_fold_fin & FOLD_COLSUM) && grid.x <= (unsigned)FOLD_WORDS && grid.x == (unsigned)cdiv(cols, 64) ? fold_counters(s) : nullptr;
+  if (dt == VFM_F32) hipLaunchKernelGGL(k_colsum1<float>, grid, dim3(256), 0, s, (const float*)x, ld, rows, cols, ws, CT, cnt, out, accumulate);
+  else if (dt == VFM_BF16) hipLaunchKernelGGL(k_colsum1<bf16_t>, grid, dim3(256), 0, s, (const bf16_t*)x, ld, rows, cols, ws, CT, cnt, out, accumulate);
   else VFM_FAIL(VFM_E_INVAL, "vfm_colsum: dtype");
-  hipLaunchKernelGGL(k_colsum2, dim3(cdiv(cols, 64)), dim3(256), 0, s, ws, cols, (int)parts, out, accumulate);
+  if (!cnt) hipLaunchKernelGGL(k_colsum2, dim3(cdiv(cols, 64)), dim3(256), 0, s, ws, cols, (int)parts, out, accumulate);
   VFM_LAUNCH_CHECK();
   return VFM_OK;
 }
diff --git a/vfmseg_amd/csrc/fold_fin.h b/vfmseg_amd/csrc/fold_fin.h
--- /dev/null
+++ b/vfmseg_amd/csrc/fold_fin.h
@@ -0,0 +1,28 @@
+#pragma once
+#include "common.h"
+
+enum { FOLD_ATTN_CLS = 1, FOLD_CHAN = 2, FOLD_COLSUM = 4, FOLD_LN_BWD = 8, FOLD_ALL = 15 };
+extern int g_fold_fin;
+extern const int g_fold_fin_default;
+constexpr int FOLD_WORDS = 4096;
+unsigned* fold_counters(hipStream_t s);
+
+template <bool COH>
+__device__ __forceinline__ float fin_ld(const float* p) {
+  if constexpr (COH) return __hip_atomic_load(p, __ATOMIC_RELAXED, __HIP_MEMORY_SCOPE_AGENT);
+  else return *p;
+}
+__device__ __forceinline__ void fin_st(float* p, float v, bool coh) {
+  if (coh) __hip_atomic_store(p, v, __ATOMIC_RELAXED, __HIP_MEMORY_SCOPE_AGENT);
+  else *p = v;
+}
+__device__ __forceinline__ bool fin_last_block(unsigned* cnt, unsigned nblocks, unsigned* slot) {
+  asm volatile("s_waitcnt vmcnt(0)" ::: "memory");
+  __syncthreads();
+  if (threadIdx.x == 0) *slot = __hip_atomic_fetch_add(cnt, 1u, __ATOMIC_RELAXED, __HIP_MEMORY_SCOPE_AGENT);
+  __syncthreads();
+  return *reinterpret_cast<volatile unsigned*>(slot) == nblocks - 1;
+}
+__device__ __forceinline__ void fin_reset(unsigned* cnt) {
+  if (threadIdx.x == 0) __hip_atomic_store(cnt, 0u, __ATOMIC_RELAXED, __HIP_MEMORY_SCOPE_AGENT);
+}
diff --git a/vfmseg_amd/csrc/gemm_bf16.hip b/vfmseg_amd/csrc/gemm_bf16.hip
--- a/vfmseg_amd/csrc/gemm_bf16.hip
+++ b/vfmseg_amd/csrc/gemm_bf16.hip
@@ -1,4 +1,5 @@
 #include "gemm_dev.h"
+#include "fold_fin.h"
 
 template <int BM, int BN, int WM_W, int WN_W, int NS>
 struct Cfg {
@@ -329,6 +330,10 @@
   if (key && strcmp(key, "attn_lds_pad") == 0) {
     extern int g_attn_lds_pad;
     g_attn_lds_pad = value;
+    return VFM_OK;
+  }
+  if (key && strcmp(key, "fold_fin") == 0) {
+    g_fold_fin = value < 0 ? g_fold_fin_default : value;
     return VFM_OK;
   }
   if (key && strcmp(key, "gemm_w44_k") == 0) {
diff --git a/vfmseg_amd/csrc/norm.hip b/vfmseg_amd/csrc/norm.hip
--- a/vfmseg_amd/csrc/norm.hip
+++ b/vfmseg_amd/csrc/norm.hip
@@ -1,4 +1,5 @@
 #include "common.h"
+#include "fold_fin.h"
 
 __device__ __forceinline__ float act_f(float v, int act) {
   return act == VFM_ACT_GELU ? gelu_f(v) : (act == VFM_ACT_RELU ? fmaxf(v, 0.f) : v);
@@ -363,10 +364,31 @@
   return VFM_OK;
 }
 
+template <bool COH>
+__device__ __forceinline__ void ln_bwd_fin_dev(const float* __restrict__ ws, int parts, int C, float* __restrict__ dw, float* __restrict__ db, int vb,
+                                               float (*sh)[4][64]) {
+  const int tx = threadIdx.x & 63, ty = threadIdx.x >> 6;
+  const int c = vb * 64 + tx;
+  float a = 0.f, b = 0.f;
+  if (c < C) {
+#pragma unroll 8
+    for (int p = ty; p < parts; p += 4) {
+      a += fin_ld<COH>(ws + ((long)p * 2 + 0) * C + c);
+      b += fin_ld<COH>(ws + ((long)p * 2 + 1) * C + c);
+    }
+  }
+  sh[0][ty][tx] = a, sh[1][ty][tx] = b;
+  __syncthreads();
+  if (ty == 0 && c < C) {
+    if (dw) dw[c] += (sh[0][0][tx] + sh[0][1][tx]) + (sh[0][2][tx] + sh[0][3][tx]);
+    if (db) db[c] += (sh[1][0][tx] + sh[1][1][tx]) + (sh[1][2][tx] + sh[1][3][tx]);
+  }
+}
 template <typename TD, int MAXPL, bool NEED_W>
 __global__ void k_ln_bwd(const TD* __restrict__ dy, long ld_dy, const float* __restrict__ x, long ld_x,
                          const float* __restrict__ w, const float* __restrict__ stats, float* __restrict__ dx, long ld_dx,
-                         int accumulate_dx, float* __restrict__ ws, long rows, int C) {
+                         int accumulate_dx, float* __restrict__ ws, long rows, int C, unsigned* __restrict__ cnt = nullptr,
+                         float* __restrict__ dw = nullptr, float* __restrict__ db = nullptr) {
   const int lane = threadIdx.x & 63, wv = threadIdx.x >> 6, nw = blockDim.x >> 6;
   float pdw[NEED_W ? MAXPL : 1], pdb[NEED_W ? MAXPL : 1];
 #pragma unroll
@@ -419,28 +441,23 @@
       const int which = c / C, cc = c - which * C;
       float a = 0.f;
       for (int k = 0; k < nw; ++k) a += sh[(k * 2 + which) * C + cc];
-      ws[((long)blockIdx.x * 2 + which) * C + cc] = a;
+      fin_st(ws + ((long)blockIdx.x * 2 + which) * C + cc, a, cnt != nullptr);
+    }
+    if (cnt) {
+      __shared__ float fsh[2][4][64];
+      __shared__ unsigned slot;
+      if (!fin_last_block(cnt, gridDim.x, &slot)) return;
+      for (int vb = 0; vb * 64 < C; ++vb) {
+        ln_bwd_fin_dev<true>(ws, (int)gridDim.x, C, dw, db, vb, fsh);
+        __syncthreads();
+      }
+      fin_reset(cnt);
     }
   }
 }
 __global__ void k_ln_bwd_fin(const float* __restrict__ ws, int parts, int C, float* __restrict__ dw, float* __restrict__ db) {
   __shared__ float sh[2][4][64];
-  const int tx = threadIdx.x & 63, ty = threadIdx.x >> 6;
-  const int c = blockIdx.x * 64 + tx;
-  float a = 0.f, b = 0.f;
-  if (c < C) {
-#pragma unroll 8
-    for (int p = ty; p < parts; p += 4) {
-      a += ws[((long)p * 2 + 0) * C + c];
-      b += ws[((long)p * 2 + 1) * C + c];
-    }
-  }
-  sh[0][ty][tx] = a, sh[1][ty][tx] = b;
-  __syncthreads();
-  if (ty == 0 && c < C) {
-    if (dw) dw[c] += (sh[0][0][tx] + sh[0][1][tx]) + (sh[0][2][tx] + sh[0][3][tx]);
-    if (db) db[c] += (sh[1][0][tx] + sh[1][1][tx]) + (sh[1][2][tx] + sh[1][3][tx]);
-  }
+  ln_bwd_fin_dev<false>(ws, parts, C, dw, db, blockIdx.x, sh);
 }
 
 template <typename TD, int MAXP4>
@@ -625,7 +642,8 @@
   const int parts = need_w ? 128 : cdiv(rows, 4);
   const size_t shm = need_w ? (size_t)4 * 2 * C * sizeof(float) : 0;
   float* wsp = need_w ? ws : nullptr;
-#define L(TD, PL, NW) hipLaunchKernelGGL((k_ln_bwd<TD, PL, NW>), dim3(parts), dim3(256), shm, s, (const TD*)dy, ld_dy, x, ld_x, w, stats, dx, ld_dx, accumulate_dx, wsp, rows, (int)C)
+  unsigned* cnt = need_w && (g_fold_fin & FOLD_LN_BWD) ? fold_counters(s) : nullptr;
+#define L(TD, PL, NW) hipLaunchKernelGGL((k_ln_bwd<TD, PL, NW>), dim3(parts), dim3(256), shm, s, (const TD*)dy, ld_dy, x, ld_x, w, stats, dx, ld_dx, accumulate_dx, wsp, rows, (int)C, cnt, dw, db)
   const int pl = (int)((C + 63) / 64);
   if (need_w) {
     if (dy_dt == VFM_BF16) { if (pl <= 4) L(bf16_t, 4, true); else L(bf16_t, 16, true); }
@@ -637,15 +655,130 @@
     else VFM_FAIL(VFM_E_INVAL, "vfm_layernorm_bwd: dtype");
   }
 #undef L
-  if (need_w) hipLaunchKernelGGL(k_ln_bwd_fin, dim3(cdiv(C, 64)), dim3(256), 0, s, ws, parts, (int)C, dw, db);
+  if (need_w && !cnt) hipLaunchKernelGGL(k_ln_bwd_fin, dim3(cdiv(C, 64)), dim3(256), 0, s, ws, parts, (int)C, dw, db);
   VFM_LAUNCH_CHECK();
   return VFM_OK;
+}
+
+__device__ __forceinline__ double wave_sum_f64(double v) {
+#pragma unroll
+  for (int o = 32; o > 0; o >>= 1) v += __shfl_xor(v, o, 64);
+  return v;
+}
+template <bool COH>
+__device__ __forceinline__ void gn_fin_fwd_dev(const float* __restrict__ ws, int nchunk, int C, int G, long P, float eps,
+                                               float* __restrict__ stats, int BG, int vb) {
+  const int i = vb * 4 + (threadIdx.x >> 6), lane = threadIdx.x & 63;
+  if (i >= BG) return;
+  const int b = i / G, g = i - b * G, cg = C / G;
+  double s = 0.0, q = 0.0;
+  for (int e = lane; e < nchunk * cg; e += 64) {
+    const int k = e / cg, j = e - k * cg;
+    const long slot = (long)b * nchunk + k;
+    s += fin_ld<COH>(ws + (slot * 2 + 0) * C + g * cg + j);
+    q += fin_ld<COH>(ws + (slot * 2 + 1) * C + g * cg + j);
+  }
+  s = wave_sum_f64(s), q = wave_sum_f64(q);
+  if (lane) return;
+  const double n = (double)P * cg;
+  const double mean = s / n;
+  double var = q / n - mean * mean;
+  if (var < 0) var = 0;
+  stats[i * 2] = (float)mean;
+  stats[i * 2 + 1] = (float)(1.0 / sqrt(var + (double)eps));
+}
+template <bool COH>
+__device__ __forceinline__ void gn_fin_bwd_dev(const float* __restrict__ ws, int nchunk, int C, int G, const float* __restrict__ w,
+                                               float* __restrict__ gs, int BG, int vb) {
+  const int i = vb * 4 + (threadIdx.x >> 6), lane = threadIdx.x & 63;
+  if (i >= BG) return;
+  const int b = i / G, g = i - b * G, cg = C / G;
+  double s1 = 0.0, s2 = 0.0;
+  for (int e = lane; e < nchunk * cg; e += 64) {
+    const int k = e / cg, j = e - k * cg;
+    const long slot = (long)b * nchunk + k;
+    const int c = g * cg + j;
+    s1 += (double)w[c] * fin_ld<COH>(ws + (slot * 2 + 0) * C + c);
+    s2 += (double)w[c] * fin_ld<COH>(ws + (slot * 2 + 1) * C + c);
+  }
+  s1 = wave_sum_f64(s1), s2 = wave_sum_f64(s2);
+  if (lane) return;
+  gs[i * 2] = (float)s1;
+  gs[i * 2 + 1] = (float)s2;
+}
+template <bool COH>
+__device__ __forceinline__ void chan_fin_wb_dev(const float* __restrict__ ws, int slots, int C, float* __restrict__ dw, float* __restrict__ db, int vb,
+                                                float (*sh)[4][64]) {
+  const int tx = threadIdx.x & 63, ty = threadIdx.x >> 6;
+  const int c = vb * 64 + tx;
+  float a = 0.f, b = 0.f;
+  if (c < C) {
+#pragma unroll 8
+    for (int k = ty; k < slots; k += 4) {
+      b += fin_ld<COH>(ws + ((long)k * 2 + 0) * C + c);
+      a += fin_ld<COH>(ws + ((long)k * 2 + 1) * C + c);
+    }
+  }
+  sh[0][ty][tx] = a, sh[1][ty][tx] = b;
+  __syncthreads();
+  if (ty == 0 && c < C) {
+    if (dw) dw[c] += (sh[0][0][tx] + sh[0][1][tx]) + (sh[0][2][tx] + sh[0][3][tx]);
+    if (db) db[c] += (sh[1][0][tx] + sh[1][1][tx]) + (sh[1][2][tx] + sh[1][3][tx]);
+  }
+}
+template <bool COH>
+__device__ __forceinline__ void bn_fin_sums_dev(const float* __restrict__ ws, int slots, int C, float* __restrict__ sums, int vb, double (*sh)[4][64]) {
+  const int tx = threadIdx.x & 63, ty = threadIdx.x >> 6;
+  const int c = vb * 64 + tx;
+  double a = 0.0, b = 0.0;
+  if (c < C) {
+#pragma unroll 8
+    for (int k = ty; k < slots; k += 4) {
+      a += fin_ld<COH>(ws + ((long)k * 2 + 0) * C + c);
+      b += fin_ld<COH>(ws + ((long)k * 2 + 1) * C + c);
+    }
+  }
+  sh[0][ty][tx] = a, sh[1][ty][tx] = b;
+  __syncthreads();
+  if (ty == 0 && c < C) {
+    sums[c] = (float)((sh[0][0][tx] + sh[0][1][tx]) + (sh[0][2][tx] + sh[0][3][tx]));
+    sums[C + c] = (float)((sh[1][0][tx] + sh[1][1][tx]) + (sh[1][2][tx] + sh[1][3][tx]));
+  }
+}
+struct ChanFin {
+  unsigned* cnt;
+  int kind;
+  int nchunk, G, BG;
+  long P;
+  float eps;
+  const float* w;
+  float* out;
+  float* dw;
+  float* db;
+};
+template <bool COH = true>
+__device__ __forceinline__ void chan_fin_run(const ChanFin& f, const float* __restrict__ ws, int C, double (*sh)[4][64]) {
+  if (f.kind == 1) {
+    for (int vb = 0; vb * 4 < f.BG; ++vb) gn_fin_fwd_dev<COH>(ws, f.nchunk, C, f.G, f.P, f.eps, f.out, f.BG, vb);
+  } else if (f.kind == 2) {
+    for (int vb = 0; vb * 4 < f.BG; ++vb) gn_fin_bwd_dev<COH>(ws, f.nchunk, C, f.G, f.w, f.out, f.BG, vb);
+    if (f.dw || f.db)
+      for (int vb = 0; vb * 64 < C; ++vb) {
+        chan_fin_wb_dev<COH>(ws, f.BG / f.G * f.nchunk, C, f.dw, f.db, vb, reinterpret_cast<float(*)[4][64]>(sh));
+        __syncthreads();
+      }
+  } else {
+    for (int vb = 0; vb * 64 < C; ++vb) {
+      bn_fin_sums_dev<COH>(ws, f.nchunk, C, f.out, vb, sh);
+      __syncthreads();
+    }
+  }
 }
 
 template <int MODE, typename TD>
 __global__ void k_chan_moments(const float* __restrict__ x, const TD* __restrict__ dy, const float* __restrict__ w,
                                const float* __restrict__ bb, const float* __restrict__ stats, int G, float eps, int act,
-                               float* __restrict__ ws, long P, int C, int rows_per_chunk) {
+                               float* __restrict__ ws, long P, int C, int rows_per_chunk, ChanFin fin) {
   __shared__ float sh[2][4][64];
   const int tx = threadIdx.x & 63, ty = threadIdx.x >> 6;
   const int c = blockIdx.x * 64 + tx;
@@ -688,10 +821,19 @@
   __syncthreads();
   if (ty == 0 && c < C) {
     const long slot = b * gridDim.y + blockIdx.y;
-    ws[(slot * 2 + 0) * C + c] = sh[0][0][tx] + sh[0][1][tx] + sh[0][2][tx] + sh[0][3][tx];
-    ws[(slot * 2 + 1) * C + c] = sh[1][0][tx] + sh[1][1][tx] + sh[1][2][tx] + sh[1][3][tx];
-  }
-}
+    fin_st(ws + (slot * 2 + 0) * C + c, sh[0][0][tx] + sh[0][1][tx] + sh[0][2][tx] + sh[0][3][tx], fin.cnt != nullptr);
+    fin_st(ws + (slot * 2 + 1) * C + c, sh[1][0][tx] + sh[1][1][tx] + sh[1][2][tx] + sh[1][3][tx], fin.cnt != nullptr);
+  }
+  if (fin.cnt) {
+    __shared__ double fsh[2][4][64];
+    __shared__ unsigned slot;
+    if (!fin_last_block(fin.cnt, gridDim.x * gridDim.y * gridDim.z, &slot)) return;
+    chan_fin_run(fin, ws, C, fsh);
+    fin_reset(fin.cnt);
+  }
+}
+static inline ChanFin chan_fin_none() { return ChanFin{nullptr, 0, 0, 0, 0, 0, 0.f, nullptr, nullptr, nullptr, nullptr}; }
+static inline unsigned* chan_fin_counter(hipStream_t s) { return (g_fold_fin & FOLD_CHAN) ? fold_counters(s) : nullptr; }
 
 static inline int pick_chunks(long P) {
   int n = (int)((P + 63) / 64);
@@ -700,31 +842,9 @@
   return n;
 }
 
-__device__ __forceinline__ double wave_sum_f64(double v) {
-#pragma unroll
-  for (int o = 32; o > 0; o >>= 1) v += __shfl_xor(v, o, 64);
-  return v;
-}
 __global__ void k_gn_fin_fwd(const float* __restrict__ ws, int nchunk, int C, int G, long P, float eps,
                              float* __restrict__ stats, int BG) {
-  const int i = blockIdx.x * (blockDim.x >> 6) + (threadIdx.x >> 6), lane = threadIdx.x & 63;
-  if (i >= BG) return;
-  const int b = i / G, g = i - b * G, cg = C / G;
-  double s = 0.0, q = 0.0;
-  for (int e = lane; e < nchunk * cg; e += 64) {
-    const int k = e / cg, j = e - k * cg;
-    const long slot = (long)b * nchunk + k;
-    s += ws[(slot * 2 + 0) * C + g * cg + j];
-    q += ws[(slot * 2 + 1) * C + g * cg + j];
-  }
-  s = wave_sum_f64(s), q = wave_sum_f64(q);
-  if (lane) return;
-  const double n = (double)P * cg;
-  const double mean = s / n;
-  double var = q / n - mean * mean;
-  if (var < 0) var = 0;
-  stats[i * 2] = (float)mean;
-  stats[i * 2 + 1] = (float)(1.0 / sqrt(var + (double)eps));
+  gn_fin_fwd_dev<false>(ws, nchunk, C, G, P, eps, stats, BG, blockIdx.x);
 }
 template <typename TO>
 __global__ void k_gn_apply(const float* __restrict__ x, const float* __restrict__ w, const float* __restrict__ b,
@@ -747,9 +867,10 @@
   const int nchunk = pick_chunks(P);
   const int rpc = (int)((P + nchunk - 1) / nchunk);
   float* ws = ws_in + B * G * 2;
+  const ChanFin fin{chan_fin_counter(s), 1, nchunk, G, (int)(B * G), P, eps, nullptr, stats, nullptr, nullptr};
   hipLaunchKernelGGL((k_chan_moments<0, float>), dim3(cdiv(C, 64), nchunk, (unsigned)B), dim3(256), 0, s, x, (const float*)nullptr,
-                     (const float*)nullptr, (const float*)nullptr, (const float*)nullptr, 0, 0.f, 0, ws, P, (int)C, rpc);
-  hipLaunchKernelGGL(k_gn_fin_fwd, dim3(cdiv(B * G, 4)), dim3(256), 0, s, ws, nchunk, (int)C, G, P, eps, stats, (int)(B * G));
+                     (const float*)nullptr, (const float*)nullptr, (const float*)nullptr, 0, 0.f, 0, ws, P, (int)C, rpc, fin);
+  if (!fin.cnt) hipLaunchKernelGGL(k_gn_fin_fwd, dim3(cdiv(B * G, 4)), dim3(256), 0, s, ws, nchunk, (int)C, G, P, eps, stats, (int)(B * G));
   const long total = B * P * C;
   const int grid = (int)((total + 255) / 256 > 8192 ? 8192 : (total + 255) / 256);
   if (y_dt == VFM_BF16) hipLaunchKernelGGL(k_gn_apply<bf16_t>, dim3(grid), dim3(256), 0, s, x, w, b, stats, G, act, (bf16_t*)y, B, P, (int)C);
@@ -761,40 +882,11 @@
 
 __global__ void k_gn_fin_bwd(const float* __restrict__ ws, int nchunk, int C, int G, const float* __restrict__ w,
                              float* __restrict__ gs, int BG) {
-  const int i = blockIdx.x * (blockDim.x >> 6) + (threadIdx.x >> 6), lane = threadIdx.x & 63;
-  if (i >= BG) return;
-  const int b = i / G, g = i - b * G, cg = C / G;
-  double s1 = 0.0, s2 = 0.0;
-  for (int e = lane; e < nchunk * cg; e += 64) {
-    const int k = e / cg, j = e - k * cg;
-    const long slot = (long)b * nchunk + k;
-    const int c = g * cg + j;
-    s1 += (double)w[c] * ws[(slot * 2 + 0) * C + c];
-    s2 += (double)w[c] * ws[(slot * 2 + 1) * C + c];
-  }
-  s1 = wave_sum_f64(s1), s2 = wave_sum_f64(s2);
-  if (lane) return;
-  gs[i * 2] = (float)s1;
-  gs[i * 2 + 1] = (float)s2;
+  gn_fin_bwd_dev<false>(ws, nchunk, C, G, w, gs, BG, blockIdx.x);
 }
 __global__ void k_chan_fin_wb(const float* __restrict__ ws, int slots, int C, float* __restrict__ dw, float* __restrict__ db) {
   __shared__ float sh[2][4][64];
-  const int tx = threadIdx.x & 63, ty = threadIdx.x >> 6;
-  const int c = blockIdx.x * 64 + tx;
-  float a = 0.f, b = 0.f;
-  if (c < C) {
-#pragma unroll 8
-    for (int k = ty; k < slots; k += 4) {
-      b += ws[((long)k * 2 + 0) * C + c];
-      a += ws[((long)k * 2 + 1) * C + c];
-    }
-  }
-  sh[0][ty][tx] = a, sh[1][ty][tx] = b;
-  __syncthreads();
-  if (ty == 0 && c < C) {
-    if (dw) dw[c] += (sh[0][0][tx] + sh[0][1][tx]) + (sh[0][2][tx] + sh[0][3][tx]);
-    if (db) db[c] += (sh[1][0][tx] + sh[1][1][tx]) + (sh[1][2][tx] + sh[1][3][tx]);
-  }
+  chan_fin_wb_dev<false>(ws, slots, C, dw, db, blockIdx.x, sh);
 }
 template <typename TD>
 __global__ void k_gn_bwd_apply(const TD* __restrict__ dy, const float* __restrict__ x, const float* __restrict__ w,
@@ -825,13 +917,14 @@
   float* gs = ws;
   float* part = ws + B * G * 2;
   dim3 grid(cdiv(C, 64), nchunk, (unsigned)B);
+  const ChanFin fin{chan_fin_counter(s), 2, nchunk, G, (int)(B * G), P, 0.f, w, gs, dw, db};
   if (dy_dt == VFM_BF16)
-    hipLaunchKernelGGL((k_chan_moments<1, bf16_t>), grid, dim3(256), 0, s, x, (const bf16_t*)dy, w, b, stats, G, 0.f, act, part, P, (int)C, rpc);
+    hipLaunchKernelGGL((k_chan_moments<1, bf16_t>), grid, dim3(256), 0, s, x, (const bf16_t*)dy, w, b, stats, G, 0.f, act, part, P, (int)C, rpc, fin);
   else if (dy_dt == VFM_F32)
-    hipLaunchKernelGGL((k_chan_moments<1, float>), grid, dim3(256), 0, s, x, (const float*)dy, w, b, stats, G, 0.f, act, part, P, (int)C, rpc);
+    hipLaunchKernelGGL((k_chan_moments<1, float>), grid, dim3(256), 0, s, x, (const float*)dy, w, b, stats, G, 0.f, act, part, P, (int)C, rpc, fin);
   else VFM_FAIL(VFM_E_INVAL, "vfm_groupnorm_bwd: dtype");
-  hipLaunchKernelGGL(k_gn_fin_bwd, dim3(cdiv(B * G, 4)), dim3(256), 0, s, part, nchunk, (int)C, G, w, gs, (int)(B * G));
-  if (dw || db) hipLaunchKernelGGL(k_chan_fin_wb, dim3(cdiv(C, 64)), dim3(256), 0, s, part, (int)(B * nchunk), (int)C, dw, db);
+  if (!fin.cnt) hipLaunchKernelGGL(k_gn_fin_bwd, dim3(cdiv(B * G, 4)), dim3(256), 0, s, part, nchunk, (int)C, G, w, gs, (int)(B * G));
+  if (!fin.cnt && (dw || db)) hipLaunchKernelGGL(k_chan_fin_wb, dim3(cdiv(C, 64)), dim3(256), 0, s, part, (int)(B * nchunk), (int)C, dw, db);
   const long total = B * P * C;
   const int g2 = (int)((total + 255) / 256 > 8192 ? 8192 : (total + 255) / 256);
   if (dy_dt == VFM_BF16) hipLaunchKernelGGL(k_gn_bwd_apply<bf16_t>, dim3(g2), dim3(256), 0, s, (const bf16_t*)dy, x, w, b, stats, gs, G, act, dx, B, P, (int)C);
@@ -1011,31 +1104,17 @@
 
 __global__ void __launch_bounds__(256) k_bn_fin_sums(const float* __restrict__ ws, int slots, int C, float* __restrict__ sums) {
   __shared__ double sh[2][4][64];
-  const int tx = threadIdx.x & 63, ty = threadIdx.x >> 6;
-  const int c = blockIdx.x * 64 + tx;
-  double a = 0.0, b = 0.0;
-  if (c < C) {
-#pragma unroll 8
-    for (int k = ty; k < slots; k += 4) {
-      a += ws[((long)k * 2 + 0) * C + c];
-      b += ws[((long)k * 2 + 1) * C + c];
-    }
-  }
-  sh[0][ty][tx] = a, sh[1][ty][tx] = b;
-  __syncthreads();
-  if (ty == 0 && c < C) {
-    sums[c] = (float)((sh[0][0][tx] + sh[0][1][tx]) + (sh[0][2][tx] + sh[0][3][tx]));
-    sums[C + c] = (float)((sh[1][0][tx] + sh[1][1][tx]) + (sh[1][2][tx] + sh[1][3][tx]));
-  }
+  bn_fin_sums_dev<false>(ws, slots, C, sums, blockIdx.x, sh);
 }
 extern "C" int vfm_bn_moments(const float* x, long rows, long C, float* sums, float* ws, void* stream) {
   VFM_CHECK(ws && sums, VFM_E_INVAL, "vfm_bn_moments: args");
   hipStream_t s = (hipStream_t)stream;
   const int nchunk = pick_chunks(rows);
   const int rpc = (int)((rows + nchunk - 1) / nchunk);
+  const ChanFin fin{chan_fin_counter(s), 3, nchunk, 0, 0, rows, 0.f, nullptr, sums, nullptr, nullptr};
   hipLaunchKernelGGL((k_chan_moments<0, float>), dim3(cdiv(C, 64), nchunk, 1), dim3(256), 0, s, x, (const float*)nullptr,
-                     (const float*)nullptr, (const float*)nullptr, (const float*)nullptr, 0, 0.f, 0, ws, rows, (int)C, rpc);
-  hipLaunchKernelGGL(k_bn_fin_sums, dim3(cdiv(C, 64)), dim3(256), 0, s, ws, nchunk, (int)C, sums);
+                     (const float*)nullptr, (const float*)nullptr, (const float*)nullptr, 0, 0.f, 0, ws, rows, (int)C, rpc, fin);
+  if (!fin.cnt) hipLaunchKernelGGL(k_bn_fin_sums, dim3(cdiv(C, 64)), dim3(256), 0, s, ws, nchunk, (int)C, sums);
   VFM_LAUNCH_CHECK();
   return VFM_OK;
 }
@@ -1087,12 +1166,13 @@
   const int nchunk = pick_chunks(rows);
   const int rpc = (int)((rows + nchunk - 1) / nchunk);
   dim3 grid(cdiv(C, 64), nchunk, 1);
+  const ChanFin fin{chan_fin_counter(s), 3, nchunk, 0, 0, rows, 0.f, nullptr, sums_dy, nullptr, nullptr};
   if (dy_dt == VFM_BF16)
-    hipLaunchKernelGGL((k_chan_moments<1, bf16_t>), grid, dim3(256), 0, s, x, (const bf16_t*)dy, w, b, mean_var, 0, eps, act, ws, rows, (int)C, rpc);
+    hipLaunchKernelGGL((k_chan_moments<1, bf16_t>), grid, dim3(256), 0, s, x, (const bf16_t*)dy, w, b, mean_var, 0, eps, act, ws, rows, (int)C, rpc, fin);
   else if (dy_dt == VFM_F32)
-    hipLaunchKernelGGL((k_chan_moments<1, float>), grid, dim3(256), 0, s, x, (const float*)dy, w, b, mean_var, 0, eps, act, ws, rows, (int)C, rpc);
+    hipLaunchKernelGGL((k_chan_moments<1, float>), grid, dim3(256), 0, s, x, (const float*)dy, w, b, mean_var, 0, eps, act, ws, rows, (int)C, rpc, fin);
   else VFM_FAIL(VFM_E_INVAL, "vfm_bn_bwd_reduce: dtype");
-  hipLaunchKernelGGL(k_bn_fin_sums, dim3(cdiv(C, 64)), dim3(256), 0, s, ws, nchunk, (int)C, sums_dy);
+  if (!fin.cnt) hipLaunchKernelGGL(k_bn_fin_sums, dim3(cdiv(C, 64)), dim3(256), 0, s, ws, nchunk, (int)C, sums_dy);
   VFM_LAUNCH_CHECK();
   return VFM_OK;
 }
```

Result: no change. 129.2 images/s, median of 6 (+0.3%).
